# importZL/semantic_segmentation

Measured on AMD Instinct MI355X. Metric: images/sec (fwd+bwd) U-Net 256x256 bs=32 per GPU, higher is better.
Workload: dtype f16; 1 GPU; unet.UNet(1,2) 256x256 fwd+bwd, CE+Dice loss, batch 32/GPU (BASELINE configs[1]); global_batch=32, parallelism=dp1, dice=per-rank

## Files before the change

include/gsseg.h:

```cpp
#ifndef GSSEG_H
#define GSSEG_H

#include <stdint.h>

#ifdef __cplusplus
extern "C" {
#endif

#define GS_ABI_VERSION 52

enum GsDtype { GS_F16 = 0, GS_BF16 = 1 };
enum GsStatus { GS_OK = 0, GS_EINVAL = -1, GS_ELAUNCH = -2, GS_EUNSUPPORTED = -3 };
enum GsAct { GS_ACT_NONE = 0, GS_ACT_RELU = 1, GS_ACT_LEAKY02 = 2, GS_ACT_TANH = 3 };

#define GS_MAX_TAPS 64

typedef struct GsConvGeom {
    int32_t N, IH, IW, Cin, in_pix_stride, in_coff;
    int32_t OHg, OWg, Cout;
    int32_t OH, OW, out_pix_stride, out_coff;
    int32_t isy, isx, osy, osx, ooy, oox;
    int32_t ntaps;
    int32_t tap_dy[GS_MAX_TAPS], tap_dx[GS_MAX_TAPS];
    int32_t tap_w[GS_MAX_TAPS];
    int32_t Dg, Din, Dout, isz, osz, ooz;
    int32_t tap_dz[GS_MAX_TAPS];
} GsConvGeom;

const char* gs_last_error(void);
int gs_abi_version(void);

int gs_conv_igemm_mtiles(const GsConvGeom* g);
int64_t gs_conv_igemm_workspace_floats(void);
int gs_conv_igemm(const GsConvGeom* g, const void* x, const void* w, void* y, const float* bias,
                  float* bn_partials, int act, int dtype, float* splitk_ws, int64_t splitk_ws_floats, void* stream);
int gs_conv_igemm_batch(int n, const GsConvGeom* const* g, const void* x, const void* const* w, void* y, const float* bias,
                        float* const* bn_partials, int act, int dtype, float* splitk_ws, int64_t splitk_ws_floats,
                        void* stream);

int gs_upconv2x2_fwd(const void* x, const void* w, const float* bias, void* y, int N, int D, int IH, int IW, int Cin,
                     int in_pix_stride, int in_coff, int Cout, int Dout, int OH, int OW, int out_pix_stride,
                     int out_coff, int ooz, int ooy, int oox, int act, int dtype, void* stream);

int gs_upconv2x2_dgrad(const void* dy, const void* wd, void* dx, int N, int IH, int IW, int Cin, int Cout, int OH, int OW,
                       int dy_pix_stride, int dy_coff, int ooy, int oox, int dx_pix_stride, int dx_coff, int dtype,
                       void* stream);

int gs_conv3x3_mtiles(int N, int H, int W, int Cout);
int gs_conv3x3_stat_rows(int N, int H, int W, int Cin, int Cout, int pair);
int gs_conv3x3_set_kernel_form(int form);
int gs_set_persistent_grid(int blocks);
int gs_get_persistent_grid(void);
int gs_conv3x3(const void* x, const void* w, void* y, const float* bias, float* bn_partials, int N, int H, int W,
               int Cin, int in_pix_stride, int in_coff, int Cout, int out_pix_stride, int out_coff,
               const int32_t* tap_dy, const int32_t* tap_dx, int act, int dtype, void* stream);

int gs_conv3x3_wgrad(const void* x, const void* dy, float* dw, int N, int H, int W, int Cin, int in_pix_stride,
                     int in_coff, int Cout, int out_pix_stride, int out_coff, int dtype, void* stream);

int gs_conv_wgrad(const GsConvGeom* g, const void* x, const void* dy, float* dw, int dtype, void* stream);
int gs_conv_wgrad_single_pass(const GsConvGeom* g);
int gs_conv_wgrad_assign(const GsConvGeom* g, const void* x, const void* dy, float* dw, int dtype, void* stream);
int gs_conv_wgrad_parts(const GsConvGeom* g);
int64_t gs_conv_wgrad_ws_floats(const GsConvGeom* g);
int gs_conv_wgrad_slabs(const GsConvGeom* g, const void* x, const void* dy, float* ws, int dtype, void* stream);
int gs_conv_wgrad_slabs_batch(int n, const GsConvGeom* const* g, const void* x, const void* dy, float* ws, int dtype,
                              void* stream);

int gs_conv_smallcin_mtiles(int N, int OH, int OW);
int gs_conv_smallcin_fwd(const float* x, const float* w, const float* bias, void* y, float* bn_partials,
                         int N, int Cin, int IH, int IW, int Cout, int OH, int OW, int k, int stride, int pad,
                         int act, int dtype, void* stream);
int64_t gs_conv_direct_wgrad_ws_floats(int N, int OH, int OW, int Cin, int Cout, int k);

int gs_stem_stats(const float* x, const float* w, float* bn_partials, float* tap_sums, int N, int H, int W, void* stream);
int gs_stem_fwd_bn(const float* x, const float* w, const float* bn_scale, const float* bn_shift, int act, void* z, int N,
                   int H, int W, int dtype, void* stream);
int gs_stem_bwd_tiles(int N, int H, int W);
int gs_stem_bwd_onepass(const float* x, const void* z, const void* dz, int dz_stride, int dz_coff, int act,
                        float* s1_partials, float* ws, int N, int H, int W, int dtype, void* stream);
int gs_stem_bwd_finalize(const float* ws, const float* s1_partials, const float* tap_sums, const float* w,
                         const float* scale, const float* mean, const float* invstd, int train_stats, float gscale, float* dw,
                         float* dgamma, float* dbeta, int N, int H, int W, void* stream);

int gs_stem_bn_bwd_wgrad(const void* y, const void* dz, int dz_stride, int dz_coff, const float* x, const float* scale,
                         const float* shift, const float* mean, const float* invstd, const float* c1, const float* c2,
                         int act, float* dw, float* ws, int N, int H, int W, float gscale, int dtype, void* stream);

int gs_conv_smallcin_wgrad(const float* x, const void* dy, float* dw, float* ws, int N, int Cin, int IH, int IW,
                           int Cout, int OH, int OW, int k, int stride, int pad, float gscale, int dtype, void* stream);
int gs_conv_smallcin_dgrad(const void* dy, const float* w, float* dx, int N, int Cin, int IH, int IW, int Cout,
                           int OH, int OW, int k, int stride, int pad, float gscale, int dtype, void* stream);

int gs_conv_smallcout_fwd(const void* x, const float* w, const float* bias, float* y, int N, int IH, int IW, int Cin,
                          int Cout, int OH, int OW, int k, int stride, int pad, int dtype, void* stream);
int gs_conv_smallcout_bwd(const void* x, const float* w, const float* dy, void* dx, float* dw, float* db, float* ws,
                          int N, int IH, int IW, int Cin, int Cout, int OH, int OW, int k, int stride, int pad,
                          float gscale, int dtype, void* stream);

int64_t gs_bn_partials_floats(int ntiles, int C);
int gs_bn_finalize(const float* partials, int ntiles, int C, double count, const float* gamma, const float* beta,
                   float* running_mean, float* running_var, float momentum, float eps,
                   float* scale, float* shift, float* mean, float* invstd, void* stream);
int gs_bn_eval_coeffs(int C, const float* gamma, const float* beta, const float* running_mean,
                      const float* running_var, float eps, float* scale, float* shift, float* mean, float* invstd,
                      void* stream);

int gs_bn_act_apply(const void* y, const float* scale, const float* shift, int act, void* z, int z_pix_stride,
                    int z_coff, void* zp, const uint8_t* keep_mask, float keep_scale, int N, int H, int W, int C,
                    int dtype, void* stream);

int gs_bn_bwd_tiles(int N, int H, int W);
int gs_bn_bwd_tiles_used(int N, int H, int W, int pooled);
int gs_bn_act_bwd_reduce(const void* y, const void* dz_a, int sa, int coff_a, const void* dzp,
                         const void* dz_b, int act_b, const uint8_t* keep_mask, float keep_scale,
                         const float* scale, const float* shift, const float* mean, const float* invstd, int act,
                         float* partials, int N, int H, int W, int C, int dtype, void* stream);
int gs_bn_bwd_coeffs(const float* partials, int ntiles, int C, double count, float gscale, float* dgamma,
                     float* dbeta, float* c1, float* c2, void* stream);
int gs_bn_act_bwd_apply(const void* y, const void* dz_a, int sa, int coff_a, const void* dzp,
                        const void* dz_b, int act_b, const uint8_t* keep_mask, float keep_scale,
                        const float* scale, const float* shift, const float* mean, const float* invstd,
                        const float* c1, const float* c2, int act, int bn, void* dy, int N, int H, int W, int C,
                        int dtype, void* stream);

int gs_maxpool3d_fwd(const void* z, int z_pix_stride, int z_coff, void* zp, int NB, int D, int H, int W, int C,
                     int dtype, void* stream);
int gs_maxpool3d_fwd_pair(const void* z_hi, const void* z_lo, int z_pix_stride, void* zp_hi, void* zp_lo, int zp_pix_stride,
                          int NB, int D, int H, int W, int C, int dtype, void* stream);
int gs_maxpool3d_fwd_pair_q8(const void* z_hi, const void* z_lo, int z_q8, int zq_coff, int z_pix_stride, void* zp_hi, void* zp_lo,
                             int zp_q8, int zp_pix_stride, int NB, int D, int H, int W, int C, int dtype, void* stream);
int gs_maxpool3d_bwd(const void* z, int z_pix_stride, int z_coff, const void* dzp, const void* dres,
                     int res_pix_stride, int res_coff, void* dz, int NB, int D, int H, int W, int C, int dtype,
                     void* stream);

int gs_maxpool2x2_fwd(const void* z, int z_pix_stride, int z_coff, void* zp, int N, int H, int W, int C, int dtype,
                      void* stream);
int gs_maxpool2x2_fwd_pair(const void* z_hi, const void* z_lo, int z_pix_stride, void* zp_hi, void* zp_lo, int zp_pix_stride, int N, int H,
                           int W, int C, int dtype, void* stream);

int gs_colsum(const void* t, int pix_stride, int coff, int N, int H, int W, int y0, int x0, int h, int w, int C,
              float gscale, float* ws, float* out, int dtype, void* stream);

int gs_head1x1_bn_fwd(const void* y_conv, const float* bn_scale, const float* bn_shift, int act, const float* w,
                      const float* bias, float* logits, int N, int H, int W, int Cout, int dtype, void* stream);
int gs_head1x1_bn_wgrad(const void* y_conv, const float* bn_scale, const float* bn_shift, int act, const float* w,
                        const float* dl, float* dw, float* db, float* ws, int N, int H, int W, int Cout, float gscale,
                        int dtype, void* stream);

int gs_bn_act_bwd_reduce_head(const void* y, const float* dl, const float* w_head, int ncls, const float* scale,
                              const float* shift, const float* mean, const float* invstd, int act, float* partials, int N,
                              int H, int W, int C, int dtype, void* stream);
int gs_bn_act_bwd_apply_head(const void* y, const float* dl, const float* w_head, int ncls, const float* scale,
                             const float* shift, const float* mean, const float* invstd, const float* c1, const float* c2,
                             int act, void* dy, int N, int H, int W, int C, int dtype, void* stream);

int gs_bn_partials_colsum(const float* partials, int ntiles, int Cfull, int coff, int C, float gscale, float* out,
                          void* stream);

int gs_pack_weight(const float* w, void* w_fwd, void* w_dgrad, int Cout, int Cin, int taps, int transposed,
                   int dtype, void* stream);

typedef struct GsPackDesc {
    const float* w;
    void* w_fwd;
    void* w_dgrad;
    int32_t Cout, Cin, taps, transposed;
} GsPackDesc;
int gs_pack_weight_multi(int n, const GsPackDesc* descs, int dtype, void* stream);
int gs_unpack_wgrad(const float* dw, float* grad, int A, int B, int taps, int transposed, float gscale, void* stream);

int64_t gs_fake_postprocess_ws_floats(int N);
int gs_fake_postprocess(const float* x, float* out, float* ws, const float* gamma_lut, int N, int64_t hw, void* stream);

int64_t gs_isic_fake_trans_ws_bytes(int planes, int64_t hw);
int gs_isic_fake_trans(const float* x, float* out, void* ws, int N, int C, int H, int W, int equalize_on, int bits,
                       int sharpness_on, float sharp_r1, float sharp_r2, int autocontrast_on, int saturation_on, float sat_r1,
                       float sat_r2, void* stream);

int gs_upconv8_image_fwd(const void* x, int in_pix_stride, int in_coff, const void* pack_fwd, int cpad, const float* bias,
                         float* out, void* u, int N, int h, int w, int Cin, int Cout, int act, int dtype, void* stream);
int gs_upconv8_image_wgrad_ok(int Cin, int Cout);
int64_t gs_upconv8_image_wgrad_ws_floats(int N, int h, int w, int Cin);
int gs_upconv8_image_wgrad(const void* x, int x_pix_stride, const void* du, int du_pix_stride, float* ws, float* dwm, int N, int h, int w,
                           int Cin, int dtype, void* stream);

int gs_upconv_merge_pack(const float* w4, const float* w6, const float* w8, const float* softmax3, void* pack_fwd,
                         void* pack_dgrad, float* merged_f32, int Cin, int Cout, int dtype, void* stream);
int gs_upconv_split_wgrad(const float* dwm, const float* w4, const float* w6, const float* w8, const float* softmax3,
                          float gscale, float* dw4, float* dw6, float* dw8, float* dots3, int Cin, int Cout,
                          void* stream);
int64_t gs_upconv_split_wgrad_ws_floats(int Cin, int Cout);
int gs_upconv_split_wgrad_det(const float* dwm, const float* w4, const float* w6, const float* w8, const float* softmax3,
                              float gscale, float* dw4, float* dw6, float* dw8, float* dots3, float* ws, int Cin, int Cout,
                              void* stream);
int gs_upconv_split_wgrad_parts_ok(int Cin, int Cout);
int gs_upconv_split_wgrad_parts(const float* slabs, int nparts, int64_t part_stride, const float* w4, const float* w6,
                                const float* w8, const float* softmax3, float gscale, float* dw4, float* dw6, float* dw8,
                                float* dots3, float* ws, int Cin, int Cout, void* stream);

int gs_nchw_to_nhwc(const float* src, void* dst, int N, int C, int H, int W, int dst_pix_stride, int dst_coff,
                    int dtype, void* stream);
int gs_nhwc_to_nchw(const void* src, int src_pix_stride, int src_coff, float* dst, int N, int C, int H, int W,
                    float gscale, int dtype, void* stream);

int gs_seg_loss_fwd(const float* logits, const uint8_t* mask, int N, int C, int H, int W, float* ws, float* out,
                    void* stream);
int gs_seg_loss_bwd(const float* logits, const uint8_t* mask, const float* out, const float* gout, float gscale,
                    float* dlogits, int N, int C, int H, int W, void* stream);
int64_t gs_dice_batched_ws_floats(int B);
int gs_dice_coeff_batched(const float* p, const float* t, int B, int64_t n_per, float* ws, float* out, void* stream);
int gs_eval_dice(const float* logits, const uint8_t* mask, int N, int C, int64_t HW, float* ws, float* out, void* stream);
int gs_eval_jaccard(const float* logits, const uint8_t* mask, int N, int64_t HW, float* ws, float* out, void* stream);
int64_t gs_jaccard_loss_out_floats(int N);
int gs_jaccard_seg_loss_fwd(const float* logits, const uint8_t* mask, int N, int64_t HW, float* ws, float* out, void* stream);
int gs_jaccard_seg_loss_bwd(const float* logits, const uint8_t* mask, const float* out, const float* gout, float gscale,
                            float* dlogits, int N, int64_t HW, void* stream);
int gs_dice_loss_fwd(const float* p, const float* t, int64_t n, float* ws, float* out, void* stream);
int gs_dice_loss_bwd(const float* t, const float* out, const float* gout, float* dp, int64_t n, void* stream);
int gs_mean_loss_fwd(const float* x, const float* t, float cval, int mode, int64_t n, float* ws, float* out,
                     void* stream);
int gs_mean_loss_bwd(const float* x, const float* t, float cval, int mode, int64_t n, const float* gout,
                     float gscale, float* dx, void* stream);

int gs_pack_weight_split(const float* w, void* pack, int Cout, int Cin, int taps, int transposed, int dtype, void* stream);
#define GS_SEG_MAX 4
typedef struct GsSegPackDesc {
    const float* w;
    void* pack;
    int32_t Cout, Cin, taps, transposed, nseg;
    int32_t kind[GS_SEG_MAX], ci0[GS_SEG_MAX], len[GS_SEG_MAX];
} GsSegPackDesc;
int gs_pack_weight_segs(int n, const GsSegPackDesc* descs, int dtype, void* stream);
int gs_conv3x3_precise(const void* x, const void* w, void* y_hi, void* y_lo, const float* bias, float* bn_partials, int N,
                       int H, int W, int K, int in_pix_stride, int in_coff, int in_wrap, int Cout, int out_pix_stride,
                       int out_coff, const int32_t* tap_dy, const int32_t* tap_dx, int act, int dtype, void* stream);
typedef struct GsQ8PackDesc {
    const float* w;
    void* pack;
    int32_t* wexp;
    int32_t Cout, Cin, taps;
} GsQ8PackDesc;
int gs_pack_weight_q8(int n, const GsQ8PackDesc* descs, int dtype, void* stream);
int gs_conv3x3_q8_ok(int W, int Cin, int Cout);
int gs_conv3x3_q8(const void* x, const void* w, const int32_t* wexp, void* y_hi, void* y_lo, float* bn_partials, int N, int H, int W,
                  int Cin, int in_pix_stride, int in_coff, int Cout, int out_pix_stride, int out_coff, int dtype, void* stream);
int gs_conv3d_3x3x3_q8(const void* x, const void* w, const int32_t* wexp, void* y_hi, void* y_lo, float* bn_partials, int NB, int D,
                       int H, int W, int Cin, int in_pix_stride, int in_coff, int Cout, int out_pix_stride, int out_coff, int dtype,
                       void* stream);
int gs_bn_act_apply_split_q8(const void* y_hi, const void* y_lo, const float* scale, const float* shift, int act, void* z_hi,
                             void* z_lo, int z_q8, int z_pix_stride, int z_coff, void* zp_hi, void* zp_lo, int zp_q8,
                             int zp_pix_stride, int N, int H, int W, int C, int dtype, void* stream);
int gs_stem_fwd_bn_pair_q8(const float* x, const float* w, const float* bn_scale, const float* bn_shift, int act, void* z_hi,
                           void* z_q, int z_pix_stride, int N, int H, int W, int dtype, void* stream);
int gs_q8_from_hi(const void* x, void* q, int64_t pixels, int C, int pix_stride, int coff, int dtype, void* stream);
int gs_conv3d_3x3x3_precise(const void* x, const void* w, void* y_hi, void* y_lo, const float* bias, float* bn_partials,
                            int NB, int D, int H, int W, int K, int in_pix_stride, int in_coff, int in_wrap, int Cout,
                            int out_pix_stride, int out_coff, const int32_t* tap_dz, const int32_t* tap_dy,
                            const int32_t* tap_dx, int act, int dtype, void* stream);
int gs_conv3d_3x3x3_precise_to(const void* x, const void* w, void* y_hi, void* y_lo, const float* bias, float* bn_partials, int NB, int D,
                               int H, int W, int K, int in_pix_stride, int in_coff, int in_wrap, int in_wrap_to, int Cout, int out_pix_stride,
                               int out_coff, const int32_t* tap_dz, const int32_t* tap_dy, const int32_t* tap_dx, int act, int dtype,
                               void* stream);
int gs_upconv2x2_fwd_precise(const void* x, const void* w, const float* bias, void* y_hi, void* y_lo, int N, int IH, int IW,
                             int K, int in_pix_stride, int in_coff, int in_wrap, int Cout, int OH, int OW,
                             int out_pix_stride, int out_coff, int ooy, int oox, int dtype, void* stream);
int gs_conv_smallcin_fwd_split(const float* x, const float* w, void* y_hi, void* y_lo, float* bn_partials, int N, int Cin,
                               int H, int W, int Cout, int k, int pad, int dtype, void* stream);
int gs_bn_act_apply_split(const void* y_hi, const void* y_lo, const float* scale, const float* shift, int act, void* z_hi,
                          void* z_lo, int z_pix_stride, int z_coff, void* zp_hi, void* zp_lo, int zp_pix_stride, int N,
                          int H, int W, int C, int dtype, void* stream);
int gs_bn_act_apply_split_pool3d(const void* y_hi, const void* y_lo, const float* scale, const float* shift, int act, void* z_hi, void* z_lo,
                                 int z_pix_stride, int z_coff, void* zp_hi, void* zp_lo, int zp_pix_stride, int NB, int D, int H, int W, int C,
                                 int dtype, void* stream);
int gs_head1x1_fwd_split(const void* x_hi, const void* x_lo, const float* w, const float* bias, float* y, int N, int H,
                         int W, int Cin, int Cout, int dtype, void* stream);
int64_t gs_head1x1_wide_bwd_ws_floats(int N, int H, int W, int ncls);
int gs_head1x1_wide_bwd(const void* z, const float* w, const float* dl, void* dz, float* dw, float* db, float* ws, int N, int H,
                        int W, int ncls, float gscale, int dtype, void* stream);
int gs_head1x1_wide_fwd(const void* x, const float* w, const float* bias, float* y, int N, int H, int W, int ncls, int dtype,
                        void* stream);
int gs_conv_widecin_mtiles(int N, int H, int W);
int gs_conv_widecin_fwd_split(const float* x, const float* w, void* y_hi, void* y_lo, float* bn_partials, int N, int Cin, int H,
                              int W, int Cout, int dtype, void* stream);
int gs_head1x1_bn_fwd_split(const void* y_hi, const void* y_lo, const float* scale, const float* shift, int act, const float* w,
                            const float* bias, float* logits, int N, int H, int W, int Cin, int Cout, int dtype, void* stream);
int gs_stem_fwd_bn_pair(const float* x, const float* w, const float* bn_scale, const float* bn_shift, int act, void* z_hi,
                        void* z_lo, int z_pix_stride, int N, int H, int W, int dtype, void* stream);
int gs_stem_bwd_onepass_strided(const float* x, const void* z, int z_pix_stride, const void* dz, int dz_stride, int dz_coff,
                                int act, float* s1_partials, float* ws, int N, int H, int W, int dtype, void* stream);

int gs_upconv2x2_wgrad_parts(int N, int IH, int IW, int Cin, int Cout);
int64_t gs_upconv2x2_wgrad_ws_floats(int N, int IH, int IW, int Cin, int Cout);
int gs_upconv2x2_wgrad_slabs(const void* x, const void* dy, float* ws, int N, int IH, int IW, int Cin, int x_pix_stride,
                             int x_coff, int Cout, int OH, int OW, int dy_pix_stride, int dy_coff, int ooy, int oox, int dtype,
                             void* stream);

int64_t gs_conv3x3_wgrad_ws_floats(int N, int H, int W, int Cin, int Cout);
int gs_conv3x3_wgrad_parts(int N, int H, int W, int Cin, int Cout);
int gs_conv3x3_wgrad_slabs(const void* x, const void* dy, float* ws, int N, int H, int W, int Cin, int in_pix_stride,
                           int in_coff, int Cout, int out_pix_stride, int out_coff, int dtype, void* stream);
int gs_wgrad_reduce_unpack(const float* ws, int nparts, float* grad, int A, int B, int taps, int transposed,
                           float gscale, void* stream);

int gs_conv3d_3x3x3_mtiles(int NB, int D, int H, int W, int Cout);
int gs_conv3d_3x3x3(const void* x, const void* w, void* y, const float* bias, float* bn_partials, int NB, int D, int H,
                    int W, int Cin, int in_pix_stride, int in_coff, int Cout, int out_pix_stride, int out_coff,
                    const int32_t* tap_dz, const int32_t* tap_dy, const int32_t* tap_dx, int act, int dtype, void* stream);
int gs_conv3d_3x3x3_wgrad(const void* x, const void* dy, float* dw, int NB, int D, int H, int W, int Cin,
                          int in_pix_stride, int in_coff, int Cout, int out_pix_stride, int out_coff, int dtype,
                          void* stream);
int64_t gs_conv3d_3x3x3_wgrad_ws_floats(int NB, int D, int H, int W, int Cin, int Cout);
int gs_conv3d_3x3x3_wgrad_parts(int NB, int D, int H, int W, int Cin, int Cout);
int gs_conv3d_3x3x3_wgrad_slabs(const void* x, const void* dy, float* ws, int NB, int D, int H, int W, int Cin,
                                int in_pix_stride, int in_coff, int Cout, int out_pix_stride, int out_coff, int dtype,
                                void* stream);

int gs_upsample2x_bilinear_fwd(const void* x, void* y, int N, int IH, int IW, int C, int in_pix_stride, int in_coff,
                               int OH, int OW, int out_pix_stride, int out_coff, int ooy, int oox, int dtype, void* stream);
int gs_upsample2x_bilinear_fwd_pair(const void* x_hi, const void* x_lo, void* y_hi, void* y_lo, int N, int IH, int IW, int C,
                                    int in_pix_stride, int in_coff, int OH, int OW, int out_pix_stride, int out_coff, int ooy,
                                    int oox, int dtype, void* stream);
int gs_upsample2x_bilinear_bwd(const void* dy, void* dx, int N, int IH, int IW, int C, int dy_pix_stride, int dy_coff,
                               int OH, int OW, int dx_pix_stride, int dx_coff, int ooy, int oox, int dtype, void* stream);

int gs_affine_warp(const float* src, float* dst, const float* mats, int N, int C, int H, int W, float thresh,
                   void* stream);

int gs_optim_chunk_elems(void);
int gs_optim_rmsprop(float* const* params, const float* const* grads, float* const* square_avg,
                     float* const* momentum_buf, const int64_t* sizes, const int32_t* chunk_tensor,
                     const int64_t* chunk_start, int nchunks, float lr, float alpha, float eps, float weight_decay,
                     float momentum, float grad_scale, void* stream);
int gs_optim_adam(float* const* params, const float* const* grads, float* const* exp_avg, float* const* exp_avg_sq,
                  const int64_t* sizes, const int32_t* chunk_tensor, const int64_t* chunk_start, int nchunks,
                  const float* step_scalars, float beta1, float beta2, float eps, float weight_decay, float grad_scale,
                  void* stream);

#ifdef __cplusplus
}
#endif
#endif
```

semantic_segmentation_amd/_lib.py:

```python
from __future__ import annotations

import ctypes
import os
import subprocess
from ctypes import POINTER, c_char_p, c_double, c_float, c_int, c_int32, c_int64, c_void_p

_HERE = os.path.dirname(os.path.abspath(__file__))
LIB_PATH = os.environ.get("GSSEG_LIB", os.path.join(_HERE, "libgsseg_hip.so"))
CSRC = os.path.join(_HERE, "csrc")

GS_F16, GS_BF16 = 0, 1
ACT_NONE, ACT_RELU, ACT_LEAKY02, ACT_TANH = 0, 1, 2, 3
GS_MAX_TAPS = 64
ABI_VERSION = 52


class GsConvGeom(ctypes.Structure):
    _fields_ = [(n, c_int32) for n in (
        "N", "IH", "IW", "Cin", "in_pix_stride", "in_coff", "OHg", "OWg", "Cout", "OH", "OW",
        "out_pix_stride", "out_coff", "isy", "isx", "osy", "osx", "ooy", "oox", "ntaps")] + [
        ("tap_dy", c_int32 * GS_MAX_TAPS), ("tap_dx", c_int32 * GS_MAX_TAPS), ("tap_w", c_int32 * GS_MAX_TAPS)] + [
        (n, c_int32) for n in ("Dg", "Din", "Dout", "isz", "osz", "ooz")] + [("tap_dz", c_int32 * GS_MAX_TAPS)]


class GsPackDesc(ctypes.Structure):
    _fields_ = [("w", c_void_p), ("w_fwd", c_void_p), ("w_dgrad", c_void_p)] + [
        (n, c_int32) for n in ("Cout", "Cin", "taps", "transposed")]


GS_SEG_MAX = 4


class GsSegPackDesc(ctypes.Structure):
    _fields_ = [("w", c_void_p), ("pack", c_void_p)] + [(n, c_int32) for n in ("Cout", "Cin", "taps", "transposed", "nseg")] + [
        ("kind", c_int32 * GS_SEG_MAX), ("ci0", c_int32 * GS_SEG_MAX), ("len", c_int32 * GS_SEG_MAX)]


class GsQ8PackDesc(ctypes.Structure):
    _fields_ = [("w", c_void_p), ("pack", c_void_p), ("wexp", c_void_p)] + [(n, c_int32) for n in ("Cout", "Cin", "taps")]


_P, _F = c_void_p, c_void_p
PROTOTYPES = {
    "gs_last_error": (c_char_p, []),
    "gs_abi_version": (c_int, []),
    "gs_conv_igemm_mtiles": (c_int, [POINTER(GsConvGeom)]),
    "gs_conv3x3_stat_rows": (c_int, [c_int] * 6),
    "gs_upconv2x2_wgrad_parts": (c_int, [c_int] * 5),
    "gs_upconv2x2_wgrad_ws_floats": (c_int64, [c_int] * 5),
    "gs_upconv2x2_wgrad_slabs": (c_int, [_P, _P, _F] + [c_int] * 14 + [c_void_p]),
    "gs_set_persistent_grid": (c_int, [c_int]),
    "gs_get_persistent_grid": (c_int, []),
    "gs_conv_igemm": (c_int, [POINTER(GsConvGeom), _P, _P, _P, _F, _F, c_int, c_int, _F, c_int64, c_void_p]),
    "gs_conv_igemm_workspace_floats": (c_int64, []),
    "gs_conv_igemm_batch": (c_int, [c_int, POINTER(POINTER(GsConvGeom)), _P, POINTER(c_void_p), _P, _F, POINTER(c_void_p),
                                    c_int, c_int, _F, c_int64, c_void_p]),
    "gs_upconv2x2_fwd": (c_int, [_P, _P, _F, _P] + [c_int] * 18 + [c_void_p]),
    "gs_upconv2x2_dgrad": (c_int, [c_void_p, c_void_p, c_void_p] + [c_int] * 14 + [c_void_p]),
    "gs_conv3x3_mtiles": (c_int, [c_int, c_int, c_int, c_int]),
    "gs_conv3x3_set_kernel_form": (c_int, [c_int]),
    "gs_conv3d_3x3x3_mtiles": (c_int, [c_int] * 5),
    "gs_conv3d_3x3x3": (c_int, [_P, _P, _P, _F, _F] + [c_int] * 10 + [POINTER(c_int32)] * 3 + [c_int, c_int, c_void_p]),
    "gs_conv3d_3x3x3_wgrad_ws_floats": (c_int64, [c_int] * 6),
    "gs_conv3d_3x3x3_wgrad_parts": (c_int, [c_int] * 6),
    "gs_conv3d_3x3x3_wgrad_slabs": (c_int, [_P, _P, _F] + [c_int] * 11 + [c_void_p]),
    "gs_conv3d_3x3x3_wgrad": (c_int, [_P, _P, _F] + [c_int] * 11 + [c_void_p]),
    "gs_upsample2x_bilinear_fwd": (c_int, [_P, _P] + [c_int] * 13 + [c_void_p]),
    "gs_upsample2x_bilinear_bwd": (c_int, [_P, _P] + [c_int] * 13 + [c_void_p]),
    "gs_affine_warp": (c_int, [_F, _F, _F, c_int, c_int, c_int, c_int, c_float, c_void_p]),
    "gs_optim_chunk_elems": (c_int, []),
    "gs_optim_rmsprop": (c_int, [_P] * 7 + [c_int] + [c_float] * 6 + [c_void_p]),
    "gs_optim_adam": (c_int, [_P] * 7 + [c_int, _P] + [c_float] * 5 + [c_void_p]),
    "gs_conv3x3": (c_int, [_P, _P, _P, _F, _F] + [c_int] * 9 + [POINTER(c_int32), POINTER(c_int32), c_int, c_int, c_void_p]),
    "gs_conv3x3_wgrad": (c_int, [_P, _P, _F] + [c_int] * 10 + [c_void_p]),
    "gs_conv3x3_wgrad_ws_floats": (c_int64, [c_int] * 5),
    "gs_conv3x3_wgrad_parts": (c_int, [c_int] * 5),
    "gs_conv3x3_wgrad_slabs": (c_int, [_P, _P, _F] + [c_int] * 10 + [c_void_p]),
    "gs_wgrad_reduce_unpack": (c_int, [_F, c_int, _F, c_int, c_int, c_int, c_int, c_float, c_void_p]),
    "gs_conv_wgrad": (c_int, [POINTER(GsConvGeom), _P, _P, _F, c_int, c_void_p]),
    "gs_conv_wgrad_assign": (c_int, [POINTER(GsConvGeom), _P, _P, _F, c_int, c_void_p]),
    "gs_conv_wgrad_single_pass": (c_int, [POINTER(GsConvGeom)]),
    "gs_conv_wgrad_parts": (c_int, [POINTER(GsConvGeom)]),
    "gs_conv_wgrad_ws_floats": (c_int64, [POINTER(GsConvGeom)]),
    "gs_conv_wgrad_slabs": (c_int, [POINTER(GsConvGeom), _P, _P, _F, c_int, c_void_p]),
    "gs_conv_wgrad_slabs_batch": (c_int, [c_int, POINTER(POINTER(GsConvGeom)), _P, _P, _F, c_int, c_void_p]),
    "gs_conv_smallcin_mtiles": (c_int, [c_int, c_int, c_int]),
    "gs_conv_smallcin_fwd": (c_int, [_F, _F, _F, _P, _F] + [c_int] * 12 + [c_void_p]),
    "gs_conv_direct_wgrad_ws_floats": (c_int64, [c_int] * 6),
    "gs_conv_smallcin_wgrad": (c_int, [_F, _P, _F, _F] + [c_int] * 10 + [c_float, c_int, c_void_p]),
    "gs_conv_smallcin_dgrad": (c_int, [_P, _F, _F] + [c_int] * 10 + [c_float, c_int, c_void_p]),
    "gs_conv_smallcout_fwd": (c_int, [_P, _F, _F, _F] + [c_int] * 11 + [c_void_p]),
    "gs_conv_smallcout_bwd": (c_int, [_P, _F, _F, _P, _F, _F, _F] + [c_int] * 10 + [c_float, c_int, c_void_p]),
    "gs_bn_partials_floats": (c_int64, [c_int, c_int]),
    "gs_bn_finalize": (c_int, [_F, c_int, c_int, c_double, _F, _F, _F, _F, c_float, c_float, _F, _F, _F, _F, c_void_p]),
    "gs_bn_eval_coeffs": (c_int, [c_int, _F, _F, _F, _F, c_float, _F, _F, _F, _F, c_void_p]),
    "gs_bn_act_apply": (c_int, [_P, _F, _F, c_int, _P, c_int, c_int, _P, _P, c_float] + [c_int] * 5 + [c_void_p]),
    "gs_bn_bwd_tiles": (c_int, [c_int, c_int, c_int]),
    "gs_bn_bwd_tiles_used": (c_int, [c_int, c_int, c_int, c_int]),
    "gs_bn_act_bwd_reduce": (c_int, [_P, _P, c_int, c_int, _P, _P, c_int, _P, c_float, _F, _F, _F, _F, c_int, _F]
                             + [c_int] * 5 + [c_void_p]),
    "gs_bn_bwd_coeffs": (c_int, [_F, c_int, c_int, c_double, c_float, _F, _F, _F, _F, c_void_p]),
    "gs_bn_act_bwd_apply": (c_int, [_P, _P, c_int, c_int, _P, _P, c_int, _P, c_float, _F, _F, _F, _F, _F, _F, c_int,
                                    c_int, _P]
                            + [c_int] * 5 + [c_void_p]),
    "gs_maxpool3d_fwd": (c_int, [_P, c_int, c_int, _P] + [c_int] * 6 + [c_void_p]),
    "gs_maxpool2x2_fwd": (c_int, [_P, c_int, c_int, _P] + [c_int] * 5 + [c_void_p]),
    "gs_maxpool2x2_fwd_pair": (c_int, [_P, _P, c_int, _P, _P, c_int] + [c_int] * 5 + [c_void_p]),
    "gs_maxpool3d_bwd": (c_int, [_P, c_int, c_int, _P, _P, c_int, c_int, _P] + [c_int] * 6 + [c_void_p]),
    "gs_colsum": (c_int, [_P, c_int, c_int] + [c_int] * 8 + [c_float, _F, _F, c_int, c_void_p]),
    "gs_stem_bn_bwd_wgrad": (c_int, [_P, _P, c_int, c_int, _F, _F, _F, _F, _F, _F, _F, c_int, _F, _F, c_int, c_int, c_int,
                                     c_float, c_int, c_void_p]),
    "gs_stem_stats": (c_int, [_F, _F, _F, _F, c_int, c_int, c_int, c_void_p]),
    "gs_stem_bwd_onepass": (c_int, [_F, _P, _P, c_int, c_int, c_int, _F, _F, c_int, c_int, c_int, c_int, c_void_p]),
    "gs_stem_bwd_finalize": (c_int, [_F, _F, _F, _F, _F, _F, _F, c_int, c_float, _F, _F, _F, c_int, c_int, c_int, c_void_p]),
    "gs_stem_fwd_bn": (c_int, [_F, _F, _F, _F, c_int, _P, c_int, c_int, c_int, c_int, c_void_p]),
    "gs_stem_bwd_tiles": (c_int, [c_int, c_int, c_int]),
    "gs_head1x1_bn_fwd": (c_int, [_P, _F, _F, c_int, _F, _F, _F] + [c_int] * 5 + [c_void_p]),
    "gs_head1x1_bn_wgrad": (c_int, [_P, _F, _F, c_int, _F, _F, _F, _F, _F] + [c_int] * 4 + [c_float, c_int, c_void_p]),
    "gs_bn_act_bwd_reduce_head": (c_int, [_P, _F, _F, c_int, _F, _F, _F, _F, c_int, _F] + [c_int] * 5 + [c_void_p]),
    "gs_bn_act_bwd_apply_head": (c_int, [_P, _F, _F, c_int, _F, _F, _F, _F, _F, _F, c_int, _P] + [c_int] * 5 + [c_void_p]),
    "gs_bn_partials_colsum": (c_int, [_F, c_int, c_int, c_int, c_int, c_float, _F, c_void_p]),
    "gs_pack_weight": (c_int, [_F, _P, _P, c_int, c_int, c_int, c_int, c_int, c_void_p]),
    "gs_pack_weight_multi": (c_int, [c_int, POINTER(GsPackDesc), c_int, c_void_p]),
    "gs_unpack_wgrad": (c_int, [_F, _F, c_int, c_int, c_int, c_int, c_float, c_void_p]),
    "gs_upconv_merge_pack": (c_int, [_F, _F, _F, _F, _P, _P, _F, c_int, c_int, c_int, c_void_p]),
    "gs_fake_postprocess_ws_floats": (c_int64, [c_int]),
    "gs_isic_fake_trans_ws_bytes": (c_int64, [c_int, c_int64]),
    "gs_isic_fake_trans": (c_int, [_F, _F, _P, c_int, c_int, c_int, c_int, c_int, c_int, c_int, c_float, c_float, c_int, c_int,
                                   c_float, c_float, c_void_p]),
    "gs_fake_postprocess": (c_int, [_F, _F, _F, _F, c_int, c_int64, c_void_p]),
    "gs_upconv8_image_fwd": (c_int, [_P, c_int, c_int, _P, c_int, _F, _F, _P] + [c_int] * 7 + [c_void_p]),
    "gs_upconv8_image_wgrad_ok": (c_int, [c_int, c_int]),
    "gs_upconv8_image_wgrad_ws_floats": (c_int64, [c_int] * 4),
    "gs_upconv8_image_wgrad": (c_int, [_P, c_int, _P, c_int, _F, _F] + [c_int] * 5 + [c_void_p]),
    "gs_upconv_split_wgrad": (c_int, [_F, _F, _F, _F, _F, c_float, _F, _F, _F, _F, c_int, c_int, c_void_p]),
    "gs_upconv_split_wgrad_det": (c_int, [_F, _F, _F, _F, _F, c_float, _F, _F, _F, _F, _F, c_int, c_int, c_void_p]),
    "gs_upconv_split_wgrad_ws_floats": (c_int64, [c_int, c_int]),
    "gs_upconv_split_wgrad_parts_ok": (c_int, [c_int, c_int]),
    "gs_upconv_split_wgrad_parts": (c_int, [_F, c_int, c_int64, _F, _F, _F, _F, c_float, _F, _F, _F, _F, _F, c_int, c_int, c_void_p]),
    "gs_nchw_to_nhwc": (c_int, [_F, _P] + [c_int] * 7 + [c_void_p]),
    "gs_nhwc_to_nchw": (c_int, [_P, c_int, c_int, _F] + [c_int] * 4 + [c_float, c_int, c_void_p]),
    "gs_seg_loss_fwd": (c_int, [_F, _P, c_int, c_int, c_int, c_int, _F, _F, c_void_p]),
    "gs_seg_loss_bwd": (c_int, [_F, _P, _F, _F, c_float, _F, c_int, c_int, c_int, c_int, c_void_p]),
    "gs_dice_batched_ws_floats": (c_int64, [c_int]),
    "gs_dice_coeff_batched": (c_int, [_F, _F, c_int, c_int64, _F, _F, c_void_p]),
    "gs_eval_dice": (c_int, [_F, _P, c_int, c_int, c_int64, _F, _F, c_void_p]),
    "gs_jaccard_loss_out_floats": (c_int64, [c_int]),
    "gs_jaccard_seg_loss_fwd": (c_int, [_F, _P, c_int, c_int64, _F, _F, c_void_p]),
    "gs_jaccard_seg_loss_bwd": (c_int, [_F, _P, _F, _F, c_float, _F, c_int, c_int64, c_void_p]),
    "gs_eval_jaccard": (c_int, [_F, _P, c_int, c_int64, _F, _F, c_void_p]),
    "gs_dice_loss_fwd": (c_int, [_F, _F, c_int64, _F, _F, c_void_p]),
    "gs_dice_loss_bwd": (c_int, [_F, _F, _F, _F, c_int64, c_void_p]),
    "gs_mean_loss_fwd": (c_int, [_F, _F, c_float, c_int, c_int64, _F, _F, c_void_p]),
    "gs_pack_weight_split": (c_int, [_F, _P, c_int, c_int, c_int, c_int, c_int, c_void_p]),
    "gs_pack_weight_segs": (c_int, [c_int, POINTER(GsSegPackDesc), c_int, c_void_p]),
    "gs_pack_weight_q8": (c_int, [c_int, POINTER(GsQ8PackDesc), c_int, c_void_p]),
    "gs_conv3x3_q8_ok": (c_int, [c_int] * 3),
    "gs_conv3x3_q8": (c_int, [_P, _P, _P, _P, _P, _F] + [c_int] * 10 + [c_void_p]),
    "gs_conv3d_3x3x3_q8": (c_int, [_P, _P, _P, _P, _P, _F] + [c_int] * 11 + [c_void_p]),
    "gs_bn_act_apply_split_q8": (c_int, [_P, _P, _F, _F, c_int, _P, _P, c_int, c_int, c_int, _P, _P, c_int, c_int] + [c_int] * 5 + [c_void_p]),
    "gs_stem_fwd_bn_pair_q8": (c_int, [_F, _F, _F, _F, c_int, _P, _P, c_int, c_int, c_int, c_int, c_int, c_void_p]),
    "gs_q8_from_hi": (c_int, [_P, _P, c_int64, c_int, c_int, c_int, c_int, c_void_p]),
    "gs_conv3d_3x3x3_precise": (c_int, [_P, _P, _P, _P, _F, _F] + [c_int] * 11 + [POINTER(c_int32)] * 3 + [c_int, c_int, c_void_p]),
    "gs_conv3d_3x3x3_precise_to": (c_int, [_P, _P, _P, _P, _F, _F] + [c_int] * 12 + [POINTER(c_int32)] * 3 + [c_int, c_int, c_void_p]),
    "gs_maxpool3d_fwd_pair_q8": (c_int, [_P, _P, c_int, c_int, c_int, _P, _P, c_int, c_int] + [c_int] * 6 + [c_void_p]),
    "gs_maxpool3d_fwd_pair": (c_int, [_P, _P, c_int, _P, _P] + [c_int] * 7 + [c_void_p]),
    "gs_upsample2x_bilinear_fwd_pair": (c_int, [_P, _P, _P, _P] + [c_int] * 13 + [c_void_p]),
    "gs_conv3x3_precise": (c_int, [_P, _P, _P, _P, _F, _F] + [c_int] * 10 + [POINTER(c_int32), POINTER(c_int32), c_int, c_int, c_void_p]),
    "gs_upconv2x2_fwd_precise": (c_int, [_P, _P, _F, _P, _P] + [c_int] * 15 + [c_void_p]),
    "gs_conv_smallcin_fwd_split": (c_int, [_F, _F, _P, _P, _F] + [c_int] * 8 + [c_void_p]),
    "gs_bn_act_apply_split": (c_int, [_P, _P, _F, _F, c_int, _P, _P, c_int, c_int, _P, _P] + [c_int] * 6 + [c_void_p]),
    "gs_bn_act_apply_split_pool3d": (c_int, [_P, _P, _F, _F, c_int, _P, _P, c_int, c_int, _P, _P] + [c_int] * 7 + [c_void_p]),
    "gs_conv_widecin_mtiles": (c_int, [c_int, c_int, c_int]),
    "gs_conv_widecin_fwd_split": (c_int, [_F, _F, _P, _P, _F] + [c_int] * 6 + [c_void_p]),
    "gs_head1x1_fwd_split": (c_int, [_P, _P, _F, _F, _F] + [c_int] * 6 + [c_void_p]),
    "gs_head1x1_wide_bwd_ws_floats": (c_int64, [c_int] * 4),
    "gs_head1x1_wide_bwd": (c_int, [_P, _F, _F, _P, _F, _F, _F] + [c_int] * 4 + [c_float, c_int, c_void_p]),
    "gs_head1x1_wide_fwd": (c_int, [_P, _F, _F, _F] + [c_int] * 5 + [c_void_p]),
    "gs_head1x1_bn_fwd_split": (c_int, [_P, _P, _F, _F, c_int, _F, _F, _F] + [c_int] * 6 + [c_void_p]),
    "gs_stem_fwd_bn_pair": (c_int, [_F, _F, _F, _F, c_int, _P, _P, c_int, c_int, c_int, c_int, c_int, c_void_p]),
    "gs_stem_bwd_onepass_strided": (c_int, [_F, _P, c_int, _P, c_int, c_int, c_int, _F, _F, c_int, c_int, c_int, c_int, c_void_p]),
    "gs_mean_loss_bwd": (c_int, [_F, _F, c_float, c_int, c_int64, _F, c_float, _F, c_void_p]),
}

_lib = None


def build(verbose: bool = False) -> str:
    cmd = ["make", "-C", CSRC, "-j", str(min(8, os.cpu_count() or 1))]
    res = subprocess.run(cmd, stdout=subprocess.PIPE, stderr=subprocess.STDOUT, text=True)
    if verbose or res.returncode != 0:
        print(res.stdout)
    if res.returncode != 0:
        raise RuntimeError("building libgsseg_hip.so failed:\n" + res.stdout[-4000:])
    return LIB_PATH


def load():
    global _lib
    if _lib is not None:
        return _lib
    import torch
    if not os.path.exists(LIB_PATH):
        raise RuntimeError(
            f"{LIB_PATH} not found: the HIP extension is not built.  Run "
            "`python -c 'import __graft_entry__ as g; g.build()'` (or make -C semantic_segmentation_amd/csrc). "
            "There is no CPU/PyTorch fallback for this path.")
    lib = ctypes.CDLL(LIB_PATH)
    for name, (res, args) in PROTOTYPES.items():
        fn = getattr(lib, name)
        fn.restype = res
        fn.argtypes = args
    if lib.gs_abi_version() != ABI_VERSION:
        raise RuntimeError(f"libgsseg_hip.so ABI {lib.gs_abi_version()} != binding {ABI_VERSION}: rebuild")
    _lib = lib
    return lib


GS_EUNSUPPORTED = -3


def check(rc: int, what: str = "") -> None:
    if rc != 0:
        msg = load().gs_last_error()
        raise RuntimeError(f"{what or 'gsseg'} failed (status {rc}): {msg.decode() if msg else ''}")


def call(name: str, *args):
    rc = getattr(load(), name)(*args)
    if rc != 0:
        check(rc, name)
    return rc
```

semantic_segmentation_amd/csrc/bn.hip:

```cpp
#include <stdlib.h>

#include "common.hpp"

namespace {

constexpr int RED_SLICES = 64;

__global__ __launch_bounds__(256) void reduce_partials_stage1(const float* __restrict__ part, int ntiles, int C,
                                                              int tiles_per_slice, double* __restrict__ out1) {
    __shared__ double red[2][8][32];
    const int cl = threadIdx.x & 31, tl = threadIdx.x >> 5;
    const int c = blockIdx.x * 32 + cl;
    const int t0 = blockIdx.y * tiles_per_slice, t1 = min(ntiles, t0 + tiles_per_slice);
    double s1 = 0.0, s2 = 0.0;
    if (c < C) {
        for (int tt = t0 + tl; tt < t1; tt += 8) {
            s1 += (double)part[((int64_t)tt * 2 + 0) * C + c];
            s2 += (double)part[((int64_t)tt * 2 + 1) * C + c];
        }
    }
    red[0][tl][cl] = s1;
    red[1][tl][cl] = s2;
    __syncthreads();
    if (tl == 0 && c < C) {
        double a = 0.0, b = 0.0;
#pragma unroll
        for (int i = 0; i < 8; ++i) { a += red[0][i][cl]; b += red[1][i][cl]; }
        out1[((int64_t)blockIdx.y * 2 + 0) * C + c] = a;
        out1[((int64_t)blockIdx.y * 2 + 1) * C + c] = b;
    }
}

template <typename T>
__device__ __forceinline__ void sum_slices_32x8(const T* __restrict__ s, int nslices, int C, double& s1, double& s2) {
    __shared__ double red[2][8][32];
    const int cl = threadIdx.x & 31, tl = threadIdx.x >> 5;
    const int c = blockIdx.x * 32 + cl;
    double a = 0.0, b = 0.0;
    if (c < C) {
#pragma unroll 4
        for (int i = tl; i < nslices; i += 8) { a += (double)s[((int64_t)i * 2 + 0) * C + c]; b += (double)s[((int64_t)i * 2 + 1) * C + c]; }
    }
    red[0][tl][cl] = a;
    red[1][tl][cl] = b;
    __syncthreads();
    s1 = 0.0; s2 = 0.0;
#pragma unroll
    for (int i = 0; i < 8; ++i) { s1 += red[0][i][cl]; s2 += red[1][i][cl]; }
}

template <typename T>
__global__ __launch_bounds__(256) void bn_finalize_kernel(const T* __restrict__ s, int nslices, int C, double count,
                                                          const float* __restrict__ gamma, const float* __restrict__ beta,
                                                          float* running_mean, float* running_var, float momentum,
                                                          float eps, float* scale, float* shift, float* mean_out,
                                                          float* invstd_out) {
    double s1, s2;
    sum_slices_32x8(s, nslices, C, s1, s2);
    const int c = blockIdx.x * 32 + (threadIdx.x & 31);
    if (c >= C || threadIdx.x >= 32) return;
    const double mean = s1 / count;
    double var = s2 / count - mean * mean;
    if (var < 0.0) var = 0.0;
    const float invstd = (float)(1.0 / sqrt(var + (double)eps));
    const float gm = gamma ? gamma[c] : 1.f, bt = beta ? beta[c] : 0.f;
    const float sc = gm * invstd;
    scale[c] = sc;
    shift[c] = bt - (float)mean * sc;
    mean_out[c] = (float)mean;
    invstd_out[c] = invstd;
    if (running_mean) running_mean[c] = (1.f - momentum) * running_mean[c] + momentum * (float)mean;
    if (running_var) {
        const double unb = count > 1.0 ? var * (count / (count - 1.0)) : var;
        running_var[c] = (1.f - momentum) * running_var[c] + momentum * (float)unb;
    }
}

__global__ void bn_eval_coeffs_kernel(int C, const float* gamma, const float* beta, const float* rm, const float* rv,
                                      float eps, float* scale, float* shift, float* mean, float* invstd) {
    const int c = blockIdx.x * blockDim.x + threadIdx.x;
    if (c >= C) return;
    const float is = 1.f / sqrtf(rv[c] + eps);
    const float sc = (gamma ? gamma[c] : 1.f) * is;
    scale[c] = sc;
    shift[c] = (beta ? beta[c] : 0.f) - rm[c] * sc;
    mean[c] = rm[c];
    invstd[c] = is;
}

template <typename T>
__global__ __launch_bounds__(256) void bn_bwd_coeffs_kernel(const T* __restrict__ s, int nslices, int C, double count,
                                                            float gscale, float* dgamma, float* dbeta, float* c1, float* c2) {
    double s1, s2;
    sum_slices_32x8(s, nslices, C, s1, s2);
    const int c = blockIdx.x * 32 + (threadIdx.x & 31);
    if (c >= C || threadIdx.x >= 32) return;
    if (dbeta) dbeta[c] = (float)(s1 * gscale);
    if (dgamma) dgamma[c] = (float)(s2 * gscale);
    c1[c] = (float)(s1 / count);
    c2[c] = (float)(s2 / count);
}

static int bn_traversal() {
    static const int v = getenv("GSSEG_BN_REV") ? atoi(getenv("GSSEG_BN_REV")) : 3;
    return v;
}

struct ApplyArgs {
    const unsigned short* y;
    const float* scale;
    const float* shift;
    unsigned short* z;
    unsigned short* zp;
    const uint8_t* keep;
    float keep_scale;
    int act, N, H, W, C, zs, zc;
    int rev;
};

template <int DT, bool POOL, bool GENERIC>
__global__ __launch_bounds__(256) void bn_act_apply_kernel(const ApplyArgs a) {
    const float slope = a.act == GS_ACT_RELU ? 0.f : (a.act == GS_ACT_LEAKY02 ? 0.2f : 1.f);
    auto fwd_a = [&](float v) __attribute__((always_inline)) { return GENERIC ? act_fwd(v, a.act) : (v > 0.f ? v : v * slope); };
    const int nch = a.C >> 3;
    const int PH = POOL ? (a.H + 1) / 2 : a.H, PW = POOL ? (a.W + 1) / 2 : a.W;
    const int64_t total = (int64_t)a.N * PH * PW * nch;
    for (int64_t lidx = (int64_t)blockIdx.x * blockDim.x + threadIdx.x; lidx < total;
         lidx += (int64_t)gridDim.x * blockDim.x) {
        const int64_t idx = a.rev ? total - 1 - lidx : lidx;
        const int ch = (int)(idx % nch);
        int64_t pidx = idx / nch;
        const int px = (int)(pidx % PW); pidx /= PW;
        const int py = (int)(pidx % PH);
        const int n = (int)(pidx / PH);
        const int c0 = ch * 8;
        float sc[8], sh[8];
        if (a.scale) {
#pragma unroll
            for (int i = 0; i < 8; ++i) { sc[i] = a.scale[c0 + i]; sh[i] = a.shift[c0 + i]; }
        } else {
#pragma unroll
            for (int i = 0; i < 8; ++i) { sc[i] = 1.f; sh[i] = 0.f; }
        }
        if (!POOL) {
            const int64_t pix = ((int64_t)n * a.H + py) * a.W + px;
            float v[8];
            unpack8<DT>(*reinterpret_cast<const uint4*>(a.y + pix * a.C + c0), v);
#pragma unroll
            for (int i = 0; i < 8; ++i) v[i] = fwd_a(v[i] * sc[i] + sh[i]);
            if (a.keep) {
                const uint2 k = *reinterpret_cast<const uint2*>(a.keep + pix * a.C + c0);
                const unsigned int kw[2] = {k.x, k.y};
#pragma unroll
                for (int i = 0; i < 8; ++i) v[i] *= ((kw[i >> 2] >> (8 * (i & 3))) & 0xffu) ? a.keep_scale : 0.f;
            }
            st16(a.z + pix * a.zs + a.zc + c0, pack8<DT>(v));
        } else {
            float mx[8];
#pragma unroll
            for (int i = 0; i < 8; ++i) mx[i] = -INFINITY;
#pragma unroll
            for (int dy = 0; dy < 2; ++dy)
#pragma unroll
                for (int dx = 0; dx < 2; ++dx) {
                    const int yy = 2 * py + dy, xx = 2 * px + dx;
                    if (yy < a.H && xx < a.W) {
                        const int64_t pix = ((int64_t)n * a.H + yy) * a.W + xx;
                        float v[8];
                        unpack8<DT>(*reinterpret_cast<const uint4*>(a.y + pix * a.C + c0), v);
#pragma unroll
                        for (int i = 0; i < 8; ++i) v[i] = fwd_a(v[i] * sc[i] + sh[i]);
                        const uint4 pk = pack8<DT>(v);
                        st16(a.z + pix * a.zs + a.zc + c0, pk);
                        float r[8];
                        unpack8<DT>(pk, r);
#pragma unroll
                        for (int i = 0; i < 8; ++i) mx[i] = fmaxf(mx[i], r[i]);
                    }
                }
            if (py < a.H / 2 && px < a.W / 2) {
                const int64_t pp = ((int64_t)n * (a.H / 2) + py) * (a.W / 2) + px;
                st16(a.zp + pp * a.C + c0, pack8<DT>(mx));
            }
        }
    }
}

__device__ __forceinline__ float mul_rn(float a, float b) {
    float r;
    asm("v_mul_f32 %0, %1, %2" : "=v"(r) : "v"(a), "v"(b));
    return r;
}

struct BwdArgs {
    const unsigned short* y;
    const unsigned short* dza;
    const unsigned short* dzp;
    const unsigned short* dzb;
    const uint8_t* keep;
    float keep_scale;
    int act_b;
    const float *scale, *shift, *mean, *invstd, *c1, *c2;
    float* partials;
    unsigned short* dy;
    int sa, ca, act, bn, N, H, W, C;
    int tile_units;
    int rev;
    const float* head_dl;
    const float* head_w;
    int head_n;
};

template <int DT, bool POOL, bool APPLY, bool GENERIC, int HEAD = 0, bool EXTRA = true, bool RN = false>
__global__ __launch_bounds__(256) void bn_act_bwd_kernel(const BwdArgs a) {
    static_assert(!HEAD || (!POOL && !GENERIC), "the head source: plain pixels, slope-family activation");
    static_assert(!(RN && GENERIC), "the rounded slope product belongs to the slope family");
    auto mul_g = [&](float g, float d) __attribute__((always_inline)) { return RN ? mul_rn(g, d) : g * d; };
    constexpr int NH = HEAD ? HEAD : 1;
    constexpr int HEAD_CHUNK = 2048;
    __shared__ float hdl[HEAD ? NH * HEAD_CHUNK : 1];
    __shared__ float red[2][256 * 8 / 8][8];
    const float slope_a = a.act == GS_ACT_RELU ? 0.f : (a.act == GS_ACT_LEAKY02 ? 0.2f : 1.f);
    const float slope_b = a.act_b == GS_ACT_RELU ? 0.f : (a.act_b == GS_ACT_LEAKY02 ? 0.2f : 1.f);
    auto grad_a = [&](float v) __attribute__((always_inline)) { return GENERIC ? act_grad(v, a.act) : (v > 0.f ? 1.f : slope_a); };
    auto grad_b = [&](float v) __attribute__((always_inline)) { return GENERIC ? act_grad(v, a.act_b) : (v > 0.f ? 1.f : slope_b); };
    auto fwd_a = [&](float v) __attribute__((always_inline)) { return GENERIC ? act_fwd(v, a.act) : (v > 0.f ? v : v * slope_a); };
    const int nch = a.C >> 3;
    const int PH = POOL ? (a.H + 1) / 2 : a.H, PW = POOL ? (a.W + 1) / 2 : a.W;
    const int units = a.N * PH * PW;
    const int lanes_per_unit = nch < 256 ? nch : 256;
    const int unit_lanes = 256 / lanes_per_unit;
    const int chl = threadIdx.x % lanes_per_unit, ul = threadIdx.x / lanes_per_unit;
    const int tile = a.rev ? (int)(gridDim.x - 1 - blockIdx.x) : (int)blockIdx.x;
    const int u0 = tile * a.tile_units;
    int u1 = u0 + a.tile_units < units ? u0 + a.tile_units : units;
    if (ul >= unit_lanes) u1 = u0;
    constexpr int UNR = 4;

    for (int ch = chl; ch - chl < nch; ch += lanes_per_unit) {
        const bool ch_ok = ch < nch;
        const int c0 = ch_ok ? ch * 8 : 0;
        if (!ch_ok) u1 = u0;
        float sc[8], sh[8], mu[8], is[8], k1[8], k2[8];
#pragma unroll
        for (int i = 0; i < 8; ++i) {
            sc[i] = a.scale ? a.scale[c0 + i] : 1.f;
            sh[i] = a.shift ? a.shift[c0 + i] : 0.f;
            mu[i] = a.mean ? a.mean[c0 + i] : 0.f;
            is[i] = a.invstd ? a.invstd[c0 + i] : 1.f;
            k1[i] = (APPLY && a.c1) ? a.c1[c0 + i] : 0.f;
            k2[i] = (APPLY && a.c2) ? a.c2[c0 + i] : 0.f;
        }
        float s1[8], s2[8];
#pragma unroll
        for (int i = 0; i < 8; ++i) { s1[i] = 0.f; s2[i] = 0.f; }
        float hw[NH][8];
        if (HEAD) {
#pragma unroll
            for (int k = 0; k < NH; ++k)
#pragma unroll
                for (int i = 0; i < 8; ++i) hw[k][i] = k < a.head_n ? a.head_w[k * a.C + c0 + i] : 0.f;
        }
        const int HWp = a.H * a.W;

        if (!POOL) {
            const int tile_end = u0 + a.tile_units < units ? u0 + a.tile_units : units;
            const int chunk = HEAD ? HEAD_CHUNK : (tile_end - u0 > 0 ? tile_end - u0 : 1);
            for (int cb = u0; cb < tile_end; cb += chunk) {
            const int ce = cb + chunk < tile_end ? cb + chunk : tile_end;
            if (HEAD) {
                __syncthreads();
                for (int i = threadIdx.x; i < ce - cb; i += 256) {
                    const int p = cb + i, n = p / HWp, hwp = p - n * HWp;
#pragma unroll
                    for (int q = 0; q < NH; ++q) hdl[q * HEAD_CHUNK + i] = q < a.head_n ? a.head_dl[((int64_t)n * a.head_n + q) * HWp + hwp] : 0.f;
                }
                __syncthreads();
            }
            const int ue = ce < u1 ? ce : u1;
            for (int ub = cb + ul; ub < ue; ub += unit_lanes * UNR) {
                uint4 ry[UNR], rg[UNR], rb[UNR];
                uint2 rk[UNR];
                bool ok[UNR];
                float hd[UNR][NH];
#pragma unroll
                for (int k = 0; k < UNR; ++k) {
                    const int u = ub + k * unit_lanes;
                    ok[k] = u < ue;
                    const int64_t pix = ok[k] ? u : cb;
                    ry[k] = *reinterpret_cast<const uint4*>(a.y + pix * a.C + c0);
                    if (HEAD) {
#pragma unroll
                        for (int q = 0; q < NH; ++q) hd[k][q] = hdl[q * HEAD_CHUNK + (int)pix - cb];
                        rg[k] = make_uint4(0, 0, 0, 0);
                    } else {
                        rg[k] = a.dza ? *reinterpret_cast<const uint4*>(a.dza + pix * a.sa + a.ca + c0) : make_uint4(0, 0, 0, 0);
                    }
                    rb[k] = (EXTRA && a.dzb) ? *reinterpret_cast<const uint4*>(a.dzb + pix * a.C + c0) : make_uint4(0, 0, 0, 0);
                    rk[k] = (EXTRA && a.keep) ? *reinterpret_cast<const uint2*>(a.keep + pix * a.C + c0) : make_uint2(0, 0);
                }
#pragma unroll
                for (int k = 0; k < UNR; ++k) {
                    if (!ok[k]) continue;
                    const int64_t pix = ub + k * unit_lanes;
                    float yv[8], g[8], gb[8], out[8];
                    unpack8<DT>(ry[k], yv);
                    unpack8<DT>(rg[k], g);
                    unpack8<DT>(rb[k], gb);
                    if (HEAD) {
#pragma unroll
                        for (int i = 0; i < 8; ++i) {
                            float t = hd[k][0] * hw[0][i];
#pragma unroll
                            for (int q = 1; q < NH; ++q) t += hd[k][q] * hw[q][i];
                            g[i] = t;
                        }
                    }
                    if (EXTRA && a.keep) {
                        const unsigned int kw[2] = {rk[k].x, rk[k].y};
#pragma unroll
                        for (int i = 0; i < 8; ++i) g[i] *= ((kw[i >> 2] >> (8 * (i & 3))) & 0xffu) ? a.keep_scale : 0.f;
                    }
#pragma unroll
                    for (int i = 0; i < 8; ++i) {
                        const float v = yv[i] * sc[i] + sh[i];
                        const float gh = mul_g(g[i], grad_a(v)) + ((EXTRA && a.dzb) ? mul_g(gb[i], grad_b(v)) : 0.f);
                        const float xh = (yv[i] - mu[i]) * is[i];
                        if (APPLY) out[i] = a.bn ? sc[i] * (gh - k1[i] - xh * k2[i]) : gh;
                        else { s1[i] += gh; s2[i] += gh * xh; }
                    }
                    if (APPLY) st16(a.dy + pix * a.C + c0, pack8<DT>(out));
                }
            }
            }
        } else {
            const int PH2 = a.H / 2, PW2 = a.W / 2;
            for (int u = u0 + ul; u < u1; u += unit_lanes) {
                const int px = u % PW;
                const int r = u / PW;
                const int py = r % PH;
                const int n = r / PH;
                uint4 ry[4], rg[4];
                bool ok[4];
                int64_t pixk[4];
#pragma unroll
                for (int k = 0; k < 4; ++k) {
                    const int yy = 2 * py + (k >> 1), xx = 2 * px + (k & 1);
                    ok[k] = yy < a.H && xx < a.W;
                    pixk[k] = ((int64_t)n * a.H + (yy < a.H ? yy : a.H - 1)) * a.W + (xx < a.W ? xx : a.W - 1);
                    ry[k] = *reinterpret_cast<const uint4*>(a.y + pixk[k] * a.C + c0);
                    rg[k] = a.dza ? *reinterpret_cast<const uint4*>(a.dza + pixk[k] * a.sa + a.ca + c0) : make_uint4(0, 0, 0, 0);
                }
                const bool pooled = (py < PH2) && (px < PW2);
                uint4 rp = make_uint4(0, 0, 0, 0);
                if (pooled && a.dzp) {
                    const int64_t pp = ((int64_t)n * PH2 + py) * PW2 + px;
                    rp = *reinterpret_cast<const uint4*>(a.dzp + pp * a.C + c0);
                }
                float yv[4][8], zr[4][8], gp[8];
                unpack8<DT>(rp, gp);
#pragma unroll
                for (int k = 0; k < 4; ++k) {
                    unpack8<DT>(ry[k], yv[k]);
                    float zt[8];
#pragma unroll
                    for (int i = 0; i < 8; ++i) zt[i] = fwd_a(yv[k][i] * sc[i] + sh[i]);
                    const uint4 pk = pack8<DT>(zt);
                    unpack8<DT>(pk, zr[k]);
                    if (!ok[k]) {
#pragma unroll
                        for (int i = 0; i < 8; ++i) zr[k][i] = -INFINITY;
                    }
                }
                int amax[8];
#pragma unroll
                for (int i = 0; i < 8; ++i) {
                    int best = 0; float bv = zr[0][i];
#pragma unroll
                    for (int k = 1; k < 4; ++k) if (zr[k][i] > bv) { bv = zr[k][i]; best = k; }
                    amax[i] = best;
                }
#pragma unroll
                for (int k = 0; k < 4; ++k) {
                    if (!ok[k]) continue;
                    float g[8], out[8];
                    unpack8<DT>(rg[k], g);
#pragma unroll
                    for (int i = 0; i < 8; ++i) {
                        const float gz = g[i] + (amax[i] == k ? gp[i] : 0.f);
                        const float v = yv[k][i] * sc[i] + sh[i];
                        const float gh = mul_g(gz, grad_a(v));
                        const float xh = (yv[k][i] - mu[i]) * is[i];
                        if (APPLY) out[i] = a.bn ? sc[i] * (gh - k1[i] - xh * k2[i]) : gh;
                        else { s1[i] += gh; s2[i] += gh * xh; }
                    }
                    if (APPLY) st16(a.dy + pixk[k] * a.C + c0, pack8<DT>(out));
                }
            }
        }
        if (!APPLY) {
            __syncthreads();
#pragma unroll
            for (int i = 0; i < 8; ++i) { red[0][threadIdx.x][i] = s1[i]; red[1][threadIdx.x][i] = s2[i]; }
            __syncthreads();
            const int nv = lanes_per_unit * 8;
            for (int v = threadIdx.x; v < 2 * nv; v += 256) {
                const int st = v >= nv ? 1 : 0, idx = v - st * nv;
                const int cl = idx >> 3, i = idx & 7;
                if (ch - chl + cl >= nch) continue;
                float tsum = 0.f;
                for (int k = 0; k < unit_lanes; ++k) tsum += red[st][k * lanes_per_unit + cl][i];
                a.partials[(int64_t)tile * 2 * a.C + st * a.C + (ch - chl + cl) * 8 + i] = tsum;
            }
        }
    }
}

template <int DT>
__global__ __launch_bounds__(256) void colsum_stage1(const unsigned short* __restrict__ t, int ps, int coff,
                                                     int64_t npix, int C, int64_t pix_per_block, float* ws,
                                                     int H, int W, int y0, int x0, int h, int w) {
    __shared__ float red[256][8];
    const int nch = C >> 3;
    const int lpu = nch < 256 ? nch : 256, ulanes = 256 / lpu;
    const int chl = threadIdx.x % lpu, ul = threadIdx.x / lpu;
    const int64_t p0 = (int64_t)blockIdx.x * pix_per_block;
    int64_t p1 = p0 + pix_per_block < npix ? p0 + pix_per_block : npix;
    if (ul >= ulanes) p1 = p0;
    for (int ch = chl; ch - chl < nch; ch += lpu) {
        float s[8];
#pragma unroll
        for (int i = 0; i < 8; ++i) s[i] = 0.f;
        if (ch >= nch) p1 = p0;
        for (int64_t p = p0 + ul; p < p1; p += ulanes) {
            float v[8];
            const int xx = (int)(p % w);
            const int64_t r = p / w;
            const int yy = (int)(r % h);
            const int64_t n = r / h;
            const int64_t pp = (n * H + y0 + yy) * W + x0 + xx;
            unpack8<DT>(*reinterpret_cast<const uint4*>(t + pp * ps + coff + ch * 8), v);
#pragma unroll
            for (int i = 0; i < 8; ++i) s[i] += v[i];
        }
        __syncthreads();
#pragma unroll
        for (int i = 0; i < 8; ++i) red[threadIdx.x][i] = s[i];
        __syncthreads();
        for (int v = threadIdx.x; v < lpu * 8; v += 256) {
            const int cl = v >> 3, i = v & 7;
            if (ch - chl + cl >= nch) continue;
            float tt = 0.f;
            for (int k = 0; k < ulanes; ++k) tt += red[k * lpu + cl][i];
            ws[(int64_t)blockIdx.x * C + (ch - chl + cl) * 8 + i] = tt;
        }
    }
}
__global__ __launch_bounds__(256) void colsum_stage2(const float* ws, int nblocks, int C, float gscale, float* out) {
    __shared__ double red[8][32];
    const int cl = threadIdx.x & 31, tl = threadIdx.x >> 5;
    const int c = blockIdx.x * 32 + cl;
    double s = 0.0;
    if (c < C) {
        double a[8] = {0, 0, 0, 0, 0, 0, 0, 0};
        int i = tl;
        for (; i + 56 < nblocks; i += 64) {
            float v[8];
#pragma unroll
            for (int u = 0; u < 8; ++u) v[u] = ws[(int64_t)(i + 8 * u) * C + c];
#pragma unroll
            for (int u = 0; u < 8; ++u) a[u] += (double)v[u];
        }
        for (; i < nblocks; i += 8) a[0] += (double)ws[(int64_t)i * C + c];
        s = ((a[0] + a[1]) + (a[2] + a[3])) + ((a[4] + a[5]) + (a[6] + a[7]));
    }
    red[tl][cl] = s;
    __syncthreads();
    if (tl == 0 && c < C) {
        double t = 0.0;
#pragma unroll
        for (int i = 0; i < 8; ++i) t += red[i][cl];
        out[c] = (float)(t * gscale);
    }
}

__global__ __launch_bounds__(256) void partials_colsum_stage1(const float* __restrict__ part, int ntiles, int Cfull, int coff, int C,
                                                              int tiles_per_slice, double* __restrict__ out1) {
    __shared__ double red[8][32];
    const int cl = threadIdx.x & 31, tl = threadIdx.x >> 5;
    const int c = blockIdx.x * 32 + cl;
    const int t0 = blockIdx.y * tiles_per_slice, t1 = min(ntiles, t0 + tiles_per_slice);
    double s1 = 0.0;
    if (c < C)
        for (int tt = t0 + tl; tt < t1; tt += 8) s1 += (double)part[(int64_t)tt * 2 * Cfull + coff + c];
    red[tl][cl] = s1;
    __syncthreads();
    if (tl == 0 && c < C) {
        double a = 0.0;
#pragma unroll
        for (int i = 0; i < 8; ++i) a += red[i][cl];
        out1[(int64_t)blockIdx.y * C + c] = a;
    }
}

template <typename T>
__global__ __launch_bounds__(256) void partials_colsum_final(const T* __restrict__ s, int n, int64_t stride, int C, float gscale,
                                                             float* __restrict__ out) {
    __shared__ double red[8][32];
    const int cl = threadIdx.x & 31, tl = threadIdx.x >> 5;
    const int c = blockIdx.x * 32 + cl;
    double a = 0.0;
    if (c < C) {
#pragma unroll 4
        for (int i = tl; i < n; i += 8) a += (double)s[(int64_t)i * stride + c];
    }
    red[tl][cl] = a;
    __syncthreads();
    if (tl == 0 && c < C) {
        double t = 0.0;
#pragma unroll
        for (int i = 0; i < 8; ++i) t += red[i][cl];
        out[c] = (float)(t * gscale);
    }
}

int direct_tiles() {
    static const int v = getenv("GSSEG_BN_DIRECT_TILES") ? atoi(getenv("GSSEG_BN_DIRECT_TILES")) : 512;
    return v;
}

int reduce_partials(const float* partials, int ntiles, int C, double** out, int* nslices, hipStream_t s) {
    int slices = ntiles < RED_SLICES ? ntiles : RED_SLICES;
    const int tps = cdiv(ntiles, slices);
    slices = cdiv(ntiles, tps);
    size_t off = ((size_t)ntiles * 2 * C * sizeof(float) + 15) & ~(size_t)15;
    double* o1 = (double*)((char*)partials + off);
    reduce_partials_stage1<<<dim3(cdiv(C, 32), slices), 256, 0, s>>>(partials, ntiles, C, tps, o1);
    *out = o1;
    *nslices = slices;
    return 0;
}

}

extern "C" int64_t gs_bn_partials_floats(int ntiles, int C) {
    return (int64_t)ntiles * 2 * C + 4 + (int64_t)RED_SLICES * 2 * C * 2;
}

extern "C" int gs_bn_finalize(const float* partials, int ntiles, int C, double count, const float* gamma,
                              const float* beta, float* running_mean, float* running_var, float momentum, float eps,
                              float* scale, float* shift, float* mean, float* invstd, void* stream) {
    GS_CHECK_ARG(partials && scale && shift && mean && invstd && ntiles > 0 && C > 0 && count > 0,
                 "gs_bn_finalize: bad arguments");
    hipStream_t s = (hipStream_t)stream;
    if (ntiles <= direct_tiles()) {
        bn_finalize_kernel<float><<<cdiv(C, 32), 256, 0, s>>>(partials, ntiles, C, count, gamma, beta, running_mean, running_var,
                                                               momentum, eps, scale, shift, mean, invstd);
        GS_CHECK_LAUNCH("gs_bn_finalize");
        return GS_OK;
    }
    double* o1; int ns;
    reduce_partials(partials, ntiles, C, &o1, &ns, s);
    bn_finalize_kernel<double><<<cdiv(C, 32), 256, 0, s>>>(o1, ns, C, count, gamma, beta, running_mean, running_var,
                                                            momentum, eps, scale, shift, mean, invstd);
    GS_CHECK_LAUNCH("gs_bn_finalize");
    return GS_OK;
}

extern "C" int gs_bn_eval_coeffs(int C, const float* gamma, const float* beta, const float* running_mean,
                                 const float* running_var, float eps, float* scale, float* shift, float* mean,
                                 float* invstd, void* stream) {
    GS_CHECK_ARG(C > 0 && running_mean && running_var && scale && shift && mean && invstd, "gs_bn_eval_coeffs: bad args");
    bn_eval_coeffs_kernel<<<cdiv(C, 128), 128, 0, (hipStream_t)stream>>>(C, gamma, beta, running_mean, running_var, eps,
                                                                         scale, shift, mean, invstd);
    GS_CHECK_LAUNCH("gs_bn_eval_coeffs");
    return GS_OK;
}

extern "C" int gs_bn_act_apply(const void* y, const float* scale, const float* shift, int act, void* z,
                               int z_pix_stride, int z_coff, void* zp, const uint8_t* keep_mask, float keep_scale,
                               int N, int H, int W, int C, int dtype, void* stream) {
    GS_CHECK_ARG(y && z && N > 0 && H > 0 && W > 0 && C > 0 && C % 8 == 0, "gs_bn_act_apply: bad arguments");
    GS_CHECK_ARG(z_pix_stride >= z_coff + C && z_pix_stride % 8 == 0 && z_coff % 8 == 0, "gs_bn_act_apply: bad z stride");
    GS_CHECK_ARG((scale == nullptr) == (shift == nullptr), "gs_bn_act_apply: scale/shift must both be given or NULL");
    GS_CHECK_ARG(!(zp && keep_mask), "gs_bn_act_apply: pool + dropout not supported together");
    ApplyArgs a{(const unsigned short*)y, scale, shift, (unsigned short*)z, (unsigned short*)zp, keep_mask, keep_scale,
                act, N, H, W, C, z_pix_stride, z_coff, bn_traversal() & 1};
    const bool pool = zp != nullptr;
    const int PH = pool ? (H + 1) / 2 : H, PW = pool ? (W + 1) / 2 : W;
    const int64_t total = (int64_t)N * PH * PW * (C / 8);
    int64_t blocks = cdiv64(total, 256);
    if (blocks > 256 * 16) blocks = 256 * 16;
    hipStream_t s = (hipStream_t)stream;
    const bool generic = act == GS_ACT_TANH;
    if (dtype == GS_F16) {
        if (generic) {
            if (pool) bn_act_apply_kernel<GS_F16, true, true><<<(int)blocks, 256, 0, s>>>(a);
            else bn_act_apply_kernel<GS_F16, false, true><<<(int)blocks, 256, 0, s>>>(a);
        } else {
            if (pool) bn_act_apply_kernel<GS_F16, true, false><<<(int)blocks, 256, 0, s>>>(a);
            else bn_act_apply_kernel<GS_F16, false, false><<<(int)blocks, 256, 0, s>>>(a);
        }
    } else if (dtype == GS_BF16) {
        if (generic) {
            if (pool) bn_act_apply_kernel<GS_BF16, true, true><<<(int)blocks, 256, 0, s>>>(a);
            else bn_act_apply_kernel<GS_BF16, false, true><<<(int)blocks, 256, 0, s>>>(a);
        } else {
            if (pool) bn_act_apply_kernel<GS_BF16, true, false><<<(int)blocks, 256, 0, s>>>(a);
            else bn_act_apply_kernel<GS_BF16, false, false><<<(int)blocks, 256, 0, s>>>(a);
        }
    } else {
        GS_CHECK_ARG(false, "gs_bn_act_apply: bad dtype");
    }
    GS_CHECK_LAUNCH("gs_bn_act_apply");
    return GS_OK;
}

static int bwd_tile_units(int64_t units) {
    int64_t tu = cdiv64(units, 1024);
    if (tu < 64) tu = 64;
    return (int)tu;
}

extern "C" int gs_bn_bwd_tiles(int N, int H, int W) {
    const int64_t units = (int64_t)N * H * W;
    return (int)cdiv64(units, bwd_tile_units(units));
}

static int launch_bwd(const BwdArgs& a0, bool apply, int dtype, hipStream_t s, int* ntiles_out) {
    BwdArgs a = a0;
    a.rev = (bn_traversal() >> (apply ? 2 : 1)) & 1;
    const bool pool = a.dzp != nullptr;
    const int PH = pool ? (a.H + 1) / 2 : a.H, PW = pool ? (a.W + 1) / 2 : a.W;
    const int64_t units = (int64_t)a.N * PH * PW;
    const int ntiles_max = gs_bn_bwd_tiles(a.N, a.H, a.W);
    a.tile_units = (int)cdiv64(units, ntiles_max);
    if (a.tile_units < 1) a.tile_units = 1;
    const int ntiles = (int)cdiv64(units, a.tile_units);
    if (ntiles_out) *ntiles_out = ntiles;
    const bool generic = a.act == GS_ACT_TANH || (a.dzb && a.act_b == GS_ACT_TANH);
    const bool leaky = !generic && (a.act == GS_ACT_LEAKY02 || (a.dzb && a.act_b == GS_ACT_LEAKY02));
#define LAUNCH(DT, G, R)                                                                                \
    do {                                                                                                \
        if (pool) {                                                                                     \
            if (apply) bn_act_bwd_kernel<DT, true, true, G, 0, true, R><<<ntiles, 256, 0, s>>>(a);      \
            else bn_act_bwd_kernel<DT, true, false, G, 0, true, R><<<ntiles, 256, 0, s>>>(a);           \
        } else if (a.dzb != nullptr || a.keep != nullptr) {                                             \
            if (apply) bn_act_bwd_kernel<DT, false, true, G, 0, true, R><<<ntiles, 256, 0, s>>>(a);     \
            else bn_act_bwd_kernel<DT, false, false, G, 0, true, R><<<ntiles, 256, 0, s>>>(a);          \
        } else {                                                                                        \
            if (apply) bn_act_bwd_kernel<DT, false, true, G, 0, false, R><<<ntiles, 256, 0, s>>>(a);    \
            else bn_act_bwd_kernel<DT, false, false, G, 0, false, R><<<ntiles, 256, 0, s>>>(a);         \
        }                                                                                               \
    } while (0)
    if (a.head_dl != nullptr) {
#define LAUNCH_HEAD(DT, NC, R)                                                                          \
    do {                                                                                                \
        if (apply) bn_act_bwd_kernel<DT, false, true, false, NC, false, R><<<ntiles, 256, 0, s>>>(a);   \
        else bn_act_bwd_kernel<DT, false, false, false, NC, false, R><<<ntiles, 256, 0, s>>>(a);        \
    } while (0)
#define LAUNCH_HEAD_N(DT, R) do { if (a.head_n <= 2) LAUNCH_HEAD(DT, 2, R); else LAUNCH_HEAD(DT, 4, R); } while (0)
        if (dtype == GS_F16) { if (leaky) LAUNCH_HEAD_N(GS_F16, true); else LAUNCH_HEAD_N(GS_F16, false); }
        else { if (leaky) LAUNCH_HEAD_N(GS_BF16, true); else LAUNCH_HEAD_N(GS_BF16, false); }
#undef LAUNCH_HEAD_N
#undef LAUNCH_HEAD
        return 0;
    }
    if (dtype == GS_F16) { if (generic) LAUNCH(GS_F16, true, false); else if (leaky) LAUNCH(GS_F16, false, true); else LAUNCH(GS_F16, false, false); }
    else { if (generic) LAUNCH(GS_BF16, true, false); else if (leaky) LAUNCH(GS_BF16, false, true); else LAUNCH(GS_BF16, false, false); }
#undef LAUNCH
    return 0;
}

extern "C" int gs_bn_bwd_tiles_used(int N, int H, int W, int pooled) {
    const int PH = pooled ? (H + 1) / 2 : H, PW = pooled ? (W + 1) / 2 : W;
    const int64_t units = (int64_t)N * PH * PW;
    const int ntiles_max = gs_bn_bwd_tiles(N, H, W);
    int64_t tu = cdiv64(units, ntiles_max);
    if (tu < 1) tu = 1;
    return (int)cdiv64(units, tu);
}

extern "C" int gs_bn_act_bwd_reduce(const void* y, const void* dz_a, int sa, int coff_a, const void* dzp,
                                    const void* dz_b, int act_b, const uint8_t* keep_mask, float keep_scale,
                                    const float* scale, const float* shift, const float* mean, const float* invstd,
                                    int act, float* partials, int N, int H, int W, int C, int dtype, void* stream) {
    GS_CHECK_ARG(!(dzp && (dz_b || keep_mask)), "gs_bn_act_bwd_reduce: pooled gradient cannot be combined with dz_b / keep_mask");
    GS_CHECK_ARG(y && partials && (dz_a || dzp || dz_b) && N > 0 && H > 0 && W > 0 && C > 0 && C % 8 == 0 && C <= 2048,
                 "gs_bn_act_bwd_reduce: bad arguments");
    GS_CHECK_ARG(dtype == GS_F16 || dtype == GS_BF16, "gs_bn_act_bwd_reduce: bad dtype");
    GS_CHECK_ARG((int64_t)N * H * W < 2147483647LL, "gs_bn_act_bwd_reduce: more than 2^31 pixels");
    GS_CHECK_ARG(!dz_a || (sa >= coff_a + C && sa % 8 == 0 && coff_a % 8 == 0), "gs_bn_act_bwd_reduce: bad dz stride");
    BwdArgs a{};
    a.y = (const unsigned short*)y; a.dza = (const unsigned short*)dz_a; a.dzp = (const unsigned short*)dzp;
    a.scale = scale; a.shift = shift; a.mean = mean; a.invstd = invstd; a.c1 = nullptr; a.c2 = nullptr;
    a.dzb = (const unsigned short*)dz_b; a.act_b = act_b; a.keep = keep_mask; a.keep_scale = keep_scale;
    a.partials = partials; a.dy = nullptr; a.sa = sa; a.ca = coff_a; a.act = act; a.bn = 1;
    a.N = N; a.H = H; a.W = W; a.C = C;
    launch_bwd(a, false, dtype, (hipStream_t)stream, nullptr);
    GS_CHECK_LAUNCH("gs_bn_act_bwd_reduce");
    return GS_OK;
}

extern "C" int gs_bn_bwd_coeffs(const float* partials, int ntiles, int C, double count, float gscale, float* dgamma,
                                float* dbeta, float* c1, float* c2, void* stream) {
    GS_CHECK_ARG(partials && c1 && c2 && ntiles > 0 && C > 0 && count > 0, "gs_bn_bwd_coeffs: bad arguments");
    hipStream_t s = (hipStream_t)stream;
    if (ntiles <= direct_tiles()) {
        bn_bwd_coeffs_kernel<float><<<cdiv(C, 32), 256, 0, s>>>(partials, ntiles, C, count, gscale, dgamma, dbeta, c1, c2);
        GS_CHECK_LAUNCH("gs_bn_bwd_coeffs");
        return GS_OK;
    }
    double* o1; int ns;
    reduce_partials(partials, ntiles, C, &o1, &ns, s);
    bn_bwd_coeffs_kernel<double><<<cdiv(C, 32), 256, 0, s>>>(o1, ns, C, count, gscale, dgamma, dbeta, c1, c2);
    GS_CHECK_LAUNCH("gs_bn_bwd_coeffs");
    return GS_OK;
}

extern "C" int gs_bn_act_bwd_apply(const void* y, const void* dz_a, int sa, int coff_a, const void* dzp,
                                   const void* dz_b, int act_b, const uint8_t* keep_mask, float keep_scale,
                                   const float* scale, const float* shift, const float* mean, const float* invstd,
                                   const float* c1, const float* c2, int act, int bn, void* dy, int N, int H, int W,
                                   int C, int dtype, void* stream) {
    GS_CHECK_ARG(!(dzp && (dz_b || keep_mask)), "gs_bn_act_bwd_apply: pooled gradient cannot be combined with dz_b / keep_mask");
    GS_CHECK_ARG(y && dy && (dz_a || dzp || dz_b) && N > 0 && H > 0 && W > 0 && C > 0 && C % 8 == 0 && C <= 2048,
                 "gs_bn_act_bwd_apply: bad arguments");
    GS_CHECK_ARG(dtype == GS_F16 || dtype == GS_BF16, "gs_bn_act_bwd_apply: bad dtype");
    GS_CHECK_ARG((int64_t)N * H * W < 2147483647LL, "gs_bn_act_bwd_apply: more than 2^31 pixels");
    GS_CHECK_ARG(!bn || (scale && shift && mean && invstd && c1 && c2), "gs_bn_act_bwd_apply: bn=1 needs all coefficients");
    GS_CHECK_ARG(!dz_a || (sa >= coff_a + C && sa % 8 == 0 && coff_a % 8 == 0), "gs_bn_act_bwd_apply: bad dz stride");
    BwdArgs a{};
    a.y = (const unsigned short*)y; a.dza = (const unsigned short*)dz_a; a.dzp = (const unsigned short*)dzp;
    a.scale = scale; a.shift = shift; a.mean = mean; a.invstd = invstd; a.c1 = c1; a.c2 = c2;
    a.dzb = (const unsigned short*)dz_b; a.act_b = act_b; a.keep = keep_mask; a.keep_scale = keep_scale;
    a.partials = nullptr; a.dy = (unsigned short*)dy; a.sa = sa; a.ca = coff_a; a.act = act; a.bn = bn;
    a.N = N; a.H = H; a.W = W; a.C = C;
    launch_bwd(a, true, dtype, (hipStream_t)stream, nullptr);
    GS_CHECK_LAUNCH("gs_bn_act_bwd_apply");
    return GS_OK;
}

static int bn_head_args(const char* who, BwdArgs& a, const void* y, const float* dl, const float* w_head, int ncls,
                        const float* scale, const float* shift, const float* mean, const float* invstd, int act, int N, int H,
                        int W, int C, int dtype) {
    GS_CHECK_ARG(y && dl && w_head && ncls >= 1 && ncls <= 4 && N > 0 && H > 0 && W > 0 && C > 0 && C % 8 == 0 && C <= 2048,
                 "%s: bad arguments", who);
    GS_CHECK_ARG(dtype == GS_F16 || dtype == GS_BF16, "%s: bad dtype", who);
    GS_CHECK_ARG((int64_t)N * H * W < 2147483647LL, "%s: more than 2^31 pixels", who);
    GS_CHECK_ARG(act == GS_ACT_NONE || act == GS_ACT_RELU || act == GS_ACT_LEAKY02, "%s: activation %d not supported", who, act);
    GS_CHECK_ARG(scale && shift && mean && invstd, "%s: needs the BatchNorm coefficients", who);
    a.y = (const unsigned short*)y; a.head_dl = dl; a.head_w = w_head; a.head_n = ncls;
    a.scale = scale; a.shift = shift; a.mean = mean; a.invstd = invstd; a.act = act; a.bn = 1;
    a.N = N; a.H = H; a.W = W; a.C = C;
    return GS_OK;
}

extern "C" int gs_bn_act_bwd_reduce_head(const void* y, const float* dl, const float* w_head, int ncls, const float* scale,
                                         const float* shift, const float* mean, const float* invstd, int act, float* partials,
                                         int N, int H, int W, int C, int dtype, void* stream) {
    BwdArgs a{};
    int rc = bn_head_args("gs_bn_act_bwd_reduce_head", a, y, dl, w_head, ncls, scale, shift, mean, invstd, act, N, H, W, C, dtype);
    if (rc) return rc;
    GS_CHECK_ARG(partials != nullptr, "gs_bn_act_bwd_reduce_head: null partials");
    a.partials = partials;
    launch_bwd(a, false, dtype, (hipStream_t)stream, nullptr);
    GS_CHECK_LAUNCH("gs_bn_act_bwd_reduce_head");
    return GS_OK;
}

extern "C" int gs_bn_act_bwd_apply_head(const void* y, const float* dl, const float* w_head, int ncls, const float* scale,
                                        const float* shift, const float* mean, const float* invstd, const float* c1,
                                        const float* c2, int act, void* dy, int N, int H, int W, int C, int dtype, void* stream) {
    BwdArgs a{};
    int rc = bn_head_args("gs_bn_act_bwd_apply_head", a, y, dl, w_head, ncls, scale, shift, mean, invstd, act, N, H, W, C, dtype);
    if (rc) return rc;
    GS_CHECK_ARG(dy && c1 && c2, "gs_bn_act_bwd_apply_head: null pointer");
    a.c1 = c1; a.c2 = c2; a.dy = (unsigned short*)dy;
    launch_bwd(a, true, dtype, (hipStream_t)stream, nullptr);
    GS_CHECK_LAUNCH("gs_bn_act_bwd_apply_head");
    return GS_OK;
}

extern "C" int gs_bn_partials_colsum(const float* partials, int ntiles, int Cfull, int coff, int C, float gscale, float* out,
                                     void* stream) {
    GS_CHECK_ARG(partials && out && ntiles > 0 && Cfull > 0 && C > 0 && coff >= 0 && coff + C <= Cfull,
                 "gs_bn_partials_colsum: bad arguments");
    hipStream_t s = (hipStream_t)stream;
    if (ntiles <= direct_tiles()) {
        partials_colsum_final<float><<<cdiv(C, 32), 256, 0, s>>>(partials + coff, ntiles, (int64_t)2 * Cfull, C, gscale, out);
    } else {
        int slices = ntiles < RED_SLICES ? ntiles : RED_SLICES;
        const int tps = cdiv(ntiles, slices);
        slices = cdiv(ntiles, tps);
        double* o1 = (double*)((char*)partials + (((size_t)ntiles * 2 * Cfull * sizeof(float) + 15) & ~(size_t)15));
        partials_colsum_stage1<<<dim3(cdiv(C, 32), slices), 256, 0, s>>>(partials, ntiles, Cfull, coff, C, tps, o1);
        partials_colsum_final<double><<<cdiv(C, 32), 256, 0, s>>>(o1, slices, (int64_t)C, C, gscale, out);
    }
    GS_CHECK_LAUNCH("gs_bn_partials_colsum");
    return GS_OK;
}

extern "C" int gs_colsum(const void* t, int pix_stride, int coff, int N, int H, int W, int y0, int x0, int h, int w,
                         int C, float gscale, float* ws, float* out, int dtype, void* stream) {
    GS_CHECK_ARG(t && ws && out && N > 0 && h > 0 && w > 0 && y0 >= 0 && x0 >= 0 && y0 + h <= H && x0 + w <= W,
                 "gs_colsum: bad region");
    GS_CHECK_ARG(C > 0 && C % 8 == 0 && C <= 2048 && pix_stride % 8 == 0 && coff % 8 == 0, "gs_colsum: bad channels");
    hipStream_t s = (hipStream_t)stream;
    const int64_t npix = (int64_t)N * h * w;
    int64_t ppb = cdiv64(npix, 1024);
    if (ppb < 32) ppb = 32;
    const int nb = (int)cdiv64(npix, ppb);
    if (dtype == GS_F16)
        colsum_stage1<GS_F16><<<nb, 256, 0, s>>>((const unsigned short*)t, pix_stride, coff, npix, C, ppb, ws, H, W, y0, x0, h, w);
    else if (dtype == GS_BF16)
        colsum_stage1<GS_BF16><<<nb, 256, 0, s>>>((const unsigned short*)t, pix_stride, coff, npix, C, ppb, ws, H, W, y0, x0, h, w);
    else GS_CHECK_ARG(false, "gs_colsum: bad dtype");
    colsum_stage2<<<cdiv(C, 32), 256, 0, s>>>(ws, nb, C, gscale, out);
    GS_CHECK_LAUNCH("gs_colsum");
    return GS_OK;
}
```

semantic_segmentation_amd/csrc/pack.hip:

```cpp
#include "common.hpp"

namespace {

template <int DT>
__global__ __launch_bounds__(256) void pack_weight_kernel(const float* __restrict__ w, unsigned short* wf,
                                                          unsigned short* wd, int Cout, int Cin, int T, int transposed) {
    const int64_t total = (int64_t)Cout * Cin * T;
    for (int64_t i = (int64_t)blockIdx.x * 256 + threadIdx.x; i < total; i += (int64_t)gridDim.x * 256) {
        const int ci = (int)(i % Cin);
        int64_t r = i / Cin;
        const int co = (int)(r % Cout);
        const int t = (int)(r / Cout);
        const int64_t src = transposed ? (((int64_t)ci * Cout + co) * T + t) : (((int64_t)co * Cin + ci) * T + t);
        const unsigned short v = Elem<DT>::from_f(w[src]);
        if (wf) wf[i] = v;
        if (wd) wd[((int64_t)t * Cin + ci) * Cout + co] = v;
    }
}

template <int DT, int T>
__global__ __launch_bounds__(256) void pack_weight_rows_kernel(const float* __restrict__ w, unsigned short* p_ab,
                                                               unsigned short* p_ba, int A, int B) {
    const int64_t n = (int64_t)A * B;
    const bool ba = blockIdx.y == 1;
    unsigned short* dst = ba ? p_ba : p_ab;
    if (dst == nullptr) return;
    for (int64_t i = (int64_t)blockIdx.x * 256 + threadIdx.x; i < n; i += (int64_t)gridDim.x * 256) {
        int a, b;
        if (!ba) { b = (int)(i % B); a = (int)(i / B); }
        else { a = (int)(i % A); b = (int)(i / A); }
        const float* src = w + ((int64_t)a * B + b) * T;
        float v[T];
#pragma unroll
        for (int t = 0; t < T; ++t) v[t] = src[t];
#pragma unroll
        for (int t = 0; t < T; ++t) dst[(int64_t)t * n + i] = Elem<DT>::from_f(v[t]);
    }
}

constexpr int PACK_MULTI_MAX = 32;
struct PackMultiArgs {
    const float* w[PACK_MULTI_MAX];
    unsigned short* p_ab[PACK_MULTI_MAX];
    unsigned short* p_ba[PACK_MULTI_MAX];
    int A[PACK_MULTI_MAX], B[PACK_MULTI_MAX], T[PACK_MULTI_MAX], first[PACK_MULTI_MAX + 1];
    int n;
};

template <int DT, int T>
__device__ __forceinline__ void pack_rows_body(const float* __restrict__ w, unsigned short* dst, int A, int B, bool ba,
                                               int block, int nblocks) {
    const int64_t n = (int64_t)A * B;
    for (int64_t i = (int64_t)block * 256 + threadIdx.x; i < n; i += (int64_t)nblocks * 256) {
        int a, b;
        if (!ba) { b = (int)(i % B); a = (int)(i / B); }
        else { a = (int)(i % A); b = (int)(i / A); }
        const float* src = w + ((int64_t)a * B + b) * T;
        float v[T];
#pragma unroll
        for (int t = 0; t < T; ++t) v[t] = src[t];
#pragma unroll
        for (int t = 0; t < T; ++t) dst[(int64_t)t * n + i] = Elem<DT>::from_f(v[t]);
    }
}

template <int DT>
__global__ __launch_bounds__(256) void pack_weight_multi_kernel(const PackMultiArgs a) {
    int d = 0;
    while (d + 1 < a.n && (int)blockIdx.x >= a.first[d + 1]) ++d;
    const bool ba = blockIdx.y == 1;
    unsigned short* dst = ba ? a.p_ba[d] : a.p_ab[d];
    if (dst == nullptr) return;
    const int block = blockIdx.x - a.first[d], nblocks = a.first[d + 1] - a.first[d];
    if (a.T[d] == 9) pack_rows_body<DT, 9>(a.w[d], dst, a.A[d], a.B[d], ba, block, nblocks);
    else if (a.T[d] == 27) pack_rows_body<DT, 27>(a.w[d], dst, a.A[d], a.B[d], ba, block, nblocks);
    else if (a.T[d] == 8) pack_rows_body<DT, 8>(a.w[d], dst, a.A[d], a.B[d], ba, block, nblocks);
    else pack_rows_body<DT, 4>(a.w[d], dst, a.A[d], a.B[d], ba, block, nblocks);
}

__global__ __launch_bounds__(256) void unpack_wgrad_kernel(const float* __restrict__ dw, float* __restrict__ grad,
                                                           int A, int B, int T, int transposed, float gscale) {
    const int64_t total = (int64_t)A * B * T;
    for (int64_t i = (int64_t)blockIdx.x * 256 + threadIdx.x; i < total; i += (int64_t)gridDim.x * 256) {
        const int t = (int)(i % T);
        int64_t r = i / T;
        int a, b;
        if (!transposed) { b = (int)(r % B); a = (int)(r / B); }
        else { a = (int)(r % A); b = (int)(r / A); }
        grad[i] = dw[((int64_t)t * A + a) * B + b] * gscale;
    }
}

template <int DT>
__global__ __launch_bounds__(256) void nchw_to_nhwc_kernel(const float* __restrict__ src, unsigned short* dst, int N,
                                                           int C, int64_t HW, int ds, int dc) {
    const int64_t total = (int64_t)N * HW * C;
    for (int64_t i = (int64_t)blockIdx.x * 256 + threadIdx.x; i < total; i += (int64_t)gridDim.x * 256) {
        const int c = (int)(i % C);
        const int64_t pix = i / C;
        const int64_t n = pix / HW, hw = pix - n * HW;
        dst[pix * ds + dc + c] = Elem<DT>::from_f(src[(n * C + c) * HW + hw]);
    }
}

template <int DT>
__global__ __launch_bounds__(256) void nhwc_to_nchw_kernel(const unsigned short* __restrict__ src, int ss, int sc,
                                                           float* __restrict__ dst, int N, int C, int64_t HW, float gscale) {
    const int64_t total = (int64_t)N * HW * C;
    for (int64_t i = (int64_t)blockIdx.x * 256 + threadIdx.x; i < total; i += (int64_t)gridDim.x * 256) {
        const int64_t hw = i % HW;
        int64_t r = i / HW;
        const int c = (int)(r % C);
        const int64_t n = r / C;
        dst[i] = Elem<DT>::to_f(src[(n * HW + hw) * ss + sc + c]) * gscale;
    }
}

inline int ew_blocks(int64_t n) {
    int64_t b = cdiv64(n, 256);
    if (b > 8192) b = 8192;
    if (b < 1) b = 1;
    return (int)b;
}

}

extern "C" int gs_pack_weight(const float* w, void* w_fwd, void* w_dgrad, int Cout, int Cin, int taps, int transposed,
                              int dtype, void* stream) {
    GS_CHECK_ARG(w && (w_fwd || w_dgrad) && Cout > 0 && Cin > 0 && taps > 0, "gs_pack_weight: bad arguments");
    const int64_t total = (int64_t)Cout * Cin * taps;
    hipStream_t s = (hipStream_t)stream;
    GS_CHECK_ARG(dtype == GS_F16 || dtype == GS_BF16, "gs_pack_weight: bad dtype");
    if (taps == 1 || taps == 4 || taps == 9 || taps == 16 || taps == 27) {
        const int A = transposed ? Cin : Cout, B = transposed ? Cout : Cin;
        unsigned short* p_ab = (unsigned short*)(transposed ? w_dgrad : w_fwd);
        unsigned short* p_ba = (unsigned short*)(transposed ? w_fwd : w_dgrad);
        dim3 grid(ew_blocks((int64_t)A * B), 2);
#define GS_PACK_ROWS(DT, TT) pack_weight_rows_kernel<DT, TT><<<grid, 256, 0, s>>>(w, p_ab, p_ba, A, B)
#define GS_PACK_T(DT)                                    \
        switch (taps) {                                  \
            case 1: GS_PACK_ROWS(DT, 1); break;          \
            case 4: GS_PACK_ROWS(DT, 4); break;          \
            case 9: GS_PACK_ROWS(DT, 9); break;          \
            case 16: GS_PACK_ROWS(DT, 16); break;        \
            default: GS_PACK_ROWS(DT, 27); break;        \
        }
        if (dtype == GS_F16) { GS_PACK_T(GS_F16) } else { GS_PACK_T(GS_BF16) }
#undef GS_PACK_T
#undef GS_PACK_ROWS
        GS_CHECK_LAUNCH("gs_pack_weight");
        return GS_OK;
    }
    if (dtype == GS_F16)
        pack_weight_kernel<GS_F16><<<ew_blocks(total), 256, 0, s>>>(w, (unsigned short*)w_fwd, (unsigned short*)w_dgrad,
                                                                    Cout, Cin, taps, transposed);
    else if (dtype == GS_BF16)
        pack_weight_kernel<GS_BF16><<<ew_blocks(total), 256, 0, s>>>(w, (unsigned short*)w_fwd, (unsigned short*)w_dgrad,
                                                                     Cout, Cin, taps, transposed);
    else GS_CHECK_ARG(false, "gs_pack_weight: bad dtype");
    GS_CHECK_LAUNCH("gs_pack_weight");
    return GS_OK;
}

extern "C" int gs_pack_weight_multi(int n, const GsPackDesc* descs, int dtype, void* stream) {
    GS_CHECK_ARG(n > 0 && descs != nullptr, "gs_pack_weight_multi: no descriptors");
    GS_CHECK_ARG(dtype == GS_F16 || dtype == GS_BF16, "gs_pack_weight_multi: bad dtype");
    hipStream_t s = (hipStream_t)stream;
    for (int base = 0; base < n; base += PACK_MULTI_MAX) {
        PackMultiArgs a;
        a.n = n - base < PACK_MULTI_MAX ? n - base : PACK_MULTI_MAX;
        int blocks = 0;
        for (int i = 0; i < a.n; ++i) {
            const GsPackDesc& d = descs[base + i];
            GS_CHECK_ARG(d.w && (d.w_fwd || d.w_dgrad) && d.Cout > 0 && d.Cin > 0 &&
                         (d.taps == 9 || d.taps == 4 || d.taps == 27 || d.taps == 8),
                         "gs_pack_weight_multi: descriptor %d: needs w, a pack, positive dims and 9 / 4 (2-D) or 27 / 8 (3-D) taps", base + i);
            a.w[i] = d.w;
            a.A[i] = d.transposed ? d.Cin : d.Cout;
            a.B[i] = d.transposed ? d.Cout : d.Cin;
            a.T[i] = d.taps;
            a.p_ab[i] = (unsigned short*)(d.transposed ? d.w_dgrad : d.w_fwd);
            a.p_ba[i] = (unsigned short*)(d.transposed ? d.w_fwd : d.w_dgrad);
            a.first[i] = blocks;
            int b = ew_blocks((int64_t)a.A[i] * a.B[i]);
            if (b > 512) b = 512;
            blocks += b;
        }
        a.first[a.n] = blocks;
        dim3 grid(blocks, 2);
        if (dtype == GS_F16) pack_weight_multi_kernel<GS_F16><<<grid, 256, 0, s>>>(a);
        else pack_weight_multi_kernel<GS_BF16><<<grid, 256, 0, s>>>(a);
        GS_CHECK_LAUNCH("gs_pack_weight_multi");
    }
    return GS_OK;
}

extern "C" int gs_unpack_wgrad(const float* dw, float* grad, int A, int B, int taps, int transposed, float gscale,
                               void* stream) {
    GS_CHECK_ARG(dw && grad && A > 0 && B > 0 && taps > 0, "gs_unpack_wgrad: bad arguments");
    const int64_t total = (int64_t)A * B * taps;
    unpack_wgrad_kernel<<<ew_blocks(total), 256, 0, (hipStream_t)stream>>>(dw, grad, A, B, taps, transposed, gscale);
    GS_CHECK_LAUNCH("gs_unpack_wgrad");
    return GS_OK;
}

extern "C" int gs_nchw_to_nhwc(const float* src, void* dst, int N, int C, int H, int W, int dst_pix_stride,
                               int dst_coff, int dtype, void* stream) {
    GS_CHECK_ARG(src && dst && N > 0 && C > 0 && H > 0 && W > 0 && dst_pix_stride >= dst_coff + C,
                 "gs_nchw_to_nhwc: bad arguments");
    const int64_t total = (int64_t)N * C * H * W;
    hipStream_t s = (hipStream_t)stream;
    if (dtype == GS_F16)
        nchw_to_nhwc_kernel<GS_F16><<<ew_blocks(total), 256, 0, s>>>(src, (unsigned short*)dst, N, C, (int64_t)H * W,
                                                                     dst_pix_stride, dst_coff);
    else if (dtype == GS_BF16)
        nchw_to_nhwc_kernel<GS_BF16><<<ew_blocks(total), 256, 0, s>>>(src, (unsigned short*)dst, N, C, (int64_t)H * W,
                                                                      dst_pix_stride, dst_coff);
    else GS_CHECK_ARG(false, "gs_nchw_to_nhwc: bad dtype");
    GS_CHECK_LAUNCH("gs_nchw_to_nhwc");
    return GS_OK;
}

extern "C" int gs_nhwc_to_nchw(const void* src, int src_pix_stride, int src_coff, float* dst, int N, int C, int H,
                               int W, float gscale, int dtype, void* stream) {
    GS_CHECK_ARG(src && dst && N > 0 && C > 0 && H > 0 && W > 0 && src_pix_stride >= src_coff + C,
                 "gs_nhwc_to_nchw: bad arguments");
    const int64_t total = (int64_t)N * C * H * W;
    hipStream_t s = (hipStream_t)stream;
    if (dtype == GS_F16)
        nhwc_to_nchw_kernel<GS_F16><<<ew_blocks(total), 256, 0, s>>>((const unsigned short*)src, src_pix_stride, src_coff,
                                                                     dst, N, C, (int64_t)H * W, gscale);
    else if (dtype == GS_BF16)
        nhwc_to_nchw_kernel<GS_BF16><<<ew_blocks(total), 256, 0, s>>>((const unsigned short*)src, src_pix_stride, src_coff,
                                                                      dst, N, C, (int64_t)H * W, gscale);
    else GS_CHECK_ARG(false, "gs_nhwc_to_nchw: bad dtype");
    GS_CHECK_LAUNCH("gs_nhwc_to_nchw");
    return GS_OK;
}
```

semantic_segmentation_amd/ops.py:

```python
from __future__ import annotations

import collections
import ctypes
import os
from typing import List, Optional, Sequence, Tuple

import torch

from . import _lib
from ._lib import ACT_NONE, GS_BF16, GS_F16, GsConvGeom

DTYPES = {"f16": (GS_F16, torch.float16), "bf16": (GS_BF16, torch.bfloat16)}


def dt_code(t: torch.Tensor) -> int:
    if t.dtype == torch.float16:
        return GS_F16
    if t.dtype == torch.bfloat16:
        return GS_BF16
    raise TypeError(f"expected a float16/bfloat16 tensor, got {t.dtype}")


def _p(t: Optional[torch.Tensor]):
    return None if t is None else t.data_ptr()
# ... 494 lines not shown
    if parts > 0 and grad.numel() == 4 * Cin * Cout and ws.numel() >= parts * 4 * Cin * Cout:
        ev = TIMER.start() if TIMER is not None else None
        rc = lib.gs_upconv2x2_wgrad_slabs(_p(x), _p(dy), _p(ws), N, IH, IW, Cin, x_stride, 0, Cout, OH, OW, dy_stride, dy_coff,
                                          ooy, oox, dt_code(x), _stream())
        if rc == 0:
            if ev is not None:
                TIMER.stop("igemm_wgrad", ev, 2.0 * N * IH * IW * Cin * 4 * Cout,
                           2.0 * N * IH * IW * (Cin + 4 * Cout) + 4.0 * 4 * Cin * Cout)
            _lib.call("gs_wgrad_reduce_unpack", _p(ws), parts, _p(grad), Cin, Cout, 4, 0, float(gscale), _stream())
            return
        if rc != _lib.GS_EUNSUPPORTED:
            _lib.check(rc, "gs_upconv2x2_wgrad_slabs")
    conv_wgrad_det(geom, dy, x, ws, grad, Cin, Cout, 4, gscale)


def conv_wgrad_det_batch(geoms, x, dy, ws, grad, gscale=1.0, reduce=True):
    _dev(x)
    _f32(grad, "grad")
    if x.dtype != dy.dtype:
        raise TypeError("conv_wgrad_det_batch: x and dy must share one 16-bit dtype")
    n, g0 = len(geoms), geoms[0]
    per = g0.ntaps * g0.Cout * g0.Cin
    parts = int(_lib.load().gs_conv_wgrad_parts(g0))
    if not reduce and parts <= 1:
        raise ValueError("conv_wgrad_det_batch: reduce=False needs a K split (conv_wgrad_parts > 1)")
    if reduce and (grad.numel() != n * per or not grad.is_contiguous()):
        raise ValueError("conv_wgrad_det_batch: grad must be contiguous [n][taps][Cout][Cin]")
    garr = (ctypes.POINTER(GsConvGeom) * n)(*[ctypes.pointer(g) for g in geoms])
    if parts > 1:
        _f32(ws, "ws")
        if ws.numel() < parts * n * per:
            raise ValueError("conv_wgrad_det_batch: workspace too small")
    target = grad if parts == 1 else ws
    ev = TIMER.start() if TIMER is not None else None
    _lib.call("gs_conv_wgrad_slabs_batch", n, garr, _p(x), _p(dy), _p(target), dt_code(x), _stream())
    if ev is not None:
        TIMER.stop("igemm_wgrad", ev, sum(_geom_flops(g) for g in geoms), sum(_geom_bytes(g, True) for g in geoms))
    if parts > 1 and reduce:
        _lib.call("gs_wgrad_reduce_unpack", _p(ws), parts, _p(grad), n * g0.ntaps * g0.Cout, g0.Cin, 1, 0, float(gscale), _stream())
    elif parts == 1 and gscale != 1.0:
        grad.mul_(gscale)
    return parts


def bn_partials_numel(ntiles: int, C: int) -> int:
    return int(_lib.load().gs_bn_partials_floats(ntiles, C))


def conv_smallcin_fwd(x, w, bias, y, bn_partials, k, stride, pad, act=ACT_NONE):
    _dev(x)
    _f32(x, "x"); _f32(w, "w"); _f32(bias, "bias"); _f32(bn_partials, "bn_partials")
    N, Cin, IH, IW = x.shape
    _, OH, OW, Cout = y.shape
    _lib.call("gs_conv_smallcin_fwd", _p(x), _p(w), _p(bias), _p(y), _p(bn_partials), N, Cin, IH, IW, Cout, OH, OW,
              k, stride, pad, act, dt_code(y), _stream())


def conv_smallcin_mtiles(N, OH, OW) -> int:
    return _lib.load().gs_conv_smallcin_mtiles(N, OH, OW)


def _direct_wgrad_ws(N, OH, OW, Cin, Cout, k, dev):
    n = int(_lib.load().gs_conv_direct_wgrad_ws_floats(N, OH, OW, Cin, Cout, k))
    return torch.empty(n, dtype=torch.float32, device=dev)


def conv_smallcin_wgrad(x, dy, dw, k, stride, pad, gscale):
    _f32(x, "x"); _f32(dw, "dw")
    N, Cin, IH, IW = x.shape
    _, OH, OW, Cout = dy.shape
    ws = _direct_wgrad_ws(N, OH, OW, Cin, Cout, k, x.device)
    _lib.call("gs_conv_smallcin_wgrad", _p(x), _p(dy), _p(dw), _p(ws), N, Cin, IH, IW, Cout, OH, OW, k, stride, pad,
              float(gscale), dt_code(dy), _stream())


def stem_bn_bwd_wgrad(y, dz, dz_stride, dz_coff, x, scale, shift, mean, invstd, c1, c2, act, dw, gscale) -> bool:
    _dev(y)
    _f32(x, "x"); _f32(dw, "dw")
    for n, t in (("scale", scale), ("shift", shift), ("mean", mean), ("invstd", invstd), ("c1", c1), ("c2", c2)):
        _f32(t, n)
    N, H, W, C = y.shape
    if C != 64 or tuple(x.shape) != (N, 1, H, W) or dw.numel() != 576 or y.dtype != dz.dtype:
        raise ValueError("stem_bn_bwd_wgrad: y [N,H,W,64], x [N,1,H,W], dw [64,1,3,3], one 16-bit dtype")
    if not (y.is_contiguous() and x.is_contiguous() and dw.is_contiguous()):
        raise ValueError("stem_bn_bwd_wgrad: y, x, dw must be contiguous")
    ws = _direct_wgrad_ws(N, H, W, 1, 64, 3, y.device)
    rc = _lib.load().gs_stem_bn_bwd_wgrad(_p(y), _p(dz), dz_stride, dz_coff, _p(x), _p(scale), _p(shift), _p(mean), _p(invstd),
                                          _p(c1), _p(c2), act, _p(dw), _p(ws), N, H, W, float(gscale), dt_code(y), _stream())
    if rc == _lib.GS_EUNSUPPORTED:
        return False
    if rc != 0:
        _lib.check(rc, "gs_stem_bn_bwd_wgrad")
    return True


def _stem_check(x, w, who):
    _dev(x)
    _f32(x, "x"); _f32(w, "w")
    if x.dim() != 4 or x.shape[1] != 1 or tuple(w.shape) != (64, 1, 3, 3) or not (x.is_contiguous() and w.is_contiguous()):
        raise ValueError(f"{who}: x [N,1,H,W] and w [64,1,3,3], contiguous fp32")
    return x.shape[0], x.shape[2], x.shape[3]


def stem_stats(x, w, bn_partials, tap_sums=None):
    N, H, W = _stem_check(x, w, "stem_stats")
    _f32(bn_partials, "bn_partials"); _f32(tap_sums, "tap_sums")
    mt = conv_smallcin_mtiles(N, H, W)
    if bn_partials.numel() < bn_partials_numel(mt, 64) or (tap_sums is not None and tap_sums.numel() < mt * 54):
        raise ValueError("stem_stats: bn_partials / tap_sums too small")
    _lib.call("gs_stem_stats", _p(x), _p(w), _p(bn_partials), _p(tap_sums), N, H, W, _stream())


def stem_bwd_onepass(x, z, dz, dz_stride, dz_coff, act, s1_partials, ws, z_stride=64) -> bool:
    _dev(x)
    _f32(x, "x"); _f32(s1_partials, "s1_partials"); _f32(ws, "ws")
    N, H, W = x.shape[0], x.shape[2], x.shape[3]
    nt = stem_bwd_tiles(N, H, W)
    if (x.shape[1] != 1 or not x.is_contiguous() or s1_partials.numel() < nt * 64 or ws.numel() < nt * 576
            or tuple(z.shape) != (N, H, W, z_stride) or not z.is_contiguous() or z.dtype != dz.dtype or z_stride % 8 or z_stride < 64):
        raise ValueError("stem_bwd_onepass: x [N,1,H,W], z dense [N,H,W,z_stride], buffers of stem_bwd_tiles * 64 / 576 floats")
    rc = _lib.load().gs_stem_bwd_onepass_strided(_p(x), _p(z), z_stride, _p(dz), dz_stride, dz_coff, act, _p(s1_partials), _p(ws),
                                                 N, H, W, dt_code(z), _stream())
    if rc == _lib.GS_EUNSUPPORTED:
        return False
    if rc != 0:
        _lib.check(rc, "gs_stem_bwd_onepass")
    return True


def stem_bwd_finalize(ws, s1_partials, tap_sums, w, scale, mean, invstd, train_stats, gscale, dw, dgamma, dbeta, N, H, W):
    for n, t in (("ws", ws), ("s1_partials", s1_partials), ("tap_sums", tap_sums), ("w", w), ("dw", dw), ("dgamma", dgamma),
                 ("dbeta", dbeta)):
        _f32(t, n)
    nt = stem_bwd_tiles(N, H, W)
    if (dw.numel() != 576 or ws.numel() < nt * 576 or s1_partials.numel() < nt * 64
            or (tap_sums is not None and tap_sums.numel() < conv_smallcin_mtiles(N, H, W) * 54)):
        raise ValueError("stem_bwd_finalize: buffer sizes")
    _lib.call("gs_stem_bwd_finalize", _p(ws), _p(s1_partials), _p(tap_sums), _p(w), _p(scale), _p(mean), _p(invstd),
              int(bool(train_stats)), float(gscale), _p(dw), _p(dgamma), _p(dbeta), N, H, W, _stream())


def stem_fwd_bn(x, w, scale, shift, act, z):
    N, H, W = _stem_check(x, w, "stem_fwd_bn")
    _f32(scale, "scale"); _f32(shift, "shift")
    if tuple(z.shape) != (N, H, W, 64) or not z.is_contiguous():
        raise ValueError("stem_fwd_bn: z must be dense [N,H,W,64]")
    _lib.call("gs_stem_fwd_bn", _p(x), _p(w), _p(scale), _p(shift), act, _p(z), N, H, W, dt_code(z), _stream())


def stem_fwd_bn_pair(x, w, scale, shift, act, zpair, write_lo=True):
    N, H, W = _stem_check(x, w, "stem_fwd_bn_pair")
    _f32(scale, "scale"); _f32(shift, "shift")
    if tuple(zpair.shape) != (N, H, W, 128) or not zpair.is_contiguous():
        raise ValueError("stem_fwd_bn_pair: zpair must be dense [N,H,W,128]")
    lo = zpair.data_ptr() + 64 * zpair.element_size() if write_lo else None
    _lib.call("gs_stem_fwd_bn_pair", _p(x), _p(w), _p(scale), _p(shift), act, _p(zpair), lo, 128, N, H, W, dt_code(zpair), _stream())


def stem_bwd_tiles(N, H, W) -> int:
    return int(_lib.load().gs_stem_bwd_tiles(N, H, W))


def conv_smallcin_dgrad(dy, w, dx, k, stride, pad, gscale):
    _f32(w, "w"); _f32(dx, "dx")
    N, Cin, IH, IW = dx.shape
    _, OH, OW, Cout = dy.shape
    _lib.call("gs_conv_smallcin_dgrad", _p(dy), _p(w), _p(dx), N, Cin, IH, IW, Cout, OH, OW, k, stride, pad,
              float(gscale), dt_code(dy), _stream())


def conv_smallcout_fwd(x, w, bias, y, k=1, stride=1, pad=0):
    _dev(x)
    _f32(w, "w"); _f32(bias, "bias"); _f32(y, "y")
    N, IH, IW, Cin = x.shape
    _, Cout, OH, OW = y.shape
    _lib.call("gs_conv_smallcout_fwd", _p(x), _p(w), _p(bias), _p(y), N, IH, IW, Cin, Cout, OH, OW, k, stride, pad,
              dt_code(x), _stream())


def conv_smallcout_bwd(x, w, dy, dx, dw, db, k=1, stride=1, pad=0, gscale=1.0):
    _f32(w, "w"); _f32(dy, "dy"); _f32(dw, "dw"); _f32(db, "db")
    ref = x if x is not None else dx
    N, IH, IW, Cin = ref.shape
    _, Cout, OH, OW = dy.shape
    ws = _direct_wgrad_ws(N, OH, OW, Cin, Cout, k, ref.device) if dw is not None else None
    _lib.call("gs_conv_smallcout_bwd", _p(x), _p(w), _p(dy), _p(dx), _p(dw), _p(db), _p(ws), N, IH, IW, Cin, Cout,
              OH, OW, k, stride, pad, float(gscale), dt_code(ref), _stream())


def bn_finalize(partials, ntiles, C, count, gamma, beta, running_mean, running_var, momentum, eps,
                scale, shift, mean, invstd):
    for n, t in (("gamma", gamma), ("beta", beta), ("running_mean", running_mean), ("running_var", running_var),
                 ("scale", scale), ("shift", shift), ("mean", mean), ("invstd", invstd)):
        _f32(t, n)
    _lib.call("gs_bn_finalize", _p(partials), ntiles, C, float(count), _p(gamma), _p(beta), _p(running_mean),
              _p(running_var), float(momentum), float(eps), _p(scale), _p(shift), _p(mean), _p(invstd), _stream())
    for t in (running_mean, running_var):
        if t is not None:
            torch.autograd.graph.increment_version(t)


def bn_eval_coeffs(C, gamma, beta, running_mean, running_var, eps, scale, shift, mean, invstd):
    _lib.call("gs_bn_eval_coeffs", C, _p(gamma), _p(beta), _p(running_mean), _p(running_var), float(eps),
              _p(scale), _p(shift), _p(mean), _p(invstd), _stream())


def bn_act_apply(y, scale, shift, act, z, z_stride, z_coff, zp=None, keep_mask=None, keep_scale=1.0):
    N, H, W, C = y.shape
    if not y.is_contiguous():
        raise ValueError("bn_act_apply: y must be dense NHWC")
    _lib.call("gs_bn_act_apply", _p(y), _p(scale), _p(shift), act, _p(z), z_stride, z_coff, _p(zp), _p(keep_mask),
              float(keep_scale), N, H, W, C, dt_code(y), _stream())


def bn_bwd_tiles(N, H, W) -> int:
    return _lib.load().gs_bn_bwd_tiles(N, H, W)


def bn_bwd_tiles_used(N, H, W, pooled: bool) -> int:
    return _lib.load().gs_bn_bwd_tiles_used(N, H, W, int(pooled))


def bn_act_bwd_reduce(y, dz_a, sa, ca, dzp, scale, shift, mean, invstd, act, partials, dz_b=None, act_b=ACT_NONE,
                      keep_mask=None, keep_scale=1.0):
    N, H, W, C = y.shape
    _lib.call("gs_bn_act_bwd_reduce", _p(y), _p(dz_a), sa, ca, _p(dzp), _p(dz_b), act_b, _p(keep_mask),
              float(keep_scale), _p(scale), _p(shift), _p(mean), _p(invstd), act, _p(partials), N, H, W, C,
              dt_code(y), _stream())


def bn_bwd_coeffs(partials, ntiles, C, count, gscale, dgamma, dbeta, c1, c2):
    _lib.call("gs_bn_bwd_coeffs", _p(partials), ntiles, C, float(count), float(gscale), _p(dgamma), _p(dbeta),
              _p(c1), _p(c2), _stream())


def bn_act_bwd_apply(y, dz_a, sa, ca, dzp, scale, shift, mean, invstd, c1, c2, act, bn, dy, dz_b=None,
                     act_b=ACT_NONE, keep_mask=None, keep_scale=1.0):
    N, H, W, C = y.shape
    _lib.call("gs_bn_act_bwd_apply", _p(y), _p(dz_a), sa, ca, _p(dzp), _p(dz_b), act_b, _p(keep_mask),
              float(keep_scale), _p(scale), _p(shift), _p(mean), _p(invstd), _p(c1), _p(c2), act, int(bn), _p(dy),
              N, H, W, C, dt_code(y), _stream())


def maxpool3d_fwd(z, zp, NB, D, H, W, C, z_stride=None, z_coff=0):
    _dev(z)
    _lib.call("gs_maxpool3d_fwd", _p(z), C if z_stride is None else z_stride, z_coff, _p(zp), NB, D, H, W, C,
              dt_code(z), _stream())


def maxpool2x2_fwd(z, zp, N, H, W, C, z_stride=None, z_coff=0):
    _dev(z)
    if z.dtype != zp.dtype:
        raise TypeError("maxpool2x2_fwd: z and zp must share one 16-bit dtype")
    _lib.call("gs_maxpool2x2_fwd", _p(z), C if z_stride is None else z_stride, z_coff, _p(zp), N, H, W, C,
              dt_code(z), _stream())


def maxpool2x2_fwd_pair(z_hi, z_lo, z_stride, zp_hi, zp_lo, zp_stride, N, H, W, C):
    _dev(z_hi)
    if not (z_hi.dtype == z_lo.dtype == zp_hi.dtype):
        raise TypeError("maxpool2x2_fwd_pair: the planes must share one 16-bit dtype")
    _lib.call("gs_maxpool2x2_fwd_pair", _p(z_hi), _p(z_lo), z_stride, _p(zp_hi), _p(zp_lo), zp_stride, N, H, W, C, dt_code(z_hi), _stream())


def maxpool3d_bwd(z, dzp, dres, dz, NB, D, H, W, C, z_stride=None, z_coff=0, res_stride=0, res_coff=0):
    _lib.call("gs_maxpool3d_bwd", _p(z), C if z_stride is None else z_stride, z_coff, _p(dzp), _p(dres), res_stride,
              res_coff, _p(dz), NB, D, H, W, C, dt_code(z), _stream())


def head1x1_bn_fwd(y_conv, scale, shift, act, w, bias, logits):
    _dev(y_conv)
    _f32(scale, "scale"); _f32(shift, "shift"); _f32(w, "w"); _f32(bias, "bias"); _f32(logits, "logits")
    N, H, W, C = y_conv.shape
    ncls = logits.shape[1]
    if C != 64 or tuple(logits.shape) != (N, ncls, H, W) or w.numel() != ncls * 64 or not (y_conv.is_contiguous() and logits.is_contiguous()):
        raise ValueError("head1x1_bn_fwd: y_conv [N,H,W,64], logits [N,ncls,H,W], w [ncls,64]")
    _lib.call("gs_head1x1_bn_fwd", _p(y_conv), _p(scale), _p(shift), act, _p(w), _p(bias), _p(logits), N, H, W, ncls,
              dt_code(y_conv), _stream())


def head1x1_bn_wgrad(y_conv, scale, shift, act, w, dl, dw, db, gscale=1.0):
    _dev(y_conv)
    _f32(scale, "scale"); _f32(shift, "shift"); _f32(w, "w"); _f32(dl, "dl"); _f32(dw, "dw"); _f32(db, "db")
    N, H, W, C = y_conv.shape
    ncls = dl.shape[1]
    if C != 64 or tuple(dl.shape) != (N, ncls, H, W) or dw.numel() != ncls * 64 or not (y_conv.is_contiguous() and dl.is_contiguous()):
        raise ValueError("head1x1_bn_wgrad: y_conv [N,H,W,64], dl [N,ncls,H,W], dw [ncls,64]")
    ws = _direct_wgrad_ws(N, H, W, 64, ncls, 1, y_conv.device)
    _lib.call("gs_head1x1_bn_wgrad", _p(y_conv), _p(scale), _p(shift), act, _p(w), _p(dl), _p(dw), _p(db), _p(ws), N, H, W,
              ncls, float(gscale), dt_code(y_conv), _stream())


def bn_act_bwd_reduce_head(y, dl, w_head, scale, shift, mean, invstd, act, partials):
    _dev(y)
    _f32(dl, "dl"); _f32(w_head, "w_head"); _f32(partials, "partials")
    N, H, W, C = y.shape
    ncls = dl.shape[1]
    if tuple(dl.shape) != (N, ncls, H, W) or w_head.numel() != ncls * C or not (dl.is_contiguous() and w_head.is_contiguous()):
        raise ValueError("bn_act_bwd_reduce_head: dl [N,ncls,H,W] and w_head [ncls,C] contiguous fp32")
    _lib.call("gs_bn_act_bwd_reduce_head", _p(y), _p(dl), _p(w_head), ncls, _p(scale), _p(shift), _p(mean), _p(invstd), act,
              _p(partials), N, H, W, C, dt_code(y), _stream())


def bn_act_bwd_apply_head(y, dl, w_head, scale, shift, mean, invstd, c1, c2, act, dy):
    _dev(y)
    _f32(dl, "dl"); _f32(w_head, "w_head")
    N, H, W, C = y.shape
    ncls = dl.shape[1]
    if tuple(dl.shape) != (N, ncls, H, W) or w_head.numel() != ncls * C or not (dl.is_contiguous() and w_head.is_contiguous()):
        raise ValueError("bn_act_bwd_apply_head: dl [N,ncls,H,W] and w_head [ncls,C] contiguous fp32")
    _lib.call("gs_bn_act_bwd_apply_head", _p(y), _p(dl), _p(w_head), ncls, _p(scale), _p(shift), _p(mean), _p(invstd),
              _p(c1), _p(c2), act, _p(dy), N, H, W, C, dt_code(y), _stream())


def bn_partials_colsum(partials, ntiles, Cfull, coff, C, gscale, out):
    _f32(partials, "partials"); _f32(out, "out")
    if partials.numel() < bn_partials_numel(ntiles, Cfull) or out.numel() < C:
        raise ValueError("bn_partials_colsum: buffer too small")
    _lib.call("gs_bn_partials_colsum", _p(partials), ntiles, Cfull, coff, C, float(gscale), _p(out), _stream())


def colsum(t, pix_stride, coff, N, H, W, y0, x0, h, w, C, gscale, ws, out):
    _f32(ws, "ws"); _f32(out, "out")
    if ws.numel() < 1024 * C:
        raise ValueError("colsum: workspace must hold 1024*C floats")
    _lib.call("gs_colsum", _p(t), pix_stride, coff, N, H, W, y0, x0, h, w, C, float(gscale), _p(ws), _p(out),
              dt_code(t), _stream())


def pack_weight(w, w_fwd, w_dgrad, transposed: bool):
    _dev(w)
    _f32(w, "weight")
    if transposed:
        Cin, Cout = w.shape[0], w.shape[1]
    else:
        Cout, Cin = w.shape[0], w.shape[1]
    taps = w.shape[2] * w.shape[3]
    ref = w_fwd if w_fwd is not None else w_dgrad
    _lib.call("gs_pack_weight", _p(w), _p(w_fwd), _p(w_dgrad), Cout, Cin, taps, int(transposed), dt_code(ref), _stream())


def pack_weight_multi(items):
    if not items:
        return
    descs = (_lib.GsPackDesc * len(items))()
    ref = None
    for d, (w, w_fwd, w_dgrad, transposed) in zip(descs, items):
        _dev(w)
        _f32(w, "weight")
        r = w_fwd if w_fwd is not None else w_dgrad
        if ref is None:
            ref = r
        elif r.dtype != ref.dtype:
            raise TypeError("pack_weight_multi: all packs must share one 16-bit dtype")
        cin, cout = (w.shape[0], w.shape[1]) if transposed else (w.shape[1], w.shape[0])
        d.w, d.w_fwd, d.w_dgrad = _p(w), _p(w_fwd), _p(w_dgrad)
        d.Cout, d.Cin, d.taps, d.transposed = cout, cin, w.shape[2] * w.shape[3], int(transposed)
    _lib.call("gs_pack_weight_multi", len(items), descs, dt_code(ref), _stream())


def unpack_wgrad(dw, grad, A, B, taps, transposed: bool, gscale):
    _f32(dw, "dw"); _f32(grad, "grad")
    _lib.call("gs_unpack_wgrad", _p(dw), _p(grad), A, B, taps, int(transposed), float(gscale), _stream())


def nchw_to_nhwc(src, dst, dst_stride=None, dst_coff=0):
    _f32(src, "src")
    N, C, H, W = src.shape
    _lib.call("gs_nchw_to_nhwc", _p(src), _p(dst), N, C, H, W, C if dst_stride is None else dst_stride, dst_coff,
              dt_code(dst), _stream())


def nhwc_to_nchw(src, dst, src_stride=None, src_coff=0, gscale=1.0):
    _f32(dst, "dst")
    N, C, H, W = dst.shape
    _lib.call("gs_nhwc_to_nchw", _p(src), C if src_stride is None else src_stride, src_coff, _p(dst), N, C, H, W,
              float(gscale), dt_code(src), _stream())


def upconv_merge_pack(w4, w6, w8, softmax3, pack_fwd=None, pack_dgrad=None, merged_f32=None):
    _dev(w8)
    for n, t in (("w4", w4), ("w6", w6), ("w8", w8), ("softmax3", softmax3), ("merged", merged_f32)):
        _f32(t, n)
    Cin, Cout = w8.shape[0], w8.shape[1]
    ref = pack_fwd if pack_fwd is not None else pack_dgrad
    code = dt_code(ref) if ref is not None else GS_F16
    _lib.call("gs_upconv_merge_pack", _p(w4), _p(w6), _p(w8), _p(softmax3), _p(pack_fwd), _p(pack_dgrad),
              _p(merged_f32), Cin, Cout, code, _stream())


def upconv8_image_fits(Cin: int, Cout: int) -> bool:
    return Cin % 8 == 0 and 1 <= Cout <= 4 and (144 * (Cin + 8) + 64 * Cout * Cin) * 2 <= 64 * 1024


def upconv8_image_fwd(x, pack_fwd, bias, out, u, N, h, w, Cin, Cout, act, in_stride=None, in_coff=0):
    _dev(x)
    _f32(bias, "bias"); _f32(out, "out")
    if x.dtype != pack_fwd.dtype or (u is not None and u.dtype != x.dtype):
        raise TypeError("upconv8_image_fwd: x, pack and u must share one 16-bit dtype")
    if pack_fwd.numel() != 4 * 16 * 8 * Cin or out.numel() != N * Cout * 4 * h * w:
        raise ValueError("upconv8_image_fwd: pack / output size")
    _lib.call("gs_upconv8_image_fwd", _p(x), Cin if in_stride is None else in_stride, in_coff, _p(pack_fwd), 8, _p(bias),
              _p(out), _p(u), N, h, w, Cin, Cout, act, dt_code(x), _stream())


def upconv8_image_wgrad_ok(Cin, Cout) -> bool:
    return bool(_lib.load().gs_upconv8_image_wgrad_ok(int(Cin), int(Cout)))


def upconv8_image_wgrad(x, du, dwm, N, h, w, Cin):
    _dev(x)
    _f32(dwm, "dwm")
    if x.dtype != du.dtype or x.dim() != 4 or du.dim() != 4 or tuple(x.shape[:3]) != (N, h, w) or tuple(du.shape[:3]) != (N, 2 * h, 2 * w):
        raise ValueError("upconv8_image_wgrad: x [N,h,w,C] and du [N,2h,2w,cpad] of one 16-bit dtype")
    if not (x.is_contiguous() and du.is_contiguous()) or dwm.numel() != 64 * Cin or not dwm.is_contiguous():
        raise ValueError("upconv8_image_wgrad: dense x / du, dwm [4][16][1][Cin]")
    ws = torch.empty(int(_lib.load().gs_upconv8_image_wgrad_ws_floats(N, h, w, Cin)), dtype=torch.float32, device=x.device)
    _lib.call("gs_upconv8_image_wgrad", _p(x), x.shape[3], _p(du), du.shape[3], _p(ws), _p(dwm), N, h, w, Cin, dt_code(x), _stream())


def upconv_split_wgrad_parts_ok(Cin, Cout) -> bool:
    return bool(_lib.load().gs_upconv_split_wgrad_parts_ok(int(Cin), int(Cout)))


def upconv_split_wgrad(dwm, w4, w6, w8, softmax3, gscale, dw4, dw6, dw8, dots3, nparts=1):
    for n, t in (("dwm", dwm), ("dw4", dw4), ("dw6", dw6), ("dw8", dw8), ("dots3", dots3)):
        _f32(t, n)
    Cin, Cout = w8.shape[0], w8.shape[1]
    ws = torch.empty(int(_lib.load().gs_upconv_split_wgrad_ws_floats(Cin, Cout)), dtype=torch.float32, device=dwm.device)
    if nparts > 1:
        if dwm.numel() < nparts * 64 * Cin * Cout:
            raise ValueError("upconv_split_wgrad: the slab stack is too small")
        _lib.call("gs_upconv_split_wgrad_parts", _p(dwm), int(nparts), 64 * Cin * Cout, _p(w4), _p(w6), _p(w8), _p(softmax3),
                  float(gscale), _p(dw4), _p(dw6), _p(dw8), _p(dots3), _p(ws), Cin, Cout, _stream())
        return
    _lib.call("gs_upconv_split_wgrad_det", _p(dwm), _p(w4), _p(w6), _p(w8), _p(softmax3), float(gscale), _p(dw4), _p(dw6),
              _p(dw8), _p(dots3), _p(ws), Cin, Cout, _stream())


def fake_postprocess(x, out, gamma_lut):
    _dev(x)
    _f32(x, "x"); _f32(out, "out"); _f32(gamma_lut, "gamma_lut")
    if not x.is_contiguous() or out.shape != x.shape or gamma_lut.numel() != 256:
        raise ValueError("fake_postprocess: contiguous x, out of the same shape and a 256-entry gamma table")
    N = x.shape[0] * (x.shape[1] if x.dim() == 4 else 1)
    hw = x.numel() // N
    ws = torch.empty(int(_lib.load().gs_fake_postprocess_ws_floats(N)), dtype=torch.float32, device=x.device)
    _lib.call("gs_fake_postprocess", _p(x), _p(out), _p(ws), _p(gamma_lut), N, hw, _stream())


def isic_fake_trans(x, out, equalize_on, bits, sharpness_on, sharpness_factor, autocontrast_on, saturation_factor):
    _dev(x)
    _f32(x, "x"); _f32(out, "out")
    if x.dim() != 4 or not x.is_contiguous() or out.shape != x.shape or not out.is_contiguous():
        raise ValueError("isic_fake_trans: contiguous x, out [N,C,H,W] of one shape")
    N, C, H, W = x.shape
    ws = torch.empty(int(_lib.load().gs_isic_fake_trans_ws_bytes(N * C, H * W)), dtype=torch.uint8, device=x.device)
    sat_on = saturation_factor is not None and C == 3
    sr = float(saturation_factor) if sat_on else 1.0
    _lib.call("gs_isic_fake_trans", _p(x), _p(out), _p(ws), N, C, H, W, int(bool(equalize_on)), int(bits),
              int(bool(sharpness_on)), float(sharpness_factor), float(1.0 - float(sharpness_factor)), int(bool(autocontrast_on)),
              int(sat_on), sr, float(1.0 - sr), _stream())


LOSS_WS = 4 * 1024


def seg_loss_fwd(logits, mask_u8, ws, out):
    _dev(logits)
    _f32(logits, "logits"); _f32(ws, "ws"); _f32(out, "out")
    if mask_u8.dtype != torch.uint8 or not mask_u8.is_contiguous():
        raise TypeError("mask must be contiguous uint8 [N,H,W]")
    N, C, H, W = logits.shape
    if mask_u8.numel() != N * H * W:
        raise ValueError("mask / logits shape mismatch")
    _lib.call("gs_seg_loss_fwd", _p(logits), _p(mask_u8), N, C, H, W, _p(ws), _p(out), _stream())


def seg_loss_bwd(logits, mask_u8, out, gout, gscale, dlogits):
    N, C, H, W = logits.shape
    _f32(dlogits, "dlogits"); _f32(gout, "gout")
    _lib.call("gs_seg_loss_bwd", _p(logits), _p(mask_u8), _p(out), _p(gout), float(gscale), _p(dlogits), N, C, H, W,
              _stream())


def dice_loss_fwd(p, t, ws, out):
    _dev(p)
    _f32(p, "input"); _f32(t, "target")
    _lib.call("gs_dice_loss_fwd", _p(p), _p(t), p.numel(), _p(ws), _p(out), _stream())


def dice_loss_bwd(t, out, gout, dp):
    _lib.call("gs_dice_loss_bwd", _p(t), _p(out), _p(gout), _p(dp), t.numel(), _stream())


def dice_coeff_batched(p, t, out):
    _dev(p)
    _f32(p, "p"); _f32(t, "t"); _f32(out, "out")
    B, n_per = p.shape
    if t.shape != p.shape or out.numel() < 1 + B:
        raise ValueError("dice_coeff_batched: p, t must be [B, n] of one shape and out hold 1 + B floats")
    ws = torch.empty(int(_lib.load().gs_dice_batched_ws_floats(B)), dtype=torch.float32, device=p.device)
    _lib.call("gs_dice_coeff_batched", _p(p), _p(t), B, n_per, _p(ws), _p(out), _stream())


def eval_dice(logits, mask_u8, out):
    _dev(logits)
    _f32(logits, "logits"); _f32(out, "out")
    N, C, H, W = logits.shape
    if mask_u8.dtype != torch.uint8 or not mask_u8.is_contiguous() or mask_u8.numel() != N * H * W:
        raise TypeError("eval_dice: mask must be contiguous uint8 [N,H,W]")
    B = N * max(1, C - 1)
    if out.numel() < 1 + B:
        raise ValueError("eval_dice: out must hold 1 + N*max(1,C-1) floats")
    ws = torch.empty(int(_lib.load().gs_dice_batched_ws_floats(B)), dtype=torch.float32, device=logits.device)
    _lib.call("gs_eval_dice", _p(logits), _p(mask_u8), N, C, H * W, _p(ws), _p(out), _stream())


def jaccard_seg_loss_fwd(logits, mask_u8, out):
    _dev(logits)
    _f32(logits, "logits"); _f32(out, "out")
    N, C, H, W = logits.shape
    if C != 1:
        raise ValueError("the Jaccard loss of train_end2end_isic.py is the one-class form")
    if mask_u8.dtype != torch.uint8 or not mask_u8.is_contiguous() or mask_u8.numel() != N * H * W:
        raise TypeError("mask must be contiguous uint8 [N,H,W]")
    if out.numel() < int(_lib.load().gs_jaccard_loss_out_floats(N)):
        raise ValueError("jaccard_seg_loss_fwd: out too small")
    ws = torch.empty(int(_lib.load().gs_dice_batched_ws_floats(N)), dtype=torch.float32, device=logits.device)
    _lib.call("gs_jaccard_seg_loss_fwd", _p(logits), _p(mask_u8), N, H * W, _p(ws), _p(out), _stream())


def jaccard_seg_loss_bwd(logits, mask_u8, out, gout, gscale, dlogits):
    _f32(gout, "gout"); _f32(dlogits, "dlogits")
    N, C, H, W = logits.shape
    _lib.call("gs_jaccard_seg_loss_bwd", _p(logits), _p(mask_u8), _p(out), _p(gout), float(gscale), _p(dlogits), N, H * W,
              _stream())


def eval_jaccard(logits, mask_u8, out):
    _dev(logits)
    _f32(logits, "logits"); _f32(out, "out")
    N, C, H, W = logits.shape
    if C != 1 or mask_u8.dtype != torch.uint8 or not mask_u8.is_contiguous() or mask_u8.numel() != N * H * W or out.numel() < 1 + N:
        raise ValueError("eval_jaccard: one-class logits, contiguous uint8 mask [N,H,W], out of 1 + N floats")
    ws = torch.empty(int(_lib.load().gs_dice_batched_ws_floats(N)), dtype=torch.float32, device=logits.device)
    _lib.call("gs_eval_jaccard", _p(logits), _p(mask_u8), N, H * W, _p(ws), _p(out), _stream())


def mean_loss_fwd(x, t, cval, mode, ws, out):
    _dev(x)
    _f32(x, "x"); _f32(t, "target")
    _lib.call("gs_mean_loss_fwd", _p(x), _p(t), float(cval), mode, x.numel(), _p(ws), _p(out), _stream())


def mean_loss_bwd(x, t, cval, mode, gout, gscale, dx):
    _lib.call("gs_mean_loss_bwd", _p(x), _p(t), float(cval), mode, x.numel(), _p(gout), float(gscale), _p(dx), _stream())


def pack_weight_split(w, pack, transposed: bool):
    _dev(w)
    _f32(w, "w")
    taps = w.shape[2] * w.shape[3]
    cin, cout = (w.shape[0], w.shape[1]) if transposed else (w.shape[1], w.shape[0])
    if pack.numel() != taps * cout * 3 * cin or not pack.is_contiguous():
        raise ValueError("pack_weight_split: pack must be contiguous [taps][Cout][3*Cin]")
    _lib.call("gs_pack_weight_split", _p(w), _p(pack), cout, cin, taps, 1 if transposed else 0, dt_code(pack), _stream())


def conv3x3_precise(x, w, y_hi, y_lo, N, H, W, Cin, Cout, in_stride, in_coff=0, out_stride=None, out_coff=0,
                    bias=None, bn_partials=None, act=ACT_NONE, taps=TAPS3_FWD):
    _dev(x)
    _f32(bias, "bias"); _f32(bn_partials, "bn_partials")
    if not (x.dtype == w.dtype == y_hi.dtype == y_lo.dtype):
        raise TypeError("conv3x3_precise: x, w, y must share one 16-bit dtype")
    if Cin % 64 != 0 or w.numel() != 9 * Cout * 3 * Cin:
        raise ValueError("conv3x3_precise: Cin must be a multiple of 64 and w the [9][Cout][3*Cin] split pack")
    if bn_partials is not None and bn_partials.numel() < bn_partials_numel(conv3x3_stat_rows(N, H, W, Cin, Cout, pair=True), Cout):
        raise ValueError("conv3x3_precise: bn_partials too small")
    dy, dx = _tap_arrays(taps)
    ev = TIMER.start() if TIMER is not None else None
    _lib.call("gs_conv3x3_precise", _p(x), _p(w), _p(y_hi), _p(y_lo), _p(bias), _p(bn_partials), N, H, W, 3 * Cin,
              in_stride, in_coff, 2 * Cin, Cout, Cout if out_stride is None else out_stride, out_coff, dy, dx, act,
              dt_code(x), _stream())
    if ev is not None:
        TIMER.stop("conv3x3_halo_precise", ev, 2.0 * N * H * W * Cout * 9 * Cin,
                   2.0 * (N * H * W * 2 * (Cin + Cout) + 9 * 3 * Cin * Cout))


def upconv2x2_fwd_precise(x, w, bias, y_hi, y_lo, N, IH, IW, Cin, Cout, OH, OW, in_stride, in_coff=0, out_stride=None,
                          out_coff=0, ooy=0, oox=0):
    _dev(x)
    _f32(bias, "bias")
    if not (x.dtype == w.dtype == y_hi.dtype == y_lo.dtype):
        raise TypeError("upconv2x2_fwd_precise: x, w, y must share one 16-bit dtype")
    if w.numel() != 4 * Cout * 3 * Cin:
        raise ValueError("upconv2x2_fwd_precise: w must be the [4][Cout][3*Cin] split pack")
    ev = TIMER.start() if TIMER is not None else None
    _lib.call("gs_upconv2x2_fwd_precise", _p(x), _p(w), _p(bias), _p(y_hi), _p(y_lo), N, IH, IW, 3 * Cin, in_stride,
              in_coff, 2 * Cin, Cout, OH, OW, Cout if out_stride is None else out_stride, out_coff, ooy, oox,
              dt_code(x), _stream())
    if ev is not None:
        TIMER.stop("igemm_fwd_precise", ev, 2.0 * N * IH * IW * Cin * 4 * Cout,
                   2.0 * (N * IH * IW * 2 * (Cin + 4 * Cout) + 4 * 3 * Cin * Cout))


def pack_weight_segs(items):
    if not items:
        return
    descs = (_lib.GsSegPackDesc * len(items))()
    ref = items[0][1]
    for d, (w, pack, transposed, segs) in zip(descs, items):
        _dev(w)
        _f32(w, "weight")
        if pack.dtype != ref.dtype:
# ... 284 lines not shown
```

semantic_segmentation_amd/unet/unet_engine.py:

```python
from __future__ import annotations

import functools
import math
import os
import warnings
from typing import Callable, Dict, List, Optional

import torch

from .. import ops
from .._lib import ACT_NONE, ACT_RELU

_TORCH_DT = {"f16": torch.float16, "bf16": torch.bfloat16}
FOLD_BN_INFERENCE = os.environ.get("GSSEG_FOLD_BN", "1") != "0"
WGRAD_SIDE_STREAM = os.environ.get("GSSEG_WGRAD_STREAM", "0") != "0"
FUSED_STEM_BWD = os.environ.get("GSSEG_STEM_BWD_FUSED", "1") != "0"
FUSED_STEM_FWD = os.environ.get("GSSEG_STEM_FWD_FUSED", "1") != "0"
FUSED_HEAD_FWD = os.environ.get("GSSEG_HEAD_FWD_FUSED", "1") != "0"
FUSED_HEAD_BWD = os.environ.get("GSSEG_HEAD_BWD_FUSED", "1") != "0"
FUSED_UP_BIAS_GRAD = os.environ.get("GSSEG_UP_BIAS_FUSED", "1") != "0"


class _ConvRec:
    __slots__ = ("name", "wkey", "bnkey", "inp", "inp_is_image", "y", "coef", "geom", "cin", "cout", "h", "w",
# ... 601 lines not shown
                ops.bn_eval_coeffs(cout, gamma.detach(), beta.detach(), rm, bufs[bnkey + ".running_var"], bn_mod.eps,
                                   coef[0], coef[1], coef[2], coef[3])
            return coef

        def stage(prefix, idx, inp, cin, cout, h, w, zbuf, z_stride, want_lo, zp=None, zp_want_lo=False, image=False,
                  lo_len=None, to_head=False):
            short = prefix.replace(".maxpool_conv.1", "") + f".{idx}"
            wkey, bnkey = f"{prefix}.double_conv.{idx}.weight", f"{prefix}.double_conv.{idx + 1}"
            wparam = params[wkey]
            rm = bufs.get(bnkey + ".running_mean")
            batch_stats = training or rm is None
            rec = _ConvRec()
            rec.name, rec.wkey, rec.bnkey = f"{prefix}.{idx}", wkey, bnkey
            wide_img = image and cin > 4
            rec.cin, rec.cout, rec.h, rec.w, rec.inp_is_image = cin, cout, h, w, image and not wide_img
            rec.inp, rec.train_stats, rec.geom, rec.z, rec.tap_sums = inp, batch_stats, None, None, None
            rec.inp_stride = None if image else 2 * cin
            ntiles = ops.conv_widecin_mtiles(N, h, w) if wide_img else ops.conv_smallcin_mtiles(N, h, w) if image else (
                ops.conv3x3_stat_rows(N, h, w, 2 * cin, cout, pair="q") if plan[short] == "q" else ops.conv3x3_stat_rows(N, h, w, cin, cout, pair=True))
            partials = empty(ops.bn_partials_numel(ntiles, cout), dtype=torch.float32) if batch_stats else None
            want_lo, zp_want_lo = int(want_lo), int(zp_want_lo)
            z_lo = zbuf[..., z_stride // 2:] if (zbuf is not None and want_lo) else None
            if (image and not full and FUSED_STEM_FWD and cin == 1 and cout == 64 and zp is None and z_stride == 2 * cout
                    and inp.is_contiguous()):
                wst = wparam.detach().contiguous()
                if need_grad:
                    rec.tap_sums = (empty(ntiles * 54, dtype=torch.float32) if batch_stats
                                    else torch.zeros(ntiles * 54, dtype=torch.float32, device=dev))
                if batch_stats:
                    ops.stem_stats(inp, wst, partials, rec.tap_sums)
                coef = bn_coef(bnkey, partials, ntiles, cout, N * h * w, batch_stats)
                if want_lo == 2:
                    ops.stem_fwd_bn_pair_q8(inp, wst, coef[0], coef[1], ACT_RELU, zbuf)
                else:
                    ops.stem_fwd_bn_pair(inp, wst, coef[0], coef[1], ACT_RELU, zbuf, write_lo=bool(want_lo))
                rec.y, rec.coef, rec.z, rec.wd = None, coef, zbuf, None
                if need_grad:
                    recs.append(rec)
                return rec
            if fold and not image and not batch_stats:
                _, fpack, fbias = self._packs[wkey + "|fsegs"]
                _, K, wrap = _segs(plan[short], cin, lo_len)
                if to_head:
                    zd = empty(2, N, h, w, cout)
                    ops.conv3x3_segs(inp, fpack, zd[0], zd[1], N, h, w, K, wrap, cin, cout, in_stride=2 * cin, bias=fbias, act=ACT_RELU)
                    return zd
                ops.conv3x3_segs(inp, fpack, zbuf, zbuf[..., z_stride // 2:], N, h, w, K, wrap, cin, cout, in_stride=2 * cin,
                                 out_stride=z_stride, out_coff=0, bias=fbias, act=ACT_RELU)
                if zp is not None:
                    ops.maxpool2x2_fwd_pair(zbuf, zbuf[..., z_stride // 2:], z_stride, zp, zp[..., zp.shape[3] // 2:], zp.shape[3],
                                            N, h, w, cout)
                return None
            y_hi, y_lo = empty(N, h, w, cout), empty(N, h, w, cout)
            if wide_img:
                ops.conv_widecin_fwd_split(inp, wparam.detach().contiguous(), y_hi, y_lo, partials)
                if need_grad:
                    cpad = (cin + 7) // 8 * 8
                    xin = (torch.zeros if cpad != cin else torch.empty)((N, h, w, cpad), dtype=tdt, device=dev)
                    ops.nchw_to_nhwc(inp, xin, dst_stride=cpad)
                    rec.inp, rec.cin, rec.wide = xin, cpad, cin
            elif image:
                ops.conv_smallcin_fwd_split(inp, wparam.detach().contiguous(), y_hi, y_lo, partials, 3, 1)
            elif plan[short] == "q":
                qpack, wexp = self._seg_pack(wkey)
                ops.conv3x3_q8(inp, qpack, wexp, y_hi, y_lo, N, h, w, cin, cout, in_stride=2 * cin, bn_partials=partials)
            else:
                _, K, wrap = _segs(plan[short], cin, lo_len)
                ops.conv3x3_segs(inp, self._seg_pack(wkey), y_hi, y_lo, N, h, w, K, wrap, cin, cout, in_stride=2 * cin,
                                 bn_partials=partials)
            coef = bn_coef(bnkey, partials, ntiles, cout, N * h * w, batch_stats)
            rec.y, rec.coef = y_hi, coef
            if wide_img:
                rec.wd = self._packed_padded(wkey, wparam, rec.cin, True)[1] if need_grad else None
            else:
                rec.wd = None if image else (self._packed(wkey, wparam, False, True, need_fwd=False)[1] if need_grad else None)
            if need_grad:
                recs.append(rec)
            if to_head:
                return rec, y_lo
            zp_hi = zp if zp is not None else None
            zp_lo = zp[..., zp.shape[3] // 2:] if (zp is not None and zp_want_lo) else None
            if want_lo == 2 or zp_want_lo == 2:
                ops.bn_act_apply_split_q8(y_hi, y_lo, coef[0], coef[1], ACT_RELU, zbuf, z_lo, want_lo == 2, z_stride, 0, zp_hi, zp_lo,
                                          zp_want_lo == 2, 0 if zp is None else zp.shape[3])
            else:
                ops.bn_act_apply_split(y_hi, y_lo, coef[0], coef[1], ACT_RELU, zbuf, z_lo, z_stride, 0, zp_hi, zp_lo,
                                       0 if zp is None else zp.shape[3])
            return rec

        def reads_lo(st):
            return 2 if plan[st] == "q" else (1 if "x" in plan[st] else 0)

        cats = [None] * 4
        for i in range(4):
            zero_needed = (hs[i] - 2 * hs[i + 1]) or (ws_[i] - 2 * ws_[i + 1])
            alloc = torch.zeros if zero_needed else torch.empty
            cats[i] = alloc((N, hs[i], ws_[i], 4 * C[i]), dtype=tdt, device=dev)
        inp, cin = x, net.n_channels
        for i in range(5):
            prefix = "inc" if i == 0 else f"down{i}.maxpool_conv.1"
            blk = "inc" if i == 0 else f"down{i}"
            h, w = hs[i], ws_[i]
            zmid = empty(N, h, w, 2 * C[i])
            stage(prefix, 0, inp, cin, C[i], h, w, zmid, 2 * C[i], reads_lo(blk + ".3"), image=(i == 0))
            if i < 4:
                pooled = empty(N, hs[i + 1], ws_[i + 1], 2 * C[i])
                stage(prefix, 3, zmid, C[i], C[i], h, w, cats[i], 4 * C[i], reads_lo(f"up{4 - i}.conv.0"),
                      zp=pooled, zp_want_lo=reads_lo(f"down{i + 1}.0"))
                inp, cin = pooled, C[i]
            else:
                x5 = empty(N, h, w, 2 * C[i])
                stage(prefix, 3, zmid, C[i], C[i], h, w, x5, 2 * C[i], reads_lo("up1.up") or bilinear)
                inp = x5

        z_last = None
        for j in range(1, 5):
            lvl = 4 - j
            prefix = f"up{j}"
            cout_t = C[lvl]
            cin_t = inp.shape[3] // 2
            h, w = hs[lvl + 1], ws_[lvl + 1]
            H2, W2 = hs[lvl], ws_[lvl]
            pt, pl = (H2 - 2 * h) // 2, (W2 - 2 * w) // 2
            cat = cats[lvl]
            wkey = prefix + ".up.weight"
            up_mode = plan[prefix + ".up"]
            up_lo_valid = True
            if bilinear:
                want = reads_lo(prefix + ".conv.0")
                if want == 2:
                    raise NotImplementedError("a 'q' stage behind the bilinear up-sampling (its pair kernel writes 16-bit lo planes)")
                ops.upsample2x_bilinear_fwd_pair(inp, inp[..., cin_t:], cat, cat[..., 2 * cout_t:] if want else None, N, h, w,
                                                 cin_t, H2, W2, in_stride=2 * cin_t, out_stride=4 * cout_t, out_coff=cout_t,
                                                 ooy=pt, oox=pl)
                up_lo_valid = want
            elif up_mode == "1" and not full:
                wf, _ = self._packed(wkey, params[wkey], True, need_grad)
                ops.upconv2x2_fwd(inp, wf, params[prefix + ".up.bias"].detach(), cat, N, 1, h, w, cin_t, cout_t, 1, H2, W2,
                                  in_stride=2 * cin_t, out_stride=4 * cout_t, out_coff=cout_t, ooy=pt, oox=pl)
                up_lo_valid = False
                if reads_lo(prefix + ".conv.0") == 2:
                    ops.q8_from_hi(cat, cat[..., 2 * cout_t:], N * H2 * W2, cout_t, 4 * cout_t, cout_t)
            else:
                if reads_lo(prefix + ".conv.0") == 2:
                    raise NotImplementedError("a 'q' stage behind a pair transposed conv (it writes 16-bit lo planes)")
                _, K, wrap = _segs(up_mode, cin_t)
                ops.upconv2x2_fwd_segs(inp, self._seg_pack(wkey), params[prefix + ".up.bias"].detach(),
                                       cat[..., cout_t:], cat[..., 3 * cout_t:], N, h, w, K, wrap, cin_t, cout_t, H2, W2,
                                       in_stride=2 * cin_t, out_stride=4 * cout_t, ooy=pt, oox=pl)
            if need_grad:
                u = _UpRec()
                u.name, u.zin, u.cat = prefix, inp, cat
                u.cin, u.cout, u.h, u.w, u.H2, u.W2, u.pt, u.pl = cin_t, cout_t, h, w, H2, W2, pt, pl
                u.wd = u.geom_bwd = u.geom_wg = None
                if not bilinear:
                    u.wd = self._packed(wkey, params[wkey], True, True)[1]
                    taps = [(py + pt, px + pl) for py in range(2) for px in range(2)]
                    u.geom_bwd = ops.make_geom(N, H2, W2, cout_t, h, w, cin_t, h, w, taps, isy=2, isx=2,
                                               in_stride=2 * cout_t, in_coff=cout_t)
                    u.geom_wg = ops.make_geom(N, H2, W2, cout_t, h, w, cin_t, h, w, taps, isy=2, isx=2,
                                              in_stride=2 * cout_t, in_coff=cout_t, out_stride=2 * cin_t)
                ups.append(u)
            cmid = params[prefix + ".conv.double_conv.0.weight"].shape[0]
            cout3 = params[prefix + ".conv.double_conv.3.weight"].shape[0]
            zmid = empty(N, H2, W2, 2 * cmid)
            stage(prefix + ".conv", 0, cat, 2 * cout_t, cmid, H2, W2, zmid, 2 * cmid, reads_lo(prefix + ".conv.3"),
                  lo_len=None if up_lo_valid else cout_t)
            if j < 4:
                zout = empty(N, H2, W2, 2 * cout3)
                nxt_lo = True if bilinear else reads_lo(f"up{j + 1}.up")
                stage(prefix + ".conv", 3, zmid, cmid, cout3, H2, W2, zout, 2 * cout3, nxt_lo)
                inp = zout
            elif fold:
                zl = stage(prefix + ".conv", 3, zmid, cmid, cout3, H2, W2, None, 0, False, to_head=True)
                zl_hi, zl_lo = zl[0], zl[1]
                last_rec = None
                z_last = zl_hi
            elif not full and FUSED_HEAD_FWD and cout3 == 64 and net.n_classes <= 4:
                last_rec, y_lo_last = stage(prefix + ".conv", 3, zmid, cmid, cout3, H2, W2, None, 0, False, to_head=True)
            else:
                zl = empty(2, N, H2, W2, cout3)
                zl_hi, zl_lo = zl[0], zl[1]
                last_rec = None
                st_rec = stage(prefix + ".conv", 3, zmid, cmid, cout3, H2, W2, None, 0, False, to_head=True)
                ops.bn_act_apply_split(st_rec[0].y, st_rec[1], st_rec[0].coef[0], st_rec[0].coef[1], ACT_RELU, zl_hi, zl_lo,
                                       cout3, 0)
                z_last = zl_hi

        logits = empty(N, net.n_classes, H, W, dtype=torch.float32)
        if z_last is None:
            ops.head1x1_bn_fwd_split(last_rec.y, y_lo_last, last_rec.coef[0], last_rec.coef[1], ACT_RELU,
                                     params["outc.conv.weight"].detach().contiguous(), params["outc.conv.bias"].detach(), logits)
        else:
            ops.head1x1_fwd_split(zl_hi, zl_lo, params["outc.conv.weight"].detach().contiguous(),
                                  params["outc.conv.bias"].detach(), logits)
        if nbt_pending:
            torch._foreach_add_(nbt_pending, 1)
        ctx = None
        if need_grad:
            ctx = dict(recs=recs, ups=ups, x=x, z_last=z_last, N=N, H=H, W=W, hs=hs, ws=ws_, C=C, training=training)
        return logits, ctx

    def backward(self, ctx, params: Dict[str, torch.Tensor], dlogits: torch.Tensor, need_dx: bool):
        net, tdt = self.net, self.tdt
        N, H, W, hs, ws_, C = ctx["N"], ctx["H"], ctx["W"], ctx["hs"], ctx["ws"], ctx["C"]
        dev = dlogits.device
        if self.dynamic_loss_scale and self.grad_ready_hook is not None:
            raise RuntimeError("dynamic_loss_scale is not supported together with the bucketed GradReducer")
        recs: Dict[str, _ConvRec] = {r.name: r for r in ctx["recs"]}
        ups: Dict[str, _UpRec] = {u.name: u for u in ctx["ups"]}
        S = float(2 ** round(math.log2(N * H * W)))
        inv_s = 1.0 / S
        renorm = None
        if self.dynamic_loss_scale:
            amax = dlogits.detach().abs().amax().float()
            k = torch.floor(-torch.log2(torch.clamp(amax * S, min=1e-30)))
            renorm = torch.exp2(torch.clamp(k, -60.0, 60.0))
            dlogits = dlogits * renorm
        grads: Dict[str, torch.Tensor] = {}

        def empty(*shape, dtype=tdt):
            return torch.empty(shape, dtype=dtype, device=dev)

        def emit(name, g):
            grads[name] = g
            if self.grad_ready_hook is not None:
                self.grad_ready_hook(name, g)

        main_stream = torch.cuda.current_stream(dev)
        side = self._side_stream(dev) if WGRAD_SIDE_STREAM else None
        deferred = []

        def flush_deferred(upto_all: bool):
            while deferred and (upto_all or len(deferred) > 1):
                name, g, ev = deferred.pop(0)
                main_stream.wait_event(ev)
                emit(name, g)

        def on_side(inputs, fn, name, g):
            if side is None:
                fn()
                emit(name, g)
                return
            ev = torch.cuda.Event()
            ev.record(main_stream)
            for t_ in inputs:
                t_.record_stream(side)
            with torch.cuda.stream(side):
                side.wait_event(ev)
                fn()
                if self.grad_ready_hook is not None:
                    done = torch.cuda.Event()
                    done.record(side)
                    deferred.append((name, g, done))
            if self.grad_ready_hook is None:
                grads[name] = g
            else:
                flush_deferred(False)

        def galloc(name, like, zero=False):
            if self.grad_alloc is not None:
                g = self.grad_alloc(name, like)
                if zero:
                    g.zero_()
                return g
            return (torch.zeros_like if zero else torch.empty_like)(like, memory_format=torch.contiguous_format)

        det_min = 8 if os.environ.get("GSSEG_WGRAD_DET", "1") == "0" else 1
        det_recs = set()
        wg_need, tot_w = 1, 0
        for r in ctx["recs"]:
            wnum = params[r.wkey].numel()
            if (not r.inp_is_image and ops.USE_HALO_CONV and r.cin % 8 == 0 and r.cout % 8 == 0 and
                    ops.conv3x3_wgrad_parts(N, r.h, r.w, r.cin, r.cout) >= det_min):
                det_recs.add(r.name)
                wg_need = max(wg_need, ops.conv3x3_wgrad_ws_floats(N, r.h, r.w, r.cin, r.cout))
            elif not r.inp_is_image:
                tot_w += wnum
        for u in ctx["ups"]:
            if u.geom_bwd is not None:
                wg_need = max(wg_need, ops.conv_wgrad_ws_floats(u.geom_wg if u.geom_wg is not None else u.geom_bwd),
                              ops.upconv2x2_wgrad_ws_floats(N, u.h, u.w, u.cin, u.cout))
        dw_arena = torch.zeros(max(tot_w, 1), dtype=torch.float32, device=dev)
        wg_ws = empty(wg_need, dtype=torch.float32)
        arena_off = [0]

        def dw_take(numel):
            a = arena_off[0]
            arena_off[0] = a + numel
            return dw_arena[a:a + numel]
        npart = 0
        for i in range(5):
            npart = max(npart, ops.bn_partials_numel(ops.bn_bwd_tiles(N, hs[i], ws_[i]), C[i]))
            if i == 0:
                npart = max(npart, ops.bn_partials_numel(ops.stem_bwd_tiles(N, hs[i], ws_[i]), 64))
            if i < 4 and ops.USE_HALO_CONV:
                npart = max(npart, ops.bn_partials_numel(ops.conv3x3_mtiles(N, hs[i], ws_[i], 2 * C[i]), 2 * C[i]))
                if N * hs[i] * ws_[i] <= 8192:
                    npart = max(npart, ops.bn_partials_numel(-(-(N * hs[i] * ws_[i]) // 16), 2 * C[i]))
        partials = empty(npart, dtype=torch.float32)
        col_ws = empty(1024 * 1024, dtype=torch.float32)

        z_last = ctx["z_last"]
        dl = (dlogits.contiguous().float() * S)
        wout = params["outc.conv.weight"]
        dwo = galloc("outc.conv.weight", wout, zero=True)
        dbo = galloc("outc.conv.bias", params["outc.conv.bias"], zero=True)
        head_src = None
        wout_c = wout.detach().contiguous()
        rlast = recs["up4.conv.3"]
        if z_last is None:
            ops.head1x1_bn_wgrad(rlast.y, rlast.coef[0], rlast.coef[1], ACT_RELU, wout_c, dl, dwo, dbo, gscale=inv_s)
        if FUSED_HEAD_BWD and wout.shape[0] <= 4 and dl.is_contiguous():
            head_src = (dl, wout_c)
            dz = None
            if z_last is not None:
                ops.conv_smallcout_bwd(z_last, wout_c, dl, None, dwo, dbo, gscale=inv_s)
        elif 4 < wout.shape[0] <= 64:
            dz = empty(N, H, W, 64)
            ops.head1x1_wide_bwd(z_last, wout_c.reshape(wout.shape[0], 64), dl, dz, dwo, dbo, gscale=inv_s)
        elif wout.shape[0] > 64:
            dzs = torch.zeros((N, H, W, 64), dtype=torch.float32, device=dev)
            for g0 in range(0, wout.shape[0], 4):
                g1 = min(g0 + 4, wout.shape[0])
                dzg = empty(N, H, W, 64)
                ops.conv_smallcout_bwd(z_last, wout_c[g0:g1].contiguous(), dl[:, g0:g1].contiguous(), dzg, dwo[g0:g1], dbo[g0:g1],
                                       gscale=inv_s)
                dzs += dzg
            dz = dzs.to(tdt)
        else:
            dz = empty(N, H, W, 64)
            if z_last is not None:
                ops.conv_smallcout_bwd(z_last, wout_c, dl, dz, dwo, dbo, gscale=inv_s)
            else:
                ops.conv_smallcout_bwd(None, wout_c, dl, dz, None, None)
        emit("outc.conv.weight", dwo)
        emit("outc.conv.bias", dbo)

        def conv_stage_bwd(rec: _ConvRec, dz_a, sa, ca, dzp, need_dinp: bool, colsum=None, head=None):
            h, w, cin, cout = rec.h, rec.w, rec.cin, rec.cout
            coef = rec.coef
            pooled = dzp is not None
            if rec.y is None:
                wst = params[rec.wkey].detach().contiguous()
                done = False
                if not need_dinp and not pooled and head is None:
                    nts = ops.stem_bwd_tiles(N, h, w)
                    sws = empty(nts * 576, dtype=torch.float32)
                    s1p = empty(nts * 64, dtype=torch.float32)
                    if ops.stem_bwd_onepass(rec.inp, rec.z, dz_a, sa, ca, ACT_RELU, s1p, sws, z_stride=rec.z.shape[3]):
                        dgamma = galloc(rec.bnkey + ".weight", params[rec.bnkey + ".weight"])
                        dbeta = galloc(rec.bnkey + ".bias", params[rec.bnkey + ".bias"])
                        dw = galloc(rec.wkey, params[rec.wkey], zero=True)
                        ops.stem_bwd_finalize(sws, s1p, rec.tap_sums, wst, coef[0], coef[2], coef[3], rec.train_stats, inv_s,
                                              dw, dgamma, dbeta, N, h, w)
                        emit(rec.wkey, dw)
                        emit(rec.bnkey + ".weight", dgamma)
                        emit(rec.bnkey + ".bias", dbeta)
                        done = True
                if done:
                    return None
                y_re = empty(N, h, w, cout)
                ops.conv_smallcin_fwd(rec.inp, wst, None, y_re, None, 3, 1, 1)
                rec.y = y_re
            ntiles = ops.bn_bwd_tiles_used(N, h, w, pooled)
            if head is not None:
                ops.bn_act_bwd_reduce_head(rec.y, head[0], head[1], coef[0], coef[1], coef[2], coef[3], ACT_RELU, partials)
            else:
                ops.bn_act_bwd_reduce(rec.y, dz_a, sa, ca, dzp, coef[0], coef[1], coef[2], coef[3], ACT_RELU, partials)
            dgamma = galloc(rec.bnkey + ".weight", params[rec.bnkey + ".weight"])
            dbeta = galloc(rec.bnkey + ".bias", params[rec.bnkey + ".bias"])
            c12 = empty(2, cout, dtype=torch.float32)
            ops.bn_bwd_coeffs(partials, ntiles, cout, N * h * w, inv_s, dgamma, dbeta, c12[0], c12[1])
            if not rec.train_stats:
                c12.zero_()
            wparam = params[rec.wkey]
            dw_stem = None
            if (rec.inp_is_image and not need_dinp and not pooled and FUSED_STEM_BWD and cin == 1 and cout == 64
                    and rec.inp.is_contiguous()):
                dw_stem = galloc(rec.wkey, wparam, zero=True)
                if ops.stem_bn_bwd_wgrad(rec.y, dz_a, sa, ca, rec.inp, coef[0], coef[1], coef[2], coef[3], c12[0], c12[1],
                                         ACT_RELU, dw_stem, inv_s):
                    emit(rec.wkey, dw_stem)
                    emit(rec.bnkey + ".weight", dgamma)
                    emit(rec.bnkey + ".bias", dbeta)
                    return None
            dy = empty(N, h, w, cout)
            if head is not None:
                ops.bn_act_bwd_apply_head(rec.y, head[0], head[1], coef[0], coef[1], coef[2], coef[3], c12[0], c12[1], ACT_RELU, dy)
            else:
                ops.bn_act_bwd_apply(rec.y, dz_a, sa, ca, dzp, coef[0], coef[1], coef[2], coef[3], c12[0], c12[1],
                                     ACT_RELU, True, dy)
            dinp = None
            if rec.inp_is_image:
                dw = dw_stem if dw_stem is not None else galloc(rec.wkey, wparam, zero=True)
                ops.conv_smallcin_wgrad(rec.inp, dy, dw, 3, 1, 1, inv_s)
                if need_dinp:
                    dinp = torch.empty_like(rec.inp)
                    ops.conv_smallcin_dgrad(dy, wparam.detach().contiguous(), dinp, 3, 1, 1, inv_s)
            elif getattr(rec, "wide", 0):
                dwp = torch.empty((cout, cin, 3, 3), dtype=torch.float32, device=dev)
                ops.conv3x3_wgrad_det(rec.inp, dy, wg_ws, dwp, N, h, w, cin, cout, inv_s)
                dw = galloc(rec.wkey, wparam)
                dw.copy_(dwp[:, :rec.wide])
                wgrad_on_side = False
                if need_dinp:
                    dxp = empty(N, h, w, cin)
                    ops.conv3x3(dy, rec.wd, dxp, N, h, w, cout, cin, ops.TAPS3_DGRAD)
                    dfull = torch.empty((N, cin, h, w), dtype=torch.float32, device=dev)
                    ops.nhwc_to_nchw(dxp, dfull, gscale=inv_s)
                    dinp = dfull[:, :rec.wide].contiguous()
            else:
                dw = galloc(rec.wkey, wparam)
                wgrad_on_side = rec.name in det_recs
                if wgrad_on_side:
                    on_side((rec.inp, dy, wg_ws, dw),
                            lambda: ops.conv3x3_wgrad_det(rec.inp, dy, wg_ws, dw, N, h, w, cin, cout, inv_s, in_stride=rec.inp_stride),
                            rec.wkey, dw)
                else:
                    dwp = dw_take(wparam.numel())
                    if ops.USE_HALO_CONV and cin % 8 == 0 and cout % 8 == 0:
                        ops.conv3x3_wgrad(rec.inp, dy, dwp, N, h, w, cin, cout, in_stride=rec.inp_stride)
                    else:
                        ops.conv_wgrad(rec.geom, rec.inp, dy, dwp)
                    ops.unpack_wgrad(dwp, dw, cout, cin, 9, False, inv_s)
                if need_dinp:
                    dinp = empty(N, h, w, cin)
                    if ops.USE_HALO_CONV and rec.inp_stride is None and rec.train_stats and stream_conv(N, h, w, cout, cin):
                        gd = ops.geom_conv_dgrad_s1(N, h, w, cin, cout, 3, 1)
                        if colsum is not None:
                            ops.conv_igemm(gd, dy, rec.wd, dinp, None, partials)
                            ops.bn_partials_colsum(partials, ops.conv_igemm_mtiles(gd), cin, colsum[0], colsum[1], inv_s, colsum[2])
                        else:
                            ops.conv_igemm(gd, dy, rec.wd, dinp)
                    elif ops.USE_HALO_CONV and colsum is not None:
                        ops.conv3x3(dy, rec.wd, dinp, N, h, w, cout, cin, ops.TAPS3_DGRAD, bn_partials=partials)
                        ops.bn_partials_colsum(partials, ops.conv3x3_stat_rows(N, h, w, cout, cin), cin, colsum[0], colsum[1], inv_s, colsum[2])
                    elif ops.USE_HALO_CONV:
                        ops.conv3x3(dy, rec.wd, dinp, N, h, w, cout, cin, ops.TAPS3_DGRAD)
                    else:
                        ops.conv_igemm(ops.geom_conv_dgrad_s1(N, h, w, cin, cout, 3, 1), dy, rec.wd, dinp)
            if rec.inp_is_image or not wgrad_on_side:
                emit(rec.wkey, dw)
            emit(rec.bnkey + ".weight", dgamma)
            emit(rec.bnkey + ".bias", dbeta)
            return dinp

        dcats = [None] * 4
        for j in range(4, 0, -1):
            lvl = 4 - j
            prefix = f"up{j}"
            cout_t = C[lvl]
            r3, r0 = recs[prefix + ".conv.3"], recs[prefix + ".conv.0"]
            dmid = conv_stage_bwd(r3, dz, r3.cout, 0, None, True, head=head_src if j == 4 else None)
            u = ups[prefix]
            db_fused = None
            if (u.geom_bwd is not None and ops.USE_HALO_CONV and FUSED_UP_BIAS_GRAD and u.pt == 0 and u.pl == 0
                    and 2 * u.h == u.H2 and 2 * u.w == u.W2):
                db_fused = galloc(prefix + ".up.bias", params[prefix + ".up.bias"])
            dcat = conv_stage_bwd(r0, dmid, r0.cout, 0, None, True,
                                  colsum=None if db_fused is None else (cout_t, cout_t, db_fused))
            dcats[lvl] = dcat
            if u.geom_bwd is None:
                dz = empty(N, u.h, u.w, u.cin)
                ops.upsample2x_bilinear_bwd(dcat, dz, N, u.h, u.w, u.cin, u.H2, u.W2, dy_stride=2 * cout_t,
                                            dy_coff=cout_t, ooy=u.pt, oox=u.pl)
                continue
            wkey = prefix + ".up.weight"
            wparam = params[wkey]
            if db_fused is not None:
                db = db_fused
            else:
                db = galloc(prefix + ".up.bias", params[prefix + ".up.bias"])
                ops.colsum(dcat, 2 * cout_t, cout_t, N, u.H2, u.W2, u.pt, u.pl, 2 * u.h, 2 * u.w, cout_t, inv_s, col_ws, db)
            dw = galloc(wkey, wparam)
            on_side((dcat, u.zin, wg_ws, dw),
                    lambda u=u, dcat=dcat, dw=dw: ops.upconv2x2_wgrad_det(
                        u.geom_wg if u.geom_wg is not None else u.geom_bwd, u.zin, dcat, wg_ws, dw, N, u.h, u.w, u.cin, u.cout,
                        u.H2, u.W2, u.zin.shape[3], 2 * u.cout, u.cout, u.pt, u.pl, inv_s),
                    wkey, dw)
            dz = empty(N, u.h, u.w, u.cin)
            ops.upconv2x2_dgrad(u.geom_bwd, dcat, u.wd, dz, N, u.h, u.w, u.cin, u.cout, u.H2, u.W2, 2 * cout_t, cout_t, u.pt, u.pl)
            emit(prefix + ".up.bias", db)

        dx = None
        dpool = None
        for i in range(4, -1, -1):
            prefix = "inc" if i == 0 else f"down{i}.maxpool_conv.1"
            if i == 4:
                dmid = conv_stage_bwd(recs[prefix + ".3"], dz, C[i], 0, None, True)
            else:
                dmid = conv_stage_bwd(recs[prefix + ".3"], dcats[i], 2 * C[i], 0, dpool, True)
            r0 = recs[prefix + ".0"]
            dinp = conv_stage_bwd(r0, dmid, C[i], 0, None, (i > 0) or need_dx)
            if i > 0:
                dpool = dinp
            else:
                dx = dinp
        if side is not None:
            flush_deferred(True)
            main_stream.wait_stream(side)
        if renorm is not None:
            inv_r = torch.reciprocal(renorm)
            torch._foreach_mul_(list(grads.values()), inv_r)
            if dx is not None:
                dx = dx * inv_r
        if self.after_backward is not None:
            self.after_backward()
        return grads, dx


class _UNetFunction(torch.autograd.Function):

    @staticmethod
    def forward(ctx, engine: UNetEngine, names, training: bool, need_grad: bool, x, *plist):
        params = dict(zip(names, plist))
        logits, ectx = engine.forward(x, params, training, need_grad)
        ctx.engine, ctx.names, ctx.ectx, ctx.plist = engine, names, ectx, plist
        ctx.x_needs_grad = x.requires_grad
        return logits

    @staticmethod
    def backward(ctx, dlogits):
        if ctx.ectx is None:
            raise RuntimeError("UNet forward ran without gradient tracking")
        params = dict(zip(ctx.names, ctx.plist))
        grads, dx = ctx.engine.backward(ctx.ectx, params, dlogits, ctx.x_needs_grad)
        fetch, alias = ctx.engine.grad_fetch, ctx.engine.grad_alloc is not None
        out = [(fetch(n) if fetch is not None else (grads[n].clone() if alias else grads[n])) if (p.requires_grad and n in grads)
               else None for n, p in zip(ctx.names, ctx.plist)]
        if ctx.engine.accumulate_grads and fetch is None and not alias:
            have, new = [], []
            for i, p in enumerate(ctx.plist):
                if out[i] is not None and p.grad is not None and p.grad.shape == out[i].shape and p.grad.dtype == out[i].dtype:
                    have.append(p.grad)
                    new.append(out[i])
                    out[i] = None
            if have:
                torch._foreach_add_(have, new)
        return (None, None, None, None, dx if ctx.x_needs_grad else None, *out)


def run_unet(engine: UNetEngine, x: torch.Tensor) -> torch.Tensor:
    items = engine.param_items()
    names = tuple(n for n, _ in items)
    plist = tuple(p for _, p in items)
    need_grad = torch.is_grad_enabled() and (x.requires_grad or any(p.requires_grad for p in plist))
    return _UNetFunction.apply(engine, names, engine.net.training, need_grad, x, *plist)
```

Before: 2094 images/sec.

## Fuse head 1x1 weight gradient into BN backward reduce; tile weight packing

The output head's 1x1 conv weight and bias gradients are now accumulated inside the BN-act backward reduce pass, which already reads the last-layer activations and logits gradient. A small finish kernel then sums the per-tile partials in double precision. This removes the separate head wgrad pass over the 64-channel full-resolution activation. The loss-scale multiply is folded into the kernels instead of materialising a scaled dl tensor. Separately, weight packing now goes through an LDS-tiled transpose that writes both forward and dgrad layouts from one tile read, replacing a strided per-row kernel launched twice. The cost is extra registers in the reduce kernel and a new launch.

```diff
diff --git a/include/gsseg.h b/include/gsseg.h
--- a/include/gsseg.h
+++ b/include/gsseg.h
@@ -7,7 +7,7 @@
 extern "C" {
 #endif
 
-#define GS_ABI_VERSION 52
+#define GS_ABI_VERSION 53
 
 enum GsDtype { GS_F16 = 0, GS_BF16 = 1 };
 enum GsStatus { GS_OK = 0, GS_EINVAL = -1, GS_ELAUNCH = -2, GS_EUNSUPPORTED = -3 };
@@ -153,7 +153,12 @@
                               int H, int W, int C, int dtype, void* stream);
 int gs_bn_act_bwd_apply_head(const void* y, const float* dl, const float* w_head, int ncls, const float* scale,
                              const float* shift, const float* mean, const float* invstd, const float* c1, const float* c2,
-                             int act, void* dy, int N, int H, int W, int C, int dtype, void* stream);
+                             int act, float dl_scale, void* dy, int N, int H, int W, int C, int dtype, void* stream);
+int64_t gs_bn_head_wgrad_ws_floats(int N, int H, int W, int ncls);
+int gs_bn_act_bwd_reduce_head_wgrad(const void* y, const float* dl, float dl_scale, const float* w_head, int ncls,
+                                    const float* scale, const float* shift, const float* mean, const float* invstd, int act,
+                                    float* partials, float* dw, float* db, float* ws, float gscale, int N, int H, int W, int C,
+                                    int dtype, void* stream);
 
 int gs_bn_partials_colsum(const float* partials, int ntiles, int Cfull, int coff, int C, float gscale, float* out,
                           void* stream);
diff --git a/semantic_segmentation_amd/_lib.py b/semantic_segmentation_amd/_lib.py
--- a/semantic_segmentation_amd/_lib.py
+++ b/semantic_segmentation_amd/_lib.py
@@ -12,7 +12,7 @@
 GS_F16, GS_BF16 = 0, 1
 ACT_NONE, ACT_RELU, ACT_LEAKY02, ACT_TANH = 0, 1, 2, 3
 GS_MAX_TAPS = 64
-ABI_VERSION = 52
+ABI_VERSION = 53
 
 
 class GsConvGeom(ctypes.Structure):
@@ -118,7 +118,10 @@
     "gs_head1x1_bn_fwd": (c_int, [_P, _F, _F, c_int, _F, _F, _F] + [c_int] * 5 + [c_void_p]),
     "gs_head1x1_bn_wgrad": (c_int, [_P, _F, _F, c_int, _F, _F, _F, _F, _F] + [c_int] * 4 + [c_float, c_int, c_void_p]),
     "gs_bn_act_bwd_reduce_head": (c_int, [_P, _F, _F, c_int, _F, _F, _F, _F, c_int, _F] + [c_int] * 5 + [c_void_p]),
-    "gs_bn_act_bwd_apply_head": (c_int, [_P, _F, _F, c_int, _F, _F, _F, _F, _F, _F, c_int, _P] + [c_int] * 5 + [c_void_p]),
+    "gs_bn_act_bwd_apply_head": (c_int, [_P, _F, _F, c_int, _F, _F, _F, _F, _F, _F, c_int, c_float, _P] + [c_int] * 5 + [c_void_p]),
+    "gs_bn_head_wgrad_ws_floats": (c_int64, [c_int] * 4),
+    "gs_bn_act_bwd_reduce_head_wgrad": (c_int, [_P, _F, c_float, _F, c_int, _F, _F, _F, _F, c_int, _F, _F, _F, _F, c_float]
+                                        + [c_int] * 5 + [c_void_p]),
     "gs_bn_partials_colsum": (c_int, [_F, c_int, c_int, c_int, c_int, c_float, _F, c_void_p]),
     "gs_pack_weight": (c_int, [_F, _P, _P, c_int, c_int, c_int, c_int, c_int, c_void_p]),
     "gs_pack_weight_multi": (c_int, [c_int, POINTER(GsPackDesc), c_int, c_void_p]),
diff --git a/semantic_segmentation_amd/csrc/bn.hip b/semantic_segmentation_amd/csrc/bn.hip
--- a/semantic_segmentation_amd/csrc/bn.hip
+++ b/semantic_segmentation_amd/csrc/bn.hip
@@ -209,11 +209,14 @@
     const float* head_dl;
     const float* head_w;
     int head_n;
+    float head_dl_scale;
+    float* head_wg;
 };
 
-template <int DT, bool POOL, bool APPLY, bool GENERIC, int HEAD = 0, bool EXTRA = true, bool RN = false>
+template <int DT, bool POOL, bool APPLY, bool GENERIC, int HEAD = 0, bool EXTRA = true, bool RN = false, bool WG = false>
 __global__ __launch_bounds__(256) void bn_act_bwd_kernel(const BwdArgs a) {
     static_assert(!HEAD || (!POOL && !GENERIC), "the head source: plain pixels, slope-family activation");
+    static_assert(!WG || (HEAD && !APPLY), "the head's weight gradient rides on the reduce pass of the head source");
     static_assert(!(RN && GENERIC), "the rounded slope product belongs to the slope family");
     auto mul_g = [&](float g, float d) __attribute__((always_inline)) { return RN ? mul_rn(g, d) : g * d; };
     constexpr int NH = HEAD ? HEAD : 1;
@@ -254,6 +257,15 @@
         float s1[8], s2[8];
 #pragma unroll
         for (int i = 0; i < 8; ++i) { s1[i] = 0.f; s2[i] = 0.f; }
+        float wacc[WG ? NH : 1][8], bacc[WG ? NH : 1];
+        if (WG) {
+#pragma unroll
+            for (int q = 0; q < NH; ++q) {
+                bacc[q] = 0.f;
+#pragma unroll
+                for (int i = 0; i < 8; ++i) wacc[q][i] = 0.f;
+            }
+        }
         float hw[NH][8];
         if (HEAD) {
 #pragma unroll
@@ -273,7 +285,8 @@
                 for (int i = threadIdx.x; i < ce - cb; i += 256) {
                     const int p = cb + i, n = p / HWp, hwp = p - n * HWp;
 #pragma unroll
-                    for (int q = 0; q < NH; ++q) hdl[q * HEAD_CHUNK + i] = q < a.head_n ? a.head_dl[((int64_t)n * a.head_n + q) * HWp + hwp] : 0.f;
+                    for (int q = 0; q < NH; ++q)
+                        hdl[q * HEAD_CHUNK + i] = q < a.head_n ? a.head_dl[((int64_t)n * a.head_n + q) * HWp + hwp] * a.head_dl_scale : 0.f;
                 }
                 __syncthreads();
             }
@@ -328,6 +341,15 @@
                         const float xh = (yv[i] - mu[i]) * is[i];
                         if (APPLY) out[i] = a.bn ? sc[i] * (gh - k1[i] - xh * k2[i]) : gh;
                         else { s1[i] += gh; s2[i] += gh * xh; }
+                        if (WG) {
+                            const float z = fwd_a(v);
+#pragma unroll
+                            for (int q = 0; q < NH; ++q) wacc[q][i] += hd[k][q] * z;
+                        }
+                    }
+                    if (WG) {
+#pragma unroll
+                        for (int q = 0; q < NH; ++q) bacc[q] += hd[k][q];
                     }
                     if (APPLY) st16(a.dy + pix * a.C + c0, pack8<DT>(out));
                 }
@@ -413,6 +435,65 @@
                 a.partials[(int64_t)tile * 2 * a.C + st * a.C + (ch - chl + cl) * 8 + i] = tsum;
             }
         }
+        if (WG) {
+            float* row = a.head_wg + (int64_t)tile * (a.head_n * 65);
+#pragma unroll
+            for (int q = 0; q < NH; ++q) {
+                if (q < a.head_n) {
+                    __syncthreads();
+#pragma unroll
+                    for (int i = 0; i < 8; ++i) red[0][threadIdx.x][i] = wacc[q][i];
+                    __syncthreads();
+                    if (threadIdx.x < 64) {
+                        const int ci = threadIdx.x;
+                        float t = 0.f;
+                        for (int k = 0; k < unit_lanes; ++k) t += red[0][k * lanes_per_unit + (ci >> 3)][ci & 7];
+                        row[q * 64 + ci] = t;
+                    }
+                }
+            }
+            __syncthreads();
+#pragma unroll
+            for (int q = 0; q < NH; ++q) red[1][threadIdx.x][q] = bacc[q];
+            __syncthreads();
+            if ((int)threadIdx.x < a.head_n) {
+                float t = 0.f;
+                for (int k = 0; k < unit_lanes; ++k) t += red[1][k * lanes_per_unit][threadIdx.x];
+                row[a.head_n * 64 + threadIdx.x] = t;
+            }
+        }
+    }
+}
+
+__global__ __launch_bounds__(256) void head_wgrad_finish_kernel(const float* __restrict__ ws, int nb, int stride, int ndw, int ndb,
+                                                                float gscale, float* dw, float* db) {
+    __shared__ double red[8][32];
+    const int jl = threadIdx.x & 31, bl = threadIdx.x >> 5;
+    const int j = blockIdx.x * 32 + jl;
+    const bool live = j < ndw + ndb;
+    double s = 0.0;
+    if (live) {
+        double acc[8] = {0, 0, 0, 0, 0, 0, 0, 0};
+        int b = bl;
+        for (; b + 56 < nb; b += 64) {
+            float v[8];
+#pragma unroll
+            for (int u = 0; u < 8; ++u) v[u] = ws[(int64_t)(b + 8 * u) * stride + j];
+#pragma unroll
+            for (int u = 0; u < 8; ++u) acc[u] += (double)v[u];
+        }
+        for (; b < nb; b += 8) acc[0] += (double)ws[(int64_t)b * stride + j];
+        s = ((acc[0] + acc[1]) + (acc[2] + acc[3])) + ((acc[4] + acc[5]) + (acc[6] + acc[7]));
+    }
+    red[bl][jl] = s;
+    __syncthreads();
+    if (bl == 0 && live) {
+        double t = 0.0;
+#pragma unroll
+        for (int i = 0; i < 8; ++i) t += red[i][jl];
+        const float o = (float)(t * gscale);
+        if (j < ndw) dw[j] += o;
+        else if (db != nullptr) db[j - ndw] += o;
     }
 }
 
@@ -657,6 +738,8 @@
 #define LAUNCH_HEAD(DT, NC, R)                                                                          \
     do {                                                                                                \
         if (apply) bn_act_bwd_kernel<DT, false, true, false, NC, false, R><<<ntiles, 256, 0, s>>>(a);   \
+        else if (a.head_wg != nullptr)                                                                  \
+            bn_act_bwd_kernel<DT, false, false, false, NC, false, R, true><<<ntiles, 256, 0, s>>>(a);   \
         else bn_act_bwd_kernel<DT, false, false, false, NC, false, R><<<ntiles, 256, 0, s>>>(a);        \
     } while (0)
 #define LAUNCH_HEAD_N(DT, R) do { if (a.head_n <= 2) LAUNCH_HEAD(DT, 2, R); else LAUNCH_HEAD(DT, 4, R); } while (0)
@@ -741,7 +824,7 @@
     return GS_OK;
 }
 
-static int bn_head_args(const char* who, BwdArgs& a, const void* y, const float* dl, const float* w_head, int ncls,
+static int bn_head_args(const char* who, BwdArgs& a, const void* y, const float* dl, float dl_scale, const float* w_head, int ncls,
                         const float* scale, const float* shift, const float* mean, const float* invstd, int act, int N, int H,
                         int W, int C, int dtype) {
     GS_CHECK_ARG(y && dl && w_head && ncls >= 1 && ncls <= 4 && N > 0 && H > 0 && W > 0 && C > 0 && C % 8 == 0 && C <= 2048,
@@ -750,7 +833,7 @@
     GS_CHECK_ARG((int64_t)N * H * W < 2147483647LL, "%s: more than 2^31 pixels", who);
     GS_CHECK_ARG(act == GS_ACT_NONE || act == GS_ACT_RELU || act == GS_ACT_LEAKY02, "%s: activation %d not supported", who, act);
     GS_CHECK_ARG(scale && shift && mean && invstd, "%s: needs the BatchNorm coefficients", who);
-    a.y = (const unsigned short*)y; a.head_dl = dl; a.head_w = w_head; a.head_n = ncls;
+    a.y = (const unsigned short*)y; a.head_dl = dl; a.head_w = w_head; a.head_n = ncls; a.head_dl_scale = dl_scale;
     a.scale = scale; a.shift = shift; a.mean = mean; a.invstd = invstd; a.act = act; a.bn = 1;
     a.N = N; a.H = H; a.W = W; a.C = C;
     return GS_OK;
@@ -760,7 +843,7 @@
                                          const float* shift, const float* mean, const float* invstd, int act, float* partials,
                                          int N, int H, int W, int C, int dtype, void* stream) {
     BwdArgs a{};
-    int rc = bn_head_args("gs_bn_act_bwd_reduce_head", a, y, dl, w_head, ncls, scale, shift, mean, invstd, act, N, H, W, C, dtype);
+    int rc = bn_head_args("gs_bn_act_bwd_reduce_head", a, y, dl, 1.f, w_head, ncls, scale, shift, mean, invstd, act, N, H, W, C, dtype);
     if (rc) return rc;
     GS_CHECK_ARG(partials != nullptr, "gs_bn_act_bwd_reduce_head: null partials");
     a.partials = partials;
@@ -769,11 +852,37 @@
     return GS_OK;
 }
 
+extern "C" int64_t gs_bn_head_wgrad_ws_floats(int N, int H, int W, int ncls) {
+    if (N <= 0 || H <= 0 || W <= 0 || ncls < 1 || ncls > 4) return 0;
+    return (int64_t)gs_bn_bwd_tiles_used(N, H, W, 0) * ncls * 65;
+}
+
+extern "C" int gs_bn_act_bwd_reduce_head_wgrad(const void* y, const float* dl, float dl_scale, const float* w_head, int ncls,
+                                               const float* scale, const float* shift, const float* mean, const float* invstd,
+                                               int act, float* partials, float* dw, float* db, float* ws, float gscale, int N,
+                                               int H, int W, int C, int dtype, void* stream) {
+    BwdArgs a{};
+    int rc = bn_head_args("gs_bn_act_bwd_reduce_head_wgrad", a, y, dl, dl_scale, w_head, ncls, scale, shift, mean, invstd, act, N, H,
+                          W, C, dtype);
+    if (rc) return rc;
+    GS_CHECK_ARG(partials && dw && ws, "gs_bn_act_bwd_reduce_head_wgrad: null pointer");
+    GS_CHECK_ARG(C == 64, "gs_bn_act_bwd_reduce_head_wgrad: C=%d, the pointwise head reads 64 channels", C);
+    a.partials = partials; a.head_wg = ws;
+    int ntiles = 0;
+    launch_bwd(a, false, dtype, (hipStream_t)stream, &ntiles);
+    GS_CHECK_LAUNCH("gs_bn_act_bwd_reduce_head_wgrad");
+    const int ndw = ncls * 64, ndb = ncls;
+    head_wgrad_finish_kernel<<<cdiv(ndw + ndb, 32), 256, 0, (hipStream_t)stream>>>(ws, ntiles, ncls * 65, ndw, ndb, gscale, dw, db);
+    GS_CHECK_LAUNCH("gs_bn_act_bwd_reduce_head_wgrad");
+    return GS_OK;
+}
+
 extern "C" int gs_bn_act_bwd_apply_head(const void* y, const float* dl, const float* w_head, int ncls, const float* scale,
                                         const float* shift, const float* mean, const float* invstd, const float* c1,
-                                        const float* c2, int act, void* dy, int N, int H, int W, int C, int dtype, void* stream) {
+                                        const float* c2, int act, float dl_scale, void* dy, int N, int H, int W, int C, int dtype,
+                                        void* stream) {
     BwdArgs a{};
-    int rc = bn_head_args("gs_bn_act_bwd_apply_head", a, y, dl, w_head, ncls, scale, shift, mean, invstd, act, N, H, W, C, dtype);
+    int rc = bn_head_args("gs_bn_act_bwd_apply_head", a, y, dl, dl_scale, w_head, ncls, scale, shift, mean, invstd, act, N, H, W, C, dtype);
     if (rc) return rc;
     GS_CHECK_ARG(dy && c1 && c2, "gs_bn_act_bwd_apply_head: null pointer");
     a.c1 = c1; a.c2 = c2; a.dy = (unsigned short*)dy;
diff --git a/semantic_segmentation_amd/csrc/pack.hip b/semantic_segmentation_amd/csrc/pack.hip
--- a/semantic_segmentation_amd/csrc/pack.hip
+++ b/semantic_segmentation_amd/csrc/pack.hip
@@ -47,35 +47,97 @@
     int n;
 };
 
+template <int T> struct PackTile { static constexpr int TA = 64, TB = 32; };
+template <> struct PackTile<27> { static constexpr int TA = 32, TB = 16; };
+template <int T> struct PackSm {
+    static constexpr int ROW = PackTile<T>::TB + 2, PLANE = PackTile<T>::TA * ROW + 2, ELEMS = T * PLANE;
+};
+constexpr int PACK_SM_ELEMS = PackSm<9>::ELEMS > PackSm<27>::ELEMS ? PackSm<9>::ELEMS : PackSm<27>::ELEMS;
+static_assert(PackSm<4>::ELEMS <= PACK_SM_ELEMS && PackSm<8>::ELEMS <= PACK_SM_ELEMS, "pack tile LDS");
+
+inline int pack_tiles(int A, int B, int T) {
+    const int ta = T == 27 ? PackTile<27>::TA : PackTile<9>::TA, tb = T == 27 ? PackTile<27>::TB : PackTile<9>::TB;
+    return cdiv(A, ta) * cdiv(B, tb);
+}
+
 template <int DT, int T>
-__device__ __forceinline__ void pack_rows_body(const float* __restrict__ w, unsigned short* dst, int A, int B, bool ba,
-                                               int block, int nblocks) {
+__device__ __forceinline__ void pack_tile_body(const float* __restrict__ w, unsigned short* p_ab, unsigned short* p_ba, int A,
+                                               int B, int tile, unsigned short* sm) {
+    constexpr int TA = PackTile<T>::TA, TB = PackTile<T>::TB, ROW = PackSm<T>::ROW, PLANE = PackSm<T>::PLANE;
+    constexpr int NQ = TB * T / 4 + 2;
+    const int tiles_b = (B + TB - 1) / TB;
+    const int a0 = (tile / tiles_b) * TA, b0 = (tile % tiles_b) * TB;
+    const int na = min(TA, A - a0), nb = min(TB, B - b0);
+    const int64_t total = (int64_t)A * B * T;
+    const int off = (int)(((uintptr_t)w >> 2) & 3);
+    const int len = nb * T;
+#pragma unroll 4
+    for (int it = threadIdx.x; it < TA * NQ; it += 256) {
+        const int al = it / NQ, q = it - al * NQ;
+        if (al >= na) break;
+        const int64_t s = ((int64_t)(a0 + al) * B + b0) * T;
+        const int64_t i0 = ((s + off) & ~(int64_t)3) - off + 4 * q;
+        if (i0 >= s + len) continue;
+        float v[4];
+        if (i0 >= 0 && i0 + 3 < total) {
+            const float4 f = *reinterpret_cast<const float4*>(w + i0);
+            v[0] = f.x; v[1] = f.y; v[2] = f.z; v[3] = f.w;
+        } else {
+#pragma unroll
+            for (int k = 0; k < 4; ++k) v[k] = (i0 + k >= 0 && i0 + k < total) ? w[i0 + k] : 0.f;
+        }
+#pragma unroll
+        for (int k = 0; k < 4; ++k) {
+            const int e = (int)(i0 + k - s);
+            if (e >= 0 && e < len) sm[(e % T) * PLANE + al * ROW + e / T] = Elem<DT>::from_f(v[k]);
+        }
+    }
+    __syncthreads();
     const int64_t n = (int64_t)A * B;
-    for (int64_t i = (int64_t)block * 256 + threadIdx.x; i < n; i += (int64_t)nblocks * 256) {
-        int a, b;
-        if (!ba) { b = (int)(i % B); a = (int)(i / B); }
-        else { a = (int)(i % A); b = (int)(i / A); }
-        const float* src = w + ((int64_t)a * B + b) * T;
-        float v[T];
-#pragma unroll
-        for (int t = 0; t < T; ++t) v[t] = src[t];
-#pragma unroll
-        for (int t = 0; t < T; ++t) dst[(int64_t)t * n + i] = Elem<DT>::from_f(v[t]);
+    if (p_ab != nullptr) {
+        if ((B & 1) == 0 && (((uintptr_t)p_ab) & 3) == 0) {
+            for (int it = threadIdx.x; it < T * TA * (TB / 2); it += 256) {
+                const int k = it % (TB / 2), al = (it / (TB / 2)) % TA, t = it / (TB / 2 * TA);
+                if (al < na && 2 * k < nb)
+                    *reinterpret_cast<unsigned int*>(p_ab + (int64_t)t * n + (int64_t)(a0 + al) * B + b0 + 2 * k) =
+                        *reinterpret_cast<const unsigned int*>(sm + t * PLANE + al * ROW + 2 * k);
+            }
+        } else {
+            for (int it = threadIdx.x; it < T * TA * TB; it += 256) {
+                const int bl = it % TB, al = (it / TB) % TA, t = it / (TB * TA);
+                if (al < na && bl < nb) p_ab[(int64_t)t * n + (int64_t)(a0 + al) * B + b0 + bl] = sm[t * PLANE + al * ROW + bl];
+            }
+        }
+    }
+    if (p_ba != nullptr) {
+        if ((A & 1) == 0 && (((uintptr_t)p_ba) & 3) == 0) {
+            for (int it = threadIdx.x; it < T * TB * (TA / 2); it += 256) {
+                const int k = it % (TA / 2), bl = (it / (TA / 2)) % TB, t = it / (TA / 2 * TB);
+                if (bl < nb && 2 * k < na) {
+                    const unsigned short* c = sm + t * PLANE + 2 * k * ROW + bl;
+                    *reinterpret_cast<unsigned int*>(p_ba + (int64_t)t * n + (int64_t)(b0 + bl) * A + a0 + 2 * k) =
+                        (unsigned int)c[0] | ((unsigned int)c[ROW] << 16);
+                }
+            }
+        } else {
+            for (int it = threadIdx.x; it < T * TB * TA; it += 256) {
+                const int al = it % TA, bl = (it / TA) % TB, t = it / (TA * TB);
+                if (al < na && bl < nb) p_ba[(int64_t)t * n + (int64_t)(b0 + bl) * A + a0 + al] = sm[t * PLANE + al * ROW + bl];
+            }
+        }
     }
 }
 
 template <int DT>
 __global__ __launch_bounds__(256) void pack_weight_multi_kernel(const PackMultiArgs a) {
+    __shared__ __attribute__((aligned(16))) unsigned short sm[PACK_SM_ELEMS];
     int d = 0;
     while (d + 1 < a.n && (int)blockIdx.x >= a.first[d + 1]) ++d;
-    const bool ba = blockIdx.y == 1;
-    unsigned short* dst = ba ? a.p_ba[d] : a.p_ab[d];
-    if (dst == nullptr) return;
-    const int block = blockIdx.x - a.first[d], nblocks = a.first[d + 1] - a.first[d];
-    if (a.T[d] == 9) pack_rows_body<DT, 9>(a.w[d], dst, a.A[d], a.B[d], ba, block, nblocks);
-    else if (a.T[d] == 27) pack_rows_body<DT, 27>(a.w[d], dst, a.A[d], a.B[d], ba, block, nblocks);
-    else if (a.T[d] == 8) pack_rows_body<DT, 8>(a.w[d], dst, a.A[d], a.B[d], ba, block, nblocks);
-    else pack_rows_body<DT, 4>(a.w[d], dst, a.A[d], a.B[d], ba, block, nblocks);
+    const int tile = blockIdx.x - a.first[d];
+    if (a.T[d] == 9) pack_tile_body<DT, 9>(a.w[d], a.p_ab[d], a.p_ba[d], a.A[d], a.B[d], tile, sm);
+    else if (a.T[d] == 27) pack_tile_body<DT, 27>(a.w[d], a.p_ab[d], a.p_ba[d], a.A[d], a.B[d], tile, sm);
+    else if (a.T[d] == 8) pack_tile_body<DT, 8>(a.w[d], a.p_ab[d], a.p_ba[d], a.A[d], a.B[d], tile, sm);
+    else pack_tile_body<DT, 4>(a.w[d], a.p_ab[d], a.p_ba[d], a.A[d], a.B[d], tile, sm);
 }
 
 __global__ __launch_bounds__(256) void unpack_wgrad_kernel(const float* __restrict__ dw, float* __restrict__ grad,
@@ -182,14 +244,13 @@
             a.p_ab[i] = (unsigned short*)(d.transposed ? d.w_dgrad : d.w_fwd);
             a.p_ba[i] = (unsigned short*)(d.transposed ? d.w_fwd : d.w_dgrad);
             a.first[i] = blocks;
-            int b = ew_blocks((int64_t)a.A[i] * a.B[i]);
-            if (b > 512) b = 512;
-            blocks += b;
+            const int64_t b = (int64_t)cdiv(a.A[i], 32) * cdiv(a.B[i], 16);
+            GS_CHECK_ARG(b < (1 << 24), "gs_pack_weight_multi: descriptor %d: too many tiles", base + i);
+            blocks += pack_tiles(a.A[i], a.B[i], a.T[i]);
         }
         a.first[a.n] = blocks;
-        dim3 grid(blocks, 2);
-        if (dtype == GS_F16) pack_weight_multi_kernel<GS_F16><<<grid, 256, 0, s>>>(a);
-        else pack_weight_multi_kernel<GS_BF16><<<grid, 256, 0, s>>>(a);
+        if (dtype == GS_F16) pack_weight_multi_kernel<GS_F16><<<blocks, 256, 0, s>>>(a);
+        else pack_weight_multi_kernel<GS_BF16><<<blocks, 256, 0, s>>>(a);
         GS_CHECK_LAUNCH("gs_pack_weight_multi");
     }
     return GS_OK;
diff --git a/semantic_segmentation_amd/ops.py b/semantic_segmentation_amd/ops.py
--- a/semantic_segmentation_amd/ops.py
+++ b/semantic_segmentation_amd/ops.py
@@ -820,7 +820,20 @@
               _p(partials), N, H, W, C, dt_code(y), _stream())
 
 
-def bn_act_bwd_apply_head(y, dl, w_head, scale, shift, mean, invstd, c1, c2, act, dy):
+def bn_act_bwd_reduce_head_wgrad(y, dl, w_head, scale, shift, mean, invstd, act, partials, dw, db, gscale=1.0, dl_scale=1.0):
+    _dev(y)
+    _f32(dl, "dl"); _f32(w_head, "w_head"); _f32(partials, "partials"); _f32(dw, "dw"); _f32(db, "db")
+    N, H, W, C = y.shape
+    ncls = dl.shape[1]
+    if (C != 64 or tuple(dl.shape) != (N, ncls, H, W) or w_head.numel() != ncls * C or dw.numel() != ncls * C or db.numel() != ncls
+            or not (y.is_contiguous() and dl.is_contiguous() and w_head.is_contiguous() and dw.is_contiguous() and db.is_contiguous())):
+        raise ValueError("bn_act_bwd_reduce_head_wgrad: y [N,H,W,64], dl [N,ncls,H,W], w_head / dw [ncls,64], db [ncls] contiguous")
+    ws = torch.empty(int(_lib.load().gs_bn_head_wgrad_ws_floats(N, H, W, ncls)), dtype=torch.float32, device=y.device)
+    _lib.call("gs_bn_act_bwd_reduce_head_wgrad", _p(y), _p(dl), float(dl_scale), _p(w_head), ncls, _p(scale), _p(shift), _p(mean),
+              _p(invstd), act, _p(partials), _p(dw), _p(db), _p(ws), float(gscale), N, H, W, C, dt_code(y), _stream())
+
+
+def bn_act_bwd_apply_head(y, dl, w_head, scale, shift, mean, invstd, c1, c2, act, dy, dl_scale=1.0):
     _dev(y)
     _f32(dl, "dl"); _f32(w_head, "w_head")
     N, H, W, C = y.shape
@@ -828,7 +841,7 @@
     if tuple(dl.shape) != (N, ncls, H, W) or w_head.numel() != ncls * C or not (dl.is_contiguous() and w_head.is_contiguous()):
         raise ValueError("bn_act_bwd_apply_head: dl [N,ncls,H,W] and w_head [ncls,C] contiguous fp32")
     _lib.call("gs_bn_act_bwd_apply_head", _p(y), _p(dl), _p(w_head), ncls, _p(scale), _p(shift), _p(mean), _p(invstd),
-              _p(c1), _p(c2), act, _p(dy), N, H, W, C, dt_code(y), _stream())
+              _p(c1), _p(c2), act, float(dl_scale), _p(dy), N, H, W, C, dt_code(y), _stream())
 
 
 def bn_partials_colsum(partials, ntiles, Cfull, coff, C, gscale, out):
diff --git a/semantic_segmentation_amd/unet/unet_engine.py b/semantic_segmentation_amd/unet/unet_engine.py
--- a/semantic_segmentation_amd/unet/unet_engine.py
+++ b/semantic_segmentation_amd/unet/unet_engine.py
@@ -927,17 +927,23 @@
         col_ws = empty(1024 * 1024, dtype=torch.float32)
 
         z_last = ctx["z_last"]
-        dl = (dlogits.contiguous().float() * S)
         wout = params["outc.conv.weight"]
+        fused_head_wg = (z_last is None and FUSED_HEAD_BWD and wout.shape[0] <= 4
+                         and os.environ.get("GSSEG_HEAD_WGRAD_FUSED", "1") != "0")
+        dl_scale = 1.0
+        if fused_head_wg and not self.dynamic_loss_scale:
+            dl, dl_scale = dlogits.detach().contiguous().float(), S
+        else:
+            dl = (dlogits.contiguous().float() * S)
         dwo = galloc("outc.conv.weight", wout, zero=True)
         dbo = galloc("outc.conv.bias", params["outc.conv.bias"], zero=True)
         head_src = None
         wout_c = wout.detach().contiguous()
         rlast = recs["up4.conv.3"]
-        if z_last is None:
+        if z_last is None and not fused_head_wg:
             ops.head1x1_bn_wgrad(rlast.y, rlast.coef[0], rlast.coef[1], ACT_RELU, wout_c, dl, dwo, dbo, gscale=inv_s)
         if FUSED_HEAD_BWD and wout.shape[0] <= 4 and dl.is_contiguous():
-            head_src = (dl, wout_c)
+            head_src = (dl, wout_c, dl_scale, (dwo, dbo) if fused_head_wg else None)
             dz = None
             if z_last is not None:
                 ops.conv_smallcout_bwd(z_last, wout_c, dl, None, dwo, dbo, gscale=inv_s)
@@ -959,8 +965,9 @@
                 ops.conv_smallcout_bwd(z_last, wout_c, dl, dz, dwo, dbo, gscale=inv_s)
             else:
                 ops.conv_smallcout_bwd(None, wout_c, dl, dz, None, None)
-        emit("outc.conv.weight", dwo)
-        emit("outc.conv.bias", dbo)
+        if not fused_head_wg:
+            emit("outc.conv.weight", dwo)
+            emit("outc.conv.bias", dbo)
 
         def conv_stage_bwd(rec: _ConvRec, dz_a, sa, ca, dzp, need_dinp: bool, colsum=None, head=None):
             h, w, cin, cout = rec.h, rec.w, rec.cin, rec.cout
@@ -989,7 +996,12 @@
                 ops.conv_smallcin_fwd(rec.inp, wst, None, y_re, None, 3, 1, 1)
                 rec.y = y_re
             ntiles = ops.bn_bwd_tiles_used(N, h, w, pooled)
-            if head is not None:
+            if head is not None and head[3] is not None:
+                ops.bn_act_bwd_reduce_head_wgrad(rec.y, head[0], head[1], coef[0], coef[1], coef[2], coef[3], ACT_RELU, partials,
+                                                 head[3][0], head[3][1], gscale=inv_s, dl_scale=head[2])
+                emit("outc.conv.weight", head[3][0])
+                emit("outc.conv.bias", head[3][1])
+            elif head is not None:
                 ops.bn_act_bwd_reduce_head(rec.y, head[0], head[1], coef[0], coef[1], coef[2], coef[3], ACT_RELU, partials)
             else:
                 ops.bn_act_bwd_reduce(rec.y, dz_a, sa, ca, dzp, coef[0], coef[1], coef[2], coef[3], ACT_RELU, partials)
@@ -1012,7 +1024,8 @@
                     return None
             dy = empty(N, h, w, cout)
             if head is not None:
-                ops.bn_act_bwd_apply_head(rec.y, head[0], head[1], coef[0], coef[1], coef[2], coef[3], c12[0], c12[1], ACT_RELU, dy)
+                ops.bn_act_bwd_apply_head(rec.y, head[0], head[1], coef[0], coef[1], coef[2], coef[3], c12[0], c12[1], ACT_RELU, dy,
+                                          dl_scale=head[2])
             else:
                 ops.bn_act_bwd_apply(rec.y, dz_a, sa, ca, dzp, coef[0], coef[1], coef[2], coef[3], c12[0], c12[1],
                                      ACT_RELU, True, dy)
```

Result: no change. 2104 images/sec (median of 6 runs) (+0.5%).
